# Mamo1031/Multimodal-MTRSSM

Measured on AMD Instinct MI355X. Metric: seq-steps/s (BxT) MoPoE-MRSSM train step, higher is better.
Workload: dtype bf16x2-split, fp32 accumulate; 1 GPU; BASELINE configs[1]: MoPoE-MRSSM train step, B=64/GPU T=50 deter=200 stoch=30, vision 1x64x64 + audio 1x128x32 + action 4; global_batch=64, seq_len=50, parallelism=dp1, hidden=200, embed=256, categoricals_x_classes=6x5, residual_blocks=3, activation=ELU, optimizer=AdamW lr 1e-3 + clip 10 (fused HIP), params=4151600, streams=1, launch=eager (host enqueues every launch), backend=none, rccl_ranks=0, collective_ranks=0, noise=uniforms keyed by global batch row (parallel.GlobalRowNoise)

## Files before the change

### include/mtrssm.h

```cpp
#ifndef MTRSSM_H
#define MTRSSM_H

#include <stddef.h>
#include <stdint.h>

#ifdef __cplusplus
extern "C" {
#endif

#define MTRSSM_VERSION 100

#define MTRSSM_OK 0
#define MTRSSM_EINVAL (-1)
#define MTRSSM_ELAUNCH (-2)
#define MTRSSM_ELDS (-3)

#define MTRSSM_ACT_IDENTITY 0
#define MTRSSM_ACT_RELU 1
#define MTRSSM_ACT_ELU 2
#define MTRSSM_ACT_TANH 3

int mtrssm_version(void);
const char* mtrssm_last_error(void);
const char* mtrssm_last_kernel(void);
// ... 52 lines not shown
  const int32_t* modality;
} MtrssmMrssmFwdIO;

int mtrssm_mrssm_rollout_fwd(const MtrssmMrssmDims* dims, const MtrssmMrssmFwdWeights* w,
                             const MtrssmMrssmFwdIO* io, void* stream);

typedef struct MtrssmMrssmClusterWeights {
  const float* w1s_t;
  const float* wf_t;
  const float* bf;
  const float* whh_t;
  const float* bhh;
  const float* wh1_t;
  const float* b3;
  const float* w4;
  const float* b4;
  const float* wa2;
  const float* ba2;
  const float* wv2;
  const float* bv2;
} MtrssmMrssmClusterWeights;
int mtrssm_mrssm_cluster_supported(const MtrssmMrssmDims* dims);
int64_t mtrssm_mrssm_cluster_workspace_bytes(const MtrssmMrssmDims* dims);
int mtrssm_mrssm_rollout_fwd_cluster(const MtrssmMrssmDims* dims, const MtrssmMrssmClusterWeights* weights, const MtrssmMrssmFwdIO* io,
                                     void* workspace, int64_t workspace_bytes, void* stream);

typedef struct MtrssmMrssmBwdWeights {
  const float* w1s_t;
  const float* w2;
  const float* wih;
  const float* whh;
  const float* wh1;
  const float* w4;
  const float* wa2;
  const float* wv2;
} MtrssmMrssmBwdWeights;

typedef struct MtrssmMrssmBwdIO {
  const float* deter0;
  const float* deter;
  const float* prior_logits;
  const float* post_logits;
  const float* sv_h1;
  const float* sv_h2;
  const float* sv_gates;
  const float* sv_heads;
  const float* sv_la;
  const float* sv_lv;
  const float* g_deter;
  const float* g_post_stoch;
  const float* g_prior_stoch;
  const float* g_post_logits;
  const float* g_prior_logits;
  const float* g_kl;
  float* g_deter0;
  float* g_stoch0;
  float* d_z1;
  float* d_h2;
  float* d_gi;
  float* d_gh;
  float* d_zh;
  float* d_lp;
  float* d_la;
  float* d_lv;
  const float* expert_logw;
  float* g_expert_logw;
  const int32_t* modality;
} MtrssmMrssmBwdIO;

int64_t mtrssm_mrssm_cluster_bwd_workspace_bytes(const MtrssmMrssmDims* dims);
int mtrssm_mrssm_rollout_bwd_cluster(const MtrssmMrssmDims* dims, const MtrssmMrssmClusterWeights* weights, const MtrssmMrssmBwdIO* io,
                                     void* workspace, int64_t workspace_bytes, void* stream);

int mtrssm_mrssm_wide_supported(const MtrssmMrssmDims* dims, int32_t pieces);
int64_t mtrssm_mrssm_wide_workspace_bytes(const MtrssmMrssmDims* dims, int32_t pieces);
int64_t mtrssm_mrssm_wide_bwd_workspace_bytes(const MtrssmMrssmDims* dims, int32_t pieces);
int mtrssm_mrssm_rollout_fwd_wide(const MtrssmMrssmDims* dims, const MtrssmMrssmClusterWeights* weights, const MtrssmMrssmFwdIO* io,
                                  int32_t pieces, void* workspace, int64_t workspace_bytes, void* stream);
int mtrssm_mrssm_rollout_bwd_wide(const MtrssmMrssmDims* dims, const MtrssmMrssmClusterWeights* weights, const MtrssmMrssmBwdIO* io,
                                  int32_t pieces, void* workspace, int64_t workspace_bytes, void* stream);

int mtrssm_mrssm_rollout_bwd(const MtrssmMrssmDims* dims, const MtrssmMrssmBwdWeights* w,
                             const MtrssmMrssmBwdIO* io, void* stream);

typedef struct MtrssmMmtrssmDims {
  int32_t B, T;
  int32_t LD, HD;
  int32_t H;
  int32_t KL, CL;
  int32_t KH, CH;
  int32_t act;
  int32_t post;
  float tau_l, tau_h;
  float keep_l, keep_h;
  float kl_w_post, kl_w_prior;
  int32_t rows_per_block;
  int32_t threads;
} MtrssmMmtrssmDims;

typedef struct MtrssmMmtrssmFwdWeights {
  const float* wxl_s_t;
  const float* wdl_t;
  const float* wxh_t;
  const float* wdh_t;
  const float* bh;
  const float* wl1_t;
  const float* bl1;
  const float* wh1_t;
  const float* bh1;
  const float* wlp2;
  const float* blp2;
  const float* wa2;
  const float* ba2;
  const float* wv2;
  const float* bv2;
  const float* whp2;
  const float* bhp2;
  const float* whq2;
  const float* bhq2;
} MtrssmMmtrssmFwdWeights;

typedef struct MtrssmMmtrssmFwdIO {
  const float* xl;
  const float* pa;
  const float* pv;
  const float* deter_l0;
  const float* deter_h0;
  const float* hidden_l0;
  const float* hidden_h0;
  const float* stoch_l0;
  const float* stoch_h0;
  const float* u_post_l;
  const float* u_post_h;
  const float* u_prior_l;
  const float* u_prior_h;
  float* deter_l;
  float* deter_h;
  float* hidden_l;
  float* hidden_h;
  float* prior_logits_l;
  float* prior_logits_h;
  float* prior_stoch_l;
  float* prior_stoch_h;
  float* post_logits_l;
  float* post_logits_h;
  float* post_stoch_l;
  float* post_stoch_h;
  float* kl_l;
  float* kl_h;
  float* sv_l1;
  float* sv_h1;
  float* sv_la;
  float* sv_lv;
  const float* expert_logw;
  const int32_t* modality;
} MtrssmMmtrssmFwdIO;

int mtrssm_mmtrssm_rollout_fwd(const MtrssmMmtrssmDims* dims, const MtrssmMmtrssmFwdWeights* w,
                               const MtrssmMmtrssmFwdIO* io, void* stream);

typedef struct MtrssmMmtrssmBwdWeights {
  const float* wxl_s_t;
  const float* wdl;
  const float* wxh_t;
  const float* wdh;
  const float* wl1;
// ... 246 lines not shown
```

### multimodal_mtrssm_amd/_lib.py

```python

from __future__ import annotations

import ctypes as C
import os
from pathlib import Path

import torch
from torch import Tensor

_HERE = Path(__file__).resolve().parent
LIB_PATH = _HERE / "libmtrssm_hip.so"

ACT_IDS = {"Identity": 0, "ReLU": 1, "ELU": 2, "Tanh": 3}

_f = C.c_float
_i = C.c_int32
_p = C.c_void_p


def _struct(name: str, fields: list[tuple[str, type]]) -> type:
    return type(name, (C.Structure,), {"_fields_": fields})


def _ptrs(*names: str) -> list[tuple[str, type]]:
    return [(n, _p) for n in names]


MrssmDims = _struct("MtrssmMrssmDims", [
    ("B", _i), ("T", _i), ("D", _i), ("H", _i), ("K", _i), ("C", _i), ("act", _i), ("post", _i),
    ("kl_w_post", _f), ("kl_w_prior", _f), ("rows_per_block", _i), ("threads", _i),
])
MrssmFwdWeights = _struct("MtrssmMrssmFwdWeights", _ptrs(
    "w1s_t", "w2_t", "b2", "wih_t", "bih", "whh_t", "bhh", "wh1_t", "b3", "w4", "b4", "wa2", "ba2", "wv2", "bv2"))
MrssmFwdIO = _struct("MtrssmMrssmFwdIO", _ptrs(
    "xa", "pa", "pv", "deter0", "stoch0", "u_post", "u_prior",
    "deter", "prior_logits", "prior_stoch", "post_logits", "post_stoch", "kl",
    "sv_h1", "sv_h2", "sv_gates", "sv_heads", "sv_la", "sv_lv", "expert_logw", "modality"))
MrssmClusterWeights = _struct("MtrssmMrssmClusterWeights", _ptrs(
    "w1s_t", "wf_t", "bf", "whh_t", "bhh", "wh1_t", "b3", "w4", "b4", "wa2", "ba2", "wv2", "bv2"))
MrssmBwdWeights = _struct("MtrssmMrssmBwdWeights", _ptrs("w1s_t", "w2", "wih", "whh", "wh1", "w4", "wa2", "wv2"))
MrssmBwdIO = _struct("MtrssmMrssmBwdIO", _ptrs(
    "deter0", "deter", "prior_logits", "post_logits", "sv_h1", "sv_h2", "sv_gates", "sv_heads", "sv_la", "sv_lv",
    "g_deter", "g_post_stoch", "g_prior_stoch", "g_post_logits", "g_prior_logits", "g_kl",
    "g_deter0", "g_stoch0", "d_z1", "d_h2", "d_gi", "d_gh", "d_zh", "d_lp", "d_la", "d_lv", "expert_logw", "g_expert_logw", "modality"))

MmtrssmDims = _struct("MtrssmMmtrssmDims", [
    ("B", _i), ("T", _i), ("LD", _i), ("HD", _i), ("H", _i), ("KL", _i), ("CL", _i), ("KH", _i), ("CH", _i),
    ("act", _i), ("post", _i), ("tau_l", _f), ("tau_h", _f), ("keep_l", _f), ("keep_h", _f),
    ("kl_w_post", _f), ("kl_w_prior", _f), ("rows_per_block", _i), ("threads", _i),
])
MmtrssmFwdWeights = _struct("MtrssmMmtrssmFwdWeights", _ptrs(
    "wxl_s_t", "wdl_t", "wxh_t", "wdh_t", "bh", "wl1_t", "bl1", "wh1_t", "bh1",
    "wlp2", "blp2", "wa2", "ba2", "wv2", "bv2", "whp2", "bhp2", "whq2", "bhq2"))
MmtrssmFwdIO = _struct("MtrssmMmtrssmFwdIO", _ptrs(
    "xl", "pa", "pv", "deter_l0", "deter_h0", "hidden_l0", "hidden_h0", "stoch_l0", "stoch_h0",
    "u_post_l", "u_post_h", "u_prior_l", "u_prior_h",
    "deter_l", "deter_h", "hidden_l", "hidden_h", "prior_logits_l", "prior_logits_h", "prior_stoch_l", "prior_stoch_h",
    "post_logits_l", "post_logits_h", "post_stoch_l", "post_stoch_h", "kl_l", "kl_h",
    "sv_l1", "sv_h1", "sv_la", "sv_lv", "expert_logw", "modality"))
MmtrssmBwdWeights = _struct("MtrssmMmtrssmBwdWeights", _ptrs(
    "wxl_s_t", "wdl", "wxh_t", "wdh", "wl1", "wh1", "wlp2", "wa2", "wv2", "whp2", "whq2"))
MmtrssmBwdIO = _struct("MtrssmMmtrssmBwdIO", _ptrs(
    "deter_l0", "deter_h0", "deter_l", "deter_h", "prior_logits_l", "prior_logits_h", "post_logits_l", "post_logits_h",
    "sv_l1", "sv_h1", "sv_la", "sv_lv",
    "g_deter_l", "g_deter_h", "g_hidden_l", "g_hidden_h", "g_post_stoch_l", "g_post_stoch_h", "g_prior_stoch_l",
    "g_prior_stoch_h", "g_post_logits_l", "g_post_logits_h", "g_prior_logits_l", "g_prior_logits_h", "g_kl_l", "g_kl_h",
    "g_deter_l0", "g_deter_h0", "g_hidden_l0", "g_hidden_h0", "g_stoch_l0", "g_stoch_h0",
    "d_ul", "d_uh", "d_zl1", "d_zh1", "d_lpl", "d_la", "d_lv", "d_lph", "d_lqh", "expert_logw", "g_expert_logw", "modality"))

ConvGeom = _struct("MtrssmConvGeom", [(n, _i) for n in (
    "N", "C", "Hs", "Ws", "C2", "Cpad", "KH", "KW", "SS", "TS", "OFFY", "OFFX", "Hq", "Wq", "OS", "QY", "QX", "Ho", "Wo",
    "Cout", "CoutPad", "pre_act", "act", "mfma_split")])

Gemm = _struct("MtrssmGemm", _ptrs("A", "B", "C", "bias", "zgrad", "colsum") + [(n, _i) for n in (
    "M", "N", "R", "lda", "ldb", "ldc", "ldz", "a_rmajor", "b_rmajor", "act_a", "act_b", "act_out", "act_z", "accumulate", "split_r")]
    + [("tickets", _p), ("n_tickets", _i), ("mfma_split", _i)])

ElboSchedule = _struct("MtrssmElboSchedule", [(n, _f) for n in ("c0", "c1", "free0", "free1", "w_a", "w_v", "beta_start", "warmup")])

STATE_MAX = 6
StateTable = _struct("MtrssmStateTable", [
    ("count", _i), ("width", _i * STATE_MAX), ("src_stride", C.c_int64 * STATE_MAX), ("src", _p * STATE_MAX), ("alt", _p * STATE_MAX),
    ("dst", _p * STATE_MAX)])

SYMBOLS: dict[str, tuple[type | None, list[type]]] = {
    "mtrssm_version": (C.c_int, []),
    "mtrssm_last_error": (C.c_char_p, []),
    "mtrssm_last_kernel": (C.c_char_p, []),
    "mtrssm_mrssm_rollout_fwd": (C.c_int, [C.POINTER(MrssmDims), C.POINTER(MrssmFwdWeights), C.POINTER(MrssmFwdIO), _p]),
    "mtrssm_mrssm_cluster_supported": (C.c_int, [C.POINTER(MrssmDims)]),
    "mtrssm_mrssm_cluster_workspace_bytes": (C.c_int64, [C.POINTER(MrssmDims)]),
    "mtrssm_mrssm_rollout_fwd_cluster": (C.c_int, [C.POINTER(MrssmDims), C.POINTER(MrssmClusterWeights), C.POINTER(MrssmFwdIO), _p, C.c_int64, _p]),
    "mtrssm_mrssm_cluster_bwd_workspace_bytes": (C.c_int64, [C.POINTER(MrssmDims)]),
    "mtrssm_mrssm_rollout_bwd_cluster": (C.c_int, [C.POINTER(MrssmDims), C.POINTER(MrssmClusterWeights), C.POINTER(MrssmBwdIO), _p, C.c_int64, _p]),
    "mtrssm_mrssm_wide_supported": (C.c_int, [C.POINTER(MrssmDims), _i]),
    "mtrssm_mrssm_wide_workspace_bytes": (C.c_int64, [C.POINTER(MrssmDims), _i]),
    "mtrssm_mrssm_wide_bwd_workspace_bytes": (C.c_int64, [C.POINTER(MrssmDims), _i]),
    "mtrssm_mrssm_rollout_fwd_wide": (C.c_int, [C.POINTER(MrssmDims), C.POINTER(MrssmClusterWeights), C.POINTER(MrssmFwdIO), _i, _p, C.c_int64, _p]),
    "mtrssm_mrssm_rollout_bwd_wide": (C.c_int, [C.POINTER(MrssmDims), C.POINTER(MrssmClusterWeights), C.POINTER(MrssmBwdIO), _i, _p, C.c_int64, _p]),
    "mtrssm_mrssm_rollout_bwd": (C.c_int, [C.POINTER(MrssmDims), C.POINTER(MrssmBwdWeights), C.POINTER(MrssmBwdIO), _p]),
    "mtrssm_mmtrssm_rollout_fwd": (C.c_int, [C.POINTER(MmtrssmDims), C.POINTER(MmtrssmFwdWeights), C.POINTER(MmtrssmFwdIO), _p]),
    "mtrssm_mmtrssm_rollout_bwd": (C.c_int, [C.POINTER(MmtrssmDims), C.POINTER(MmtrssmBwdWeights), C.POINTER(MmtrssmBwdIO), _p]),
    "mtrssm_mmtrssm_wide_supported": (C.c_int, [C.POINTER(MmtrssmDims), _i]),
    "mtrssm_mmtrssm_wide_workspace_bytes": (C.c_int64, [C.POINTER(MmtrssmDims), _i]),
    "mtrssm_mmtrssm_wide_bwd_workspace_bytes": (C.c_int64, [C.POINTER(MmtrssmDims), _i]),
    "mtrssm_mmtrssm_rollout_fwd_wide": (C.c_int, [C.POINTER(MmtrssmDims), C.POINTER(MmtrssmFwdWeights), C.POINTER(MmtrssmFwdIO), _i, _p, C.c_int64, _p]),
    "mtrssm_mmtrssm_rollout_bwd_wide": (C.c_int, [C.POINTER(MmtrssmDims), C.POINTER(MmtrssmBwdWeights), C.POINTER(MmtrssmBwdIO), _i, _p, C.c_int64, _p]),
    "mtrssm_conv_gather_gemm": (C.c_int, [C.POINTER(ConvGeom), _p, _p, _p, _p, _p, _p, _p, _p, _p]),
    "mtrssm_conv_gather_gemm_pair": (C.c_int, [C.POINTER(ConvGeom), _p, _p, _p, _p, _p, _p, _p, _p,
                                               C.POINTER(ConvGeom), _p, _p, _p, _p, _p, _p, _p, _p, _p]),
    "mtrssm_conv_gather_pair_merges": (C.c_int, [C.POINTER(ConvGeom), C.POINTER(ConvGeom), _i]),
    "mtrssm_residual_block_fwd_supported": (C.c_int, [C.POINTER(ConvGeom)]),
    "mtrssm_residual_block_fwd": (C.c_int, [C.POINTER(ConvGeom), _p, _p, _p, _p, _p, _p, _p, C.POINTER(ConvGeom), _p, _p, _p, _p, _p, _p, _p, _p]),
    "mtrssm_pack_conv_weight": (C.c_int, [_p, _i, _i, _i, _i, C.c_int64, C.c_int64, C.c_int64, C.c_int64, _i, _i, _i, _p, _p, _p]),
    "mtrssm_pack_conv_weights": (C.c_int, [_p, _i, _i, _p]),
    "mtrssm_unpack_conv_grads": (C.c_int, [_p, _i, _i, _p]),
    "mtrssm_conv_weight_grad": (C.c_int, [C.POINTER(ConvGeom), _p, _p, _p, _i, _p, _p, _p, C.c_int64, _p]),
    "mtrssm_conv_weight_grad_deferred": (C.c_int, [C.POINTER(ConvGeom), _p, _p, _p, _i, _p, _p, _p, C.c_int64, _p]),
    "mtrssm_residual_bwd1x1_supported": (C.c_int, [C.POINTER(ConvGeom)]),
    "mtrssm_residual_bwd1x1": (C.c_int, [C.POINTER(ConvGeom), _p, _p, _p, _p, _p, _p, _p, C.c_int64, _i, _p]),
    "mtrssm_conv_weight_grad_src_bias_supported": (C.c_int, [C.POINTER(ConvGeom), _i]),
    "mtrssm_conv_weight_grad_src_bias": (C.c_int, [C.POINTER(ConvGeom), _p, _p, _i, _p, _p, _p, C.c_int64, _i, _p]),
    "mtrssm_conv_weight_grad_reduce": (C.c_int, [_p]),
    "mtrssm_conv_weight_grad_workspace_bytes": (C.c_int64, [C.POINTER(ConvGeom), _i]),
    "mtrssm_residual_bwd1x1_pair_supported": (C.c_int, [C.POINTER(ConvGeom), C.POINTER(ConvGeom)]),
    "mtrssm_residual_bwd1x1_pair": (C.c_int, [C.POINTER(ConvGeom), _p, _p, _p, _p, _p, _p, _p, C.c_int64,
                                              C.POINTER(ConvGeom), _p, _p, _p, _p, _p, _p, _p, C.c_int64, _i, _p]),
    "mtrssm_conv_weight_grad_pair_supported": (C.c_int, [C.POINTER(ConvGeom), C.POINTER(ConvGeom)]),
    "mtrssm_conv_weight_grad_pair": (C.c_int, [C.POINTER(ConvGeom), _p, _p, _p, _p, _p, C.c_int64,
                                               C.POINTER(ConvGeom), _p, _p, _p, _p, _p, C.c_int64, _i, _p]),
    "mtrssm_channel_sum": (C.c_int, [_p, _i, _i, _i, _p, _p]),
    "mtrssm_convt_k4s2_thin": (C.c_int, [_i, _i, _i, _i, _i, _p, _p, _p, _i, _i, _p, _p]),
    "mtrssm_convt_k4s2_band_supported": (C.c_int, [_i, _i, _i, _i, _i]),
    "mtrssm_convt_k4s2_band": (C.c_int, [_i, _i, _i, _i, _i, _p, _p, _p, _i, _i, _p, _p]),
    "mtrssm_convt_quad_supported": (C.c_int, [C.POINTER(ConvGeom)]),
    "mtrssm_convt_quad": (C.c_int, [C.POINTER(ConvGeom), _p, C.POINTER(C.c_void_p), _p, _p, _p, C.POINTER(ConvGeom), _p, C.POINTER(C.c_void_p),
                                    _p, _p, _p, _p]),
    "mtrssm_conv_tgather_thin": (C.c_int, [_i] * 11 + [_p, _p, _p, _i, _i, _p, _p, _p, _p]),
    "mtrssm_episode_gather": (C.c_int, [_p, _p, _p, C.c_int64, C.c_int64, C.c_int64, C.c_int64, C.c_int64, _f, _p, _p, _p]),
    "mtrssm_episode_gather_window": (C.c_int, [_p, _p, _p, _p, C.c_int64, C.c_int64, C.c_int64, C.c_int64, C.c_int64, _f, _p, _p, _p]),
    "mtrssm_state_select": (C.c_int, [C.POINTER(StateTable), _p, C.c_int64, _p]),
    "mtrssm_state_save": (C.c_int, [C.POINTER(StateTable), C.c_int64, C.c_int64, _p]),
    "mtrssm_state_save_at": (C.c_int, [C.POINTER(StateTable), _p, C.c_int64, C.c_int64, _p]),
    "mtrssm_episode_gather_ragged": (C.c_int, [_p, _p, _p, _p, _p, C.c_int64, C.c_int64, C.c_int64, C.c_int64, C.c_int64, _f, _p, _p, _p, _p]),
    "mtrssm_episode_gather_seeded": (C.c_int, [_p, _p, _p, _p, _p, C.c_uint32, C.c_uint32, C.c_uint32, C.c_int64, C.c_int64, C.c_int64, C.c_int64,
                                               C.c_int64, _f, _p, _p, _p]),
    "mtrssm_step_mask_ragged": (C.c_int, [_p, _p, C.c_int64, C.c_int64, C.c_int64, _f, _f, C.c_int64, C.c_int64, _p, _p, _p, _p, _p, _p, _p, _p]),
    "mtrssm_step_mask_forecast": (C.c_int, [_p, _p, _p, C.c_int64, C.c_int64, C.c_int64, _f, _f, C.c_int64, C.c_int64, C.c_int64, C.c_int64, _p, _p, _p,
                                            _p, _p, _p, _p, _p, _p]),
    "mtrssm_ensemble_score": (C.c_int, [_p, _p, _p, C.c_int64, C.c_int64, C.c_int64, C.c_int64, _i, _p, _p, _p, _p, _p, _p]),
    "mtrssm_horizon_table": (C.c_int, [_p, C.c_int64, _p, _p, C.c_int64, C.c_int64, _p, _p, _p]),
    "mtrssm_digit_features": (C.c_int, [_p, C.c_int64, _p, C.c_int64, _i, _p, _p, _p, _p, _p, _p]),
    "mtrssm_digit_head": (C.c_int, [_p, _p, _p, C.c_int64, _p, C.c_int64, _p, _p, _p]),
    "mtrssm_word_counts": (C.c_int, [_p, _p, C.c_int64, _p, _p]),
    "mtrssm_elbo_combine_counted_fwd": (C.c_int, [_p, _p, _p, _p, _p, _p, C.c_int64, C.c_float, C.c_float, _p, _p, _p, _p, _p]),
    "mtrssm_elbo_combine_counted_bwd": (C.c_int, [_p, _p, _p, _p, _p, _p, C.c_int64, C.c_float, C.c_float, _p, _p, _p, _p, _p]),
    "mtrssm_elbo_schedule_fwd": (C.c_int, [_p, _p, _p, _p, _p, _p, _p, C.c_int64, ElboSchedule, _p, _p, _p, _p, _p, _p, _p]),
    "mtrssm_elbo_schedule_bwd": (C.c_int, [_p, _p, _p, _p, _p, _p, _p, _p, _p, C.c_int64, ElboSchedule, _p, _p, _p, _p, _p]),
    "mtrssm_elbo_combine_fwd": (C.c_int, [_p, _p, _p, _p, C.c_int64, C.c_float, C.c_float, _p, _p, _p, _p, _p]),
    "mtrssm_elbo_combine_bwd": (C.c_int, [_p, _p, _p, _p, C.c_int64, C.c_float, C.c_float, _p, _p, _p, _p, _p]),
    "mtrssm_categorical_sample_fwd": (C.c_int, [_p, _p, C.c_int64, _i, _i, _p, _p, _p, _p]),
    "mtrssm_categorical_sample_bwd": (C.c_int, [_p, _p, _p, C.c_int64, _i, _i, _p, _p]),
    "mtrssm_gaussian_nll_fwd": (C.c_int, [_p, _p, C.c_int64, C.c_int64, _i, _p, _p]),
    "mtrssm_gaussian_nll_bwd": (C.c_int, [_p, _p, _p, C.c_int64, C.c_int64, _i, _p, _p]),
    "mtrssm_gaussian_nll_masked_fwd": (C.c_int, [_p, _p, _p, _p, C.c_int64, C.c_int64, _i, _p, _p]),
    "mtrssm_gaussian_nll_masked_bwd": (C.c_int, [_p, _p, _p, _p, _p, C.c_int64, C.c_int64, _i, _p, _p]),
    "mtrssm_modality_dropout": (C.c_int, [_p, C.c_int64, C.c_int64, C.c_int64, _f, _f, C.c_int64, C.c_int64, _p, _p, _p, _p, _p, _p]),
    "mtrssm_sumsq": (C.c_int, [_p, C.c_int64, _p, _p]),
    "mtrssm_adamw_step": (C.c_int, [_p, _p, _p, _p, C.c_int64, _p, _f, _f, _f, _f, _f, _f, _f, _i, _p]),
    "mtrssm_gemm": (C.c_int, [C.POINTER(Gemm), _p]),
    "mtrssm_gemm_group": (C.c_int, [C.POINTER(Gemm), _i, _p]),
    "mtrssm_clear": (C.c_int, [_p, C.c_int64, _p]),
    "mtrssm_adamw_prepare": (C.c_int, [_p, C.c_int64, _p, _p, _p, _f, _f, _p]),
    "mtrssm_adamw_apply": (C.c_int, [_p, _p, _p, _p, _p, C.c_int64, _p, _p, _p, _f, _f, _f, _f, _f, _f, _p]),
}

_LIB: C.CDLL | None = None


class MtrssmLibraryError(RuntimeError):
    """The HIP library is missing or a kernel call failed.  There is no fallback path."""


# ... 113 lines not shown
```

### multimodal_mtrssm_amd/cnn.py

```python

from __future__ import annotations

from typing import Any

import torch
from torch import Tensor, nn

from multimodal_mtrssm_amd import _lib
from multimodal_mtrssm_amd.linear import linear
from multimodal_mtrssm_amd.conv import (
    gemm_pieces,
    conv2d,
    conv2d_pair,
    conv_transpose2d,
    conv_transpose2d_pair,
    residual_block,
    residual_block_pair,
)


def _act(name: str) -> nn.Module:
    return getattr(nn, name)()


def _cfg(config: Any) -> dict[str, Any]:
    return dict(config) if isinstance(config, dict) else dict(vars(config))


def _conv(x: Tensor, m: nn.Conv2d, *, pre_act: bool, act: int, coords: Tensor | None = None) -> Tensor:
    return conv2d(x, m.weight, m.bias, stride=m.stride[0], padding=m.padding[0], pre_act=pre_act, act=act, coords=coords)


def _deconv(x: Tensor, m: nn.ConvTranspose2d, *, pre_act: bool, act: int) -> Tensor:
    return conv_transpose2d(x, m.weight, m.bias, stride=m.stride[0], padding=m.padding[0],
                            output_padding=m.output_padding[0], pre_act=pre_act, act=act)


class ResidualBlock(nn.Module):

    def __init__(self, channels: int, intermediate: int, activation_name: str) -> None:
        super().__init__()
        self.conv3 = nn.Conv2d(channels, intermediate, 3, 1, 1)
        self.conv1 = nn.Conv2d(intermediate, channels, 1, 1, 0)
        self.act_id = _lib.ACT_IDS[activation_name]

    def forward(self, x: Tensor) -> Tensor:
        return residual_block(x, self.conv3.weight, self.conv3.bias, self.conv1.weight, self.conv1.bias, act=self.act_id)

    def params(self) -> tuple[Tensor, Tensor, Tensor, Tensor]:
        return self.conv3.weight, self.conv3.bias, self.conv1.weight, self.conv1.bias


def _res_pair(res_a: nn.ModuleList, res_b: nn.ModuleList, xa: Tensor, xb: Tensor) -> tuple[Tensor, Tensor]:
    n = min(len(res_a), len(res_b))
    for ba, bb in zip(res_a[:n], res_b[:n], strict=True):
        if ba.act_id == bb.act_id and ba.conv3.weight.shape == bb.conv3.weight.shape and ba.conv1.weight.shape == bb.conv1.weight.shape:
            xa, xb = residual_block_pair(xa, ba.params(), xb, bb.params(), act=ba.act_id)
        else:
            xa, xb = ba(xa), bb(xb)
    for ba in res_a[n:]:
        xa = ba(xa)
    for bb in res_b[n:]:
        xb = bb(xb)
    return xa, xb


def _same_layer(ma: nn.Module, mb: nn.Module) -> bool:
    return (ma.weight.shape[0] == mb.weight.shape[0] and ma.weight.shape[2:] == mb.weight.shape[2:] and ma.stride == mb.stride
            and ma.padding == mb.padding and getattr(ma, "output_padding", 0) == getattr(mb, "output_padding", 0))


def _conv_pair(xa: Tensor, ma: nn.Conv2d, ca: Tensor | None, xb: Tensor, mb: nn.Conv2d, cb: Tensor | None, *, pre_act: bool,
               act_a: int, act_b: int) -> tuple[Tensor, Tensor]:
    if _same_layer(ma, mb) and act_a == act_b:
        return conv2d_pair((xa, ma.weight, ma.bias, ma.stride[0], ma.padding[0], pre_act, act_a, ca),
                           (xb, mb.weight, mb.bias, mb.stride[0], mb.padding[0], pre_act, act_b, cb))
    return _conv(xa, ma, pre_act=pre_act, act=act_a, coords=ca), _conv(xb, mb, pre_act=pre_act, act=act_b, coords=cb)


def encode_pair(enc_a: "Encoder", enc_b: "Encoder", xa: Tensor, xb: Tensor) -> tuple[Tensor, Tensor]:
    lead_a, lead_b = xa.shape[:-3], xb.shape[:-3]
    xa, ca = enc_a.prepare(xa)
    xb, cb = enc_b.prepare(xb)
    if len(enc_a.convs) == len(enc_b.convs) and (enc_a.res_in is None) == (enc_b.res_in is None):
        for i, (ma, mb) in enumerate(zip(enc_a.convs, enc_b.convs, strict=True)):
            xa, xb = _conv_pair(xa, ma, ca if i == 0 else None, xb, mb, cb if i == 0 else None, pre_act=i > 0, act_a=enc_a.act_id,
                                act_b=enc_b.act_id)
        if enc_a.res_in is not None:
            xa, xb = _conv_pair(xa, enc_a.res_in, None, xb, enc_b.res_in, None, pre_act=True, act_a=enc_a.act_id, act_b=enc_b.act_id)
    else:
        xa, xb = enc_a.stem_convs(xa, ca), enc_b.stem_convs(xb, cb)
    xa, xb = _res_pair(enc_a.res, enc_b.res, xa, xb)
    return enc_a.head(xa, lead_a), enc_b.head(xb, lead_b)


def decode_pair(dec_a: "Decoder", dec_b: "Decoder", fa: Tensor, fb: Tensor, *, raw: bool = False) -> tuple[Tensor, Tensor]:
    lead_a, lead_b = fa.shape[:-1], fb.shape[:-1]
    xa, xb = dec_a.stem(fa), dec_b.stem(fb)
    xa, xb = _res_pair(dec_a.res, dec_b.res, xa, xb)
    if len(dec_a.deconvs) != len(dec_b.deconvs) or (len(dec_a.res) > 0) != (len(dec_b.res) > 0):
        return dec_a.tail(xa, lead_a, raw=raw), dec_b.tail(xb, lead_b, raw=raw)
    for i, (ma, mb) in enumerate(zip(dec_a.deconvs, dec_b.deconvs, strict=True)):
        pre = i > 0 or len(dec_a.res) > 0
        if _same_layer(ma, mb) and dec_a.act_id == dec_b.act_id:
            xa, xb = conv_transpose2d_pair(
                (xa, ma.weight, ma.bias, ma.stride[0], ma.padding[0], ma.output_padding[0], pre, dec_a.act_id),
                (xb, mb.weight, mb.bias, mb.stride[0], mb.padding[0], mb.output_padding[0], pre, dec_b.act_id))
        else:
            xa, xb = _deconv(xa, ma, pre_act=pre, act=dec_a.act_id), _deconv(xb, mb, pre_act=pre, act=dec_b.act_id)
    return dec_a.finish(xa, lead_a, raw=raw), dec_b.finish(xb, lead_b, raw=raw)


class Encoder(nn.Module):

    def __init__(self, config: Any) -> None:
        super().__init__()
        self.cfg = _cfg(config)
        self.coord_conv = bool(self.cfg.get("coord_conv", False))
        self.act = _act(self.cfg["activation_name"])
        self.act_id = _lib.ACT_IDS[self.cfg["activation_name"]]
        self.out_act = _act(self.cfg.get("out_activation_name", "Identity"))
        self.convs = nn.ModuleList()
        self.res_in: nn.Module | None = None
        self.res = nn.ModuleList()
        self.linears = nn.ModuleList()
        self.input_shape: tuple[int, int, int] | None = None
        self._coords: Tensor | None = None
        if self.cfg.get("input_shape") is not None:
            self.materialize(tuple(self.cfg["input_shape"]))

    def materialize(self, input_shape: tuple[int, ...]) -> None:
        cfg = self.cfg
        c, h, w = (int(v) for v in input_shape)
        self.input_shape = (c, h, w)
        cin = c + (2 if self.coord_conv else 0)
        for ch, k, s, p in zip(cfg["channels"], cfg["kernel_sizes"], cfg["strides"], cfg["paddings"], strict=True):
            self.convs.append(nn.Conv2d(cin, ch, k, s, p))
            h, w, cin = (h + 2 * p - k) // s + 1, (w + 2 * p - k) // s + 1, ch
        if cfg.get("num_residual_blocks", 0) > 0:
            rout = cfg["residual_output_size"]
            self.res_in = nn.Conv2d(cin, rout, 3, 1, 1)
            for _ in range(cfg["num_residual_blocks"]):
                self.res.append(ResidualBlock(rout, cfg["residual_intermediate_size"], cfg["activation_name"]))
            cin = rout
        width = cin * h * w
        for out in cfg["linear_sizes"]:
            self.linears.append(nn.Linear(width, out))
            width = out

    def _coord_channels(self, x: Tensor) -> Tensor:
        h, w = x.shape[-2:]
        if self._coords is None or self._coords.shape[-2:] != (h, w) or self._coords.device != x.device:
            yy = torch.linspace(-1.0, 1.0, h, dtype=x.dtype, device=x.device)
            xx = torch.linspace(-1.0, 1.0, w, dtype=x.dtype, device=x.device)
            self._coords = torch.stack([yy[:, None].expand(h, w), xx[None, :].expand(h, w)], dim=0)
        return self._coords

    def forward(self, x: Tensor) -> Tensor:
        lead = x.shape[:-3]
        x = self.stem(x)
        for blk in self.res:
            x = blk(x)
        return self.head(x, lead)

    def prepare(self, x: Tensor) -> tuple[Tensor, Tensor | None]:
        if len(self.linears) == 0:
            self.materialize(tuple(x.shape[-3:]))
            self.to(x.device)
        x = x.reshape(-1, *x.shape[-3:]).float()
        return x, (self._coord_channels(x) if self.coord_conv else None)

    def stem_convs(self, x: Tensor, coords: Tensor | None) -> Tensor:
        for i, conv in enumerate(self.convs):
            x = _conv(x, conv, pre_act=i > 0, act=self.act_id, coords=coords if i == 0 else None)
        if self.res_in is not None:
            x = _conv(x, self.res_in, pre_act=True, act=self.act_id)
        return x

    def stem(self, x: Tensor) -> Tensor:
        return self.stem_convs(*self.prepare(x))

    def head(self, x: Tensor, lead: torch.Size) -> Tensor:
        x = x.flatten(start_dim=1)
        for lin in self.linears:
            x = linear(x, lin.weight, lin.bias, pre_act=self.act_id, pieces=gemm_pieces())
        return self.out_act(x).reshape(*lead, -1)


class Decoder(nn.Module):

    def __init__(self, config: Any) -> None:
        super().__init__()
        cfg = self.cfg = _cfg(config)
        self.act = _act(cfg["activation_name"])
        self.act_id = _lib.ACT_IDS[cfg["activation_name"]]
        self.out_act = _act(cfg.get("out_activation_name", "Identity"))
        self.conv_in_shape = tuple(int(v) for v in cfg["conv_in_shape"])
        self.linears = nn.ModuleList()
        self.res = nn.ModuleList()
        self.deconvs = nn.ModuleList()
        cin = self.conv_in_shape[0]
        for _ in range(cfg.get("num_residual_blocks", 0)):
            self.res.append(ResidualBlock(cin, cfg["residual_intermediate_size"], cfg["activation_name"]))
        n = len(cfg["channels"])
        ops = cfg.get("output_paddings", [0] * n)
        for ch, k, s, p, op in zip(cfg["channels"], cfg["kernel_sizes"], cfg["strides"], cfg["paddings"], ops, strict=True):
            self.deconvs.append(nn.ConvTranspose2d(cin, ch, k, s, p, op))
            cin = ch
        if cfg.get("in_features") is not None:
            self.materialize(int(cfg["in_features"]))

    def materialize(self, in_features: int) -> None:
        width = in_features
        for out in self.cfg["linear_sizes"]:
            self.linears.append(nn.Linear(width, out))
            width = out
        self.in_features = in_features

    def forward(self, f: Tensor, *, raw: bool = False) -> Tensor:
        lead = f.shape[:-1]
        x = self.stem(f)
        for blk in self.res:
            x = blk(x)
        return self.tail(x, lead, raw=raw)

    @property
    def out_act_id(self) -> int | None:
        name = type(self.out_act).__name__
        return {"Identity": 0, "Tanh": 3}.get(name)

    def stem(self, f: Tensor) -> Tensor:
        if len(self.linears) == 0:
            self.materialize(f.shape[-1])
            self.to(f.device)
        x = f.reshape(-1, f.shape[-1])
        for i, lin in enumerate(self.linears):
            x = linear(x, lin.weight, lin.bias, pre_act=self.act_id if i > 0 else 0, pieces=gemm_pieces())
        return x.reshape(-1, *self.conv_in_shape)

    def tail(self, x: Tensor, lead: torch.Size, *, raw: bool = False) -> Tensor:
        for i, dc in enumerate(self.deconvs):
            x = _deconv(x, dc, pre_act=i > 0 or len(self.res) > 0, act=self.act_id)
        return self.finish(x, lead, raw=raw)

    def finish(self, x: Tensor, lead: torch.Size, *, raw: bool = False) -> Tensor:
        if not raw:
            x = self.out_act(x)
        return x.reshape(*lead, *x.shape[-3:])
```

### multimodal_mtrssm_amd/core.py

```python

from __future__ import annotations

import torch
from torch import Tensor, nn

from multimodal_mtrssm_amd import cnn, conv, scan
from multimodal_mtrssm_amd.carry import StateCarry
from multimodal_mtrssm_amd.distributions import MultiOneHot, MultiOneHotFactory, draw_uniforms, kl_divergence, onehot_from_uniforms
from multimodal_mtrssm_amd.digits import DigitClassifier, word_counts
from multimodal_mtrssm_amd.dropout import ModalityDropout, StepMask, ragged_step_mask
from multimodal_mtrssm_amd.experts import ExpertWeights
from multimodal_mtrssm_amd.forecast import Forecast
from multimodal_mtrssm_amd.networks import MTRNN, Representation, Transition
from multimodal_mtrssm_amd.objective import likelihood
from multimodal_mtrssm_amd.schedule import ElboSchedule, ElboTerms
from multimodal_mtrssm_amd.skill import ForecastSkill, SkillTable
from multimodal_mtrssm_amd.words import TransitionTable, WordTransitions
from multimodal_mtrssm_amd.state import MTState, State

try:
    from lightning import LightningModule as _Base
except ImportError:

    class _Base(nn.Module):
        @property
        def device(self) -> torch.device:
            for p in self.parameters():
                return p.device
            return torch.device("cpu")

        def log_dict(self, *args, **kwargs) -> None:
            return None


Noise = dict[str, Tensor | None]

def _pairable(a: nn.Module, b: nn.Module, kind: type) -> bool:
    return conv.PAIR_LAUNCH and isinstance(a, kind) and isinstance(b, kind)


def _st_onehot(dist: MultiOneHot, u: Tensor | None) -> Tensor:
    if u is None:
        return dist.rsample()
    onehot = onehot_from_uniforms(dist.probs.detach(), u.to(dist.probs))
    return (onehot + (dist.probs - dist.probs.detach())).flatten(start_dim=-2)


class _CategoricalHead(torch.autograd.Function):

    @staticmethod
    def forward(ctx, logits: Tensor, u: Tensor, cats: int, classes: int):
        from multimodal_mtrssm_amd import _lib

        ctx.set_materialize_grads(False)
        logits, u = logits.contiguous().float(), u.contiguous().float()
        rows = logits.numel() // (cats * classes)
        logp = torch.empty(*logits.shape[:-1], cats, classes, device=logits.device, dtype=torch.float32)
        probs, onehot = torch.empty_like(logp), torch.empty_like(logits)
        _lib.check(_lib.load().mtrssm_categorical_sample_fwd(_lib.ptr(logits), _lib.ptr(u), rows, cats, classes, _lib.ptr(logp), _lib.ptr(probs),
                                                             _lib.ptr(onehot), _lib.stream_ptr(logits.device)), "mtrssm_categorical_sample_fwd")
        ctx.save_for_backward(probs)
        ctx.dims = (rows, cats, classes)
        return onehot, logp, probs

    @staticmethod
    def backward(ctx, g_stoch, g_logp, g_probs):
        from multimodal_mtrssm_amd import _lib

        (probs,) = ctx.saved_tensors
        rows, cats, classes = ctx.dims
        gp = None
        if g_stoch is not None:
            gp = g_stoch.reshape(probs.shape)
        if g_probs is not None:
            gp = g_probs if gp is None else gp + g_probs
        if gp is None and g_logp is None:
            return None, None, None, None
        gp = None if gp is None else gp.contiguous().float()
        gl = None if g_logp is None else g_logp.contiguous().float()
        d = torch.empty(*probs.shape[:-2], cats * classes, device=probs.device, dtype=torch.float32)
        _lib.check(_lib.load().mtrssm_categorical_sample_bwd(_lib.ptr(probs), _lib.ptr(gp), _lib.ptr(gl), rows, cats, classes, _lib.ptr(d),
                                                             _lib.stream_ptr(probs.device)), "mtrssm_categorical_sample_bwd")
        return d, None, None, None


class _ElboCombine(torch.autograd.Function):

    @staticmethod
    def forward(ctx, nll_a: Tensor, nll_v: Tensor, kl0: Tensor, kl1: Tensor | None, c0: float, c1: float):
        from multimodal_mtrssm_amd import _lib

        ctx.set_materialize_grads(False)
        nll_a, nll_v, kl0 = nll_a.contiguous().float(), nll_v.contiguous().float(), kl0.contiguous().float()
        kl1 = None if kl1 is None else kl1.contiguous().float()
        outs = [torch.empty((), device=kl0.device, dtype=torch.float32) for _ in range(4)]
        _lib.check(_lib.load().mtrssm_elbo_combine_fwd(_lib.ptr(nll_a), _lib.ptr(nll_v), _lib.ptr(kl0), _lib.ptr(kl1), kl0.numel(), float(c0), float(c1),
                                                       _lib.ptr(outs[0]), _lib.ptr(outs[1]), _lib.ptr(outs[2]) if kl1 is not None else None,
                                                       _lib.ptr(outs[3]), _lib.stream_ptr(kl0.device)), "mtrssm_elbo_combine_fwd")
        ctx.meta = (kl0.shape, None if kl1 is None else kl1.shape, float(c0), float(c1))
        ctx.dev = kl0.device
        return outs[0], outs[1], outs[2], outs[3]

    @staticmethod
    def backward(ctx, g_recon, g_k0, g_k1, g_loss):
        from multimodal_mtrssm_amd import _lib

        shape0, shape1, c0, c1 = ctx.meta
        n = 1
        for d in shape0:
            n *= d
        g_a, g_v = (torch.empty((), device=ctx.dev, dtype=torch.float32) for _ in range(2))
        g_kl0 = torch.empty(shape0, device=ctx.dev, dtype=torch.float32)
        g_kl1 = None if shape1 is None else torch.empty(shape1, device=ctx.dev, dtype=torch.float32)
        opt = lambda t: None if t is None else _lib.ptr(t.contiguous().float())
        _lib.check(_lib.load().mtrssm_elbo_combine_bwd(opt(g_recon), opt(g_k0), opt(g_k1) if shape1 is not None else None, opt(g_loss), n, c0, c1,
                                                       _lib.ptr(g_a), _lib.ptr(g_v), _lib.ptr(g_kl0), _lib.ptr(g_kl1), _lib.stream_ptr(ctx.dev)),
                   "mtrssm_elbo_combine_bwd")
        return g_a, g_v, g_kl0, g_kl1, None, None


class _ElboCombineCounted(torch.autograd.Function):

    @staticmethod
    def forward(ctx, nll_a: Tensor, nll_v: Tensor, kl0: Tensor, kl1: Tensor | None, live: Tensor, count: Tensor, c0: float, c1: float):
        from multimodal_mtrssm_amd import _lib

        ctx.set_materialize_grads(False)
        nll_a, nll_v, kl0 = nll_a.contiguous().float(), nll_v.contiguous().float(), kl0.contiguous().float()
        kl1 = None if kl1 is None else kl1.contiguous().float()
        live, count = live.contiguous().float(), count.contiguous().float()
        if live.numel() != kl0.numel() or count.numel() != 1:
            msg = f"live must have one entry per KL step ({kl0.numel()}), count one; got {live.numel()} and {count.numel()}"
            raise ValueError(msg)
        outs = [torch.empty((), device=kl0.device, dtype=torch.float32) for _ in range(4)]
        _lib.check(_lib.load().mtrssm_elbo_combine_counted_fwd(
            _lib.ptr(nll_a), _lib.ptr(nll_v), _lib.ptr(kl0), _lib.ptr(kl1), _lib.ptr(live), _lib.ptr(count), kl0.numel(), float(c0), float(c1),
            _lib.ptr(outs[0]), _lib.ptr(outs[1]), _lib.ptr(outs[2]) if kl1 is not None else None, _lib.ptr(outs[3]),
            _lib.stream_ptr(kl0.device)), "mtrssm_elbo_combine_counted_fwd")
        ctx.meta = (kl0.shape, None if kl1 is None else kl1.shape, float(c0), float(c1))
        ctx.dev = kl0.device
        ctx.save_for_backward(live, count)
        return outs[0], outs[1], outs[2], outs[3]

    @staticmethod
    def backward(ctx, g_recon, g_k0, g_k1, g_loss):
        from multimodal_mtrssm_amd import _lib

        shape0, shape1, c0, c1 = ctx.meta
        live, count = ctx.saved_tensors
        g_a, g_v = (torch.empty((), device=ctx.dev, dtype=torch.float32) for _ in range(2))
        g_kl0 = torch.empty(shape0, device=ctx.dev, dtype=torch.float32)
        g_kl1 = None if shape1 is None else torch.empty(shape1, device=ctx.dev, dtype=torch.float32)
        opt = lambda t: None if t is None else _lib.ptr(t.contiguous().float())
        _lib.check(_lib.load().mtrssm_elbo_combine_counted_bwd(
            opt(g_recon), opt(g_k0), opt(g_k1) if shape1 is not None else None, opt(g_loss), _lib.ptr(live), _lib.ptr(count), live.numel(), c0, c1,
            _lib.ptr(g_a), _lib.ptr(g_v), _lib.ptr(g_kl0), _lib.ptr(g_kl1), _lib.stream_ptr(ctx.dev)), "mtrssm_elbo_combine_counted_bwd")
        return g_a, g_v, g_kl0, g_kl1, None, None, None, None


class _ElboScheduled(torch.autograd.Function):

    @staticmethod
    def forward(ctx, nll_a: Tensor, nll_v: Tensor, kl0: Tensor, kl1: Tensor | None, live: Tensor | None, count: Tensor | None,
                step: Tensor | None, sched: ElboSchedule, c0: float, c1: float):
        from multimodal_mtrssm_amd import _lib

# ... 197 lines not shown
        self.vision_decoder = vision_decoder
        self.scan_rows_per_block = 0
        self.scan_threads = 0
        self.modality_dropout: ModalityDropout | None = None
        self.state_carry: StateCarry | None = None
        self.forecast: Forecast | None = None
        self.val_forecast: Forecast | None = None
        self.elbo_schedule: ElboSchedule | None = None
        self.val_skill: ForecastSkill | None = None
        self.skill_table: SkillTable | None = None
        self.expert_weights: ExpertWeights | None = None
        self.weights_timeseries: Tensor | None = None
        self._weights_both: Tensor | None = None

    @staticmethod
    def get_observations_from_batch(batch: tuple[Tensor, ...]) -> tuple[Tensor, Tensor]:
        return batch[1], batch[2]

    @staticmethod
    def get_initial_observation(observations: tuple[Tensor, Tensor]) -> tuple[Tensor, Tensor]:
        audio_obs, vision_obs = observations
        return audio_obs[:, 0], vision_obs[:, 0]

    @staticmethod
    def get_targets_from_batch(batch: tuple[Tensor, ...]) -> dict[str, Tensor]:
        return {"recon/audio": batch[4], "recon/vision": batch[5]}

    @staticmethod
    def get_modality_mask_from_batch(batch: tuple[Tensor, ...]) -> Tensor | None:
        return batch[6] if len(batch) > 6 else None

    def encode_observation(self, observation: tuple[Tensor, Tensor] | Tensor, modality_mask: Tensor | None = None) -> Tensor:
        if isinstance(observation, tuple):
            audio_obs, vision_obs = observation
            ea = None if audio_obs is None else self.audio_encoder(audio_obs)
            ev = None if vision_obs is None else self.vision_encoder(vision_obs)
            if ea is None and ev is None:
                msg = "observation: at least one of (audio_obs, vision_obs) must be given"
                raise ValueError(msg)
            return _masked_mean_embed(ea, ev, modality_mask)
        return observation

    def decode_state(self, state: State | MTState) -> dict[str, Tensor]:
        return {"recon/audio": self.audio_decoder(state.feature), "recon/vision": self.vision_decoder(state.feature)}

    @staticmethod
    def compute_reconstruction_loss(reconstructions: dict[str, Tensor], targets: dict[str, Tensor],
                                    modality_mask: Tensor | None = None) -> dict[str, Tensor]:
        fa = fv = None
        if modality_mask is not None:
            fa, fv = modality_mask[..., 0], modality_mask[..., 1]
        audio = likelihood(prediction=reconstructions["recon/audio"], target=targets["recon/audio"], event_ndims=3, frame_mask=fa)
        vision = likelihood(prediction=reconstructions["recon/vision"], target=targets["recon/vision"], event_ndims=3, frame_mask=fv)
        return {"recon": audio + vision, "recon/audio": audio, "recon/vision": vision}

    def _encode_both(self, audio_obs: Tensor, vision_obs: Tensor) -> tuple[Tensor, Tensor]:
        if _pairable(self.audio_encoder, self.vision_encoder, cnn.Encoder):
            return cnn.encode_pair(self.audio_encoder, self.vision_encoder, audio_obs, vision_obs)
        return self.audio_encoder(audio_obs), self.vision_encoder(vision_obs)

    def _reconstruction_losses(self, feature: Tensor, targets: dict[str, Tensor], *, sum_recon: bool = True,
                               modality_mask: Tensor | None = None, step_mask: StepMask | None = None) -> dict[str, Tensor]:
        da, dv = self.audio_decoder, self.vision_decoder
        fused = isinstance(da, cnn.Decoder) and isinstance(dv, cnn.Decoder) and da.out_act_id is not None and dv.out_act_id is not None
        if fused and _pairable(da, dv, cnn.Decoder):
            pa, pv = cnn.decode_pair(da, dv, feature, feature, raw=True)
        elif fused:
            pa, pv = da(feature, raw=True), dv(feature, raw=True)
        else:
            pa, pv = da(feature), dv(feature)
        fa = fv = ca = cv = None
        if modality_mask is not None:
            fa, fv = modality_mask[..., 0], modality_mask[..., 1]
        if step_mask is not None:
            ca, cv = (step_mask.present_audio, step_mask.count_audio), (step_mask.present_vision, step_mask.count_vision)
        audio = likelihood(prediction=pa, target=targets["recon/audio"], event_ndims=3, out_act=da.out_act_id if fused else 0,
                           frame_mask=fa, frame_present=ca)
        vision = likelihood(prediction=pv, target=targets["recon/vision"], event_ndims=3, out_act=dv.out_act_id if fused else 0,
                            frame_mask=fv, frame_present=cv)
        if not sum_recon:
            return {"recon/audio": audio, "recon/vision": vision}
        return {"recon": audio + vision, "recon/audio": audio, "recon/vision": vision}

    def _initial_from_embed(self, obs_embed: Tensor, u_init: Tensor | None) -> State:
        deter = self.init_proj(obs_embed)
        logits = self.transition.rnn_to_prior_projector(deter)
        dist, stoch = _sampled_head(self.representation.distribution_factory, logits, u_init)
        return State(deter=deter, distribution=dist, stoch=stoch)

    def _initial_embed(self, observation: tuple[Tensor, Tensor] | Tensor, modality_mask: Tensor | None) -> Tensor:
        if modality_mask is not None:
            if not isinstance(observation, tuple):
                msg = "modality_mask needs the (audio_obs, vision_obs) tuple"
                raise ValueError(msg)
            ref = observation[0] if observation[0] is not None else observation[1]
            _check_modality_mask(modality_mask, ref.shape[0], None, ref.device, first_step=True)
            for j, name in enumerate(("audio", "vision")):
                if observation[j] is None and bool(modality_mask[:, j].any()):
                    msg = f"modality_mask marks {name} present, but the observation carries None for it"
                    raise ValueError(msg)
        return self.encode_observation(observation, modality_mask)

    def initial_state(self, observation: tuple[Tensor, Tensor] | Tensor, noise: Noise | None = None,
                      modality_mask: Tensor | None = None) -> State:
        u = None if noise is None else noise.get("u_init")
        return self._initial_from_embed(self._initial_embed(observation, modality_mask), u).to(self.device)

    def noise_shapes(self, batch: int, steps: int) -> dict[str, tuple[int, ...]]:
        k = self.transition.distribution_factory.category_size
        return self._with_mask_noise({"u_init": (batch, k), "u_post": (batch, steps, k)}, batch, steps)

    def _with_mask_noise(self, shapes: dict[str, tuple[int, ...]], batch: int, steps: int) -> dict[str, tuple[int, ...]]:
        if self.modality_dropout is not None:
            shapes["u_mask"] = self.modality_dropout.noise_shape(batch, steps)
        if self.forecast is not None:
            shapes["u_context"] = self.forecast.noise_shape(batch)
        return shapes

    def _rollout_embedded(self, actions: Tensor, audio_embed: Tensor | None, vision_embed: Tensor | None, prev_state: State,
                          noise: Noise | None, *, sample_prior: bool, modality: Tensor | None = None,
                          expert_log_weights: Tensor | None = None) -> dict[str, Tensor]:
        noise = noise or {}
        B, T = actions.shape[:2]
        K = self.transition.distribution_factory.category_size
        logw = self._expert_logw(audio_embed, vision_embed, expert_log_weights, B, T)
        self._report_weights(logw, modality, B, T, actions.device)
        u_post = noise.get("u_post")
        u_prior = noise.get("u_prior")
        if u_post is None:
            u_post = _rand(actions, B, T, K)
        if u_prior is None and sample_prior:
            u_prior = _rand(actions, B, T, K)
        return scan.mrssm_posterior_rollout(
            self.transition, self.audio_representation, self.vision_representation, actions, audio_embed, vision_embed,
            prev_state.deter, prev_state.stoch, u_post, u_prior, balancing=bool(self.use_kl_balancing),
            rows_per_block=self.scan_rows_per_block, threads=self.scan_threads, modality=modality, expert_logw=logw,
        )

    def _expert_logw(self, audio_embed: Tensor | None, vision_embed: Tensor | None, explicit: Tensor | None, B: int, T: int) -> Tensor | None:
        if audio_embed is None or vision_embed is None:
            return None
        if explicit is not None:
            return scan.check_expert_logw(explicit, B, T)
        if self.expert_weights is None:
            return None
        return self.expert_weights(audio_embed, vision_embed)

    def _report_weights(self, logw: Tensor | None, codes: Tensor | None, B: int, T: int, device: torch.device) -> None:
        if logw is None and self.expert_weights is None:
            return
        with torch.no_grad():
            if codes is None:
                codes = torch.full((B, T), 3, device=device, dtype=torch.int32)
            self._weights_both = (codes & 3) == 3
            self.weights_timeseries = ExpertWeights.table(logw, codes & 3)

    def _posterior_from_rollout(self, out: dict[str, Tensor]) -> State:
        post = State(deter=out["deter"], distribution=self.audio_representation.distribution_factory(out["post_logits"]), stoch=out["post_stoch"])
        post.kl_per_step = out["kl"]
        return post

    def _states_from_rollout(self, out: dict[str, Tensor]) -> tuple[State, State]:
        factory = self.audio_representation.distribution_factory
        prior = State(deter=out["deter"], distribution=factory(out["prior_logits"]), stoch=out["prior_stoch"])
        return self._posterior_from_rollout(out), prior

    def rollout_representation(
# ... 343 lines not shown
                return None
            _check_modality_mask(mask, B, T, batch[0].device, first_step=True)
            return StepMask.from_mask(mask)
        if mask is not None:
            msg = "give a modality_mask (or a 7-tuple batch) or a modality_dropout, not both"
            raise ValueError(msg)
        if not isinstance(modality_dropout, ModalityDropout):
            msg = f"modality_dropout must be a ModalityDropout, got {type(modality_dropout).__name__}"
            raise ValueError(msg)
        return modality_dropout.sample(self._dropout_uniforms(batch, noise, modality_dropout, modality_dropout.world), T).step_mask()

    def shared_step(self, batch: tuple[Tensor, ...], noise: Noise | None = None, modality_mask: Tensor | None = None,
                    modality_dropout: ModalityDropout | None = None, state_carry: StateCarry | None = None,
                    reset: Tensor | None = None, *, carry_prefix: str = "train", lengths: Tensor | None = None,
                    forecast: Forecast | None = None, elbo_schedule: ElboSchedule | None = None,
                    expert_log_weights: Tensor | None = None) -> dict[str, Tensor]:
        if forecast is not None:
            if modality_mask is not None or self.get_modality_mask_from_batch(batch) is not None:
                msg = "forecast= decides what the model observes: a modality_mask (or a 7-tuple batch) already says what is seen, give one of them"
                raise ValueError(msg)
            if state_carry is not None:
                msg = "forecast= does not combine with state_carry: the state a forecast step ends with is an open-loop state, not one to continue from"
                raise ValueError(msg)
            return self._elbo_step(batch, noise, self._forecast_step_mask(batch, noise, forecast, modality_dropout, lengths), schedule=elbo_schedule,
                                   expert_log_weights=expert_log_weights)
        reset_host = None
        if state_carry is not None:
            reset_host = getattr(batch, "reset_host", None) if reset is None else (None if reset.is_cuda else reset)
        on_device = state_carry is not None and isinstance(reset, Tensor) and reset.is_cuda
        sm = self._step_mask(batch, noise, modality_mask, modality_dropout, lengths, reset_host, trust_reset=on_device)
        if state_carry is None:
            return self._elbo_step(batch, noise, sm, schedule=elbo_schedule, expert_log_weights=expert_log_weights)
        return self._elbo_step(batch, noise, sm, self._carry_of(batch, state_carry, reset, carry_prefix), schedule=elbo_schedule,
                               expert_log_weights=expert_log_weights)

    @staticmethod
    def _carry_of(batch: tuple[Tensor, ...], state_carry: StateCarry, reset: Tensor | None, prefix: str) -> tuple[StateCarry, str, Tensor]:
        if not isinstance(state_carry, StateCarry):
            msg = f"state_carry must be a StateCarry, got {type(state_carry).__name__}"
            raise ValueError(msg)
        dev = batch[0].device
        if reset is None:
            reset, reset_host = getattr(batch, "reset", None), getattr(batch, "reset_host", None)
            if reset is None:
                msg = "state_carry needs reset= (bool [B]) or a batch that carries one (an EpisodeBatch of a windowed loader)"
                raise ValueError(msg)
        elif not isinstance(reset, Tensor) or reset.dtype != torch.bool:
            msg = f"reset must be a bool tensor, got {getattr(reset, 'dtype', type(reset))}"
            raise ValueError(msg)
        else:
            reset_host = None if reset.is_cuda else reset
        if tuple(reset.shape) != (batch[0].shape[0],):
            msg = f"reset must have shape ({batch[0].shape[0]},), got {tuple(reset.shape)}"
            raise ValueError(msg)
        state_carry.check(prefix, batch[0].shape[0], reset_host)
        return state_carry, prefix, reset.to(dev).contiguous()

    _FRESH_KEYS = ("deter", "stoch")
    _LAST_KEYS = {"deter": "deter", "stoch": "post_stoch"}

    def _state0(self, fresh: State | MTState, carry: tuple[StateCarry, str, Tensor] | None) -> State | MTState:
        if carry is None:
            return fresh
        sc, prefix, reset = carry
        got = sc.select(prefix, reset, {k: getattr(fresh, k) for k in self._FRESH_KEYS})
        return self._state_like(fresh, got)

    @staticmethod
    def _state_like(fresh: State, got: dict[str, Tensor]) -> State:
        return State(deter=got["deter"], distribution=fresh.distribution, stoch=got["stoch"])

    def _save_carry(self, out: dict[str, Tensor], carry: tuple[StateCarry, str, Tensor] | None, last: Tensor | None = None) -> None:
        if carry is not None:
            carry[0].save(carry[1], {k: out[v] for k, v in self._LAST_KEYS.items()}, last)

    def _elbo_step(self, batch: tuple[Tensor, ...], noise: Noise | None, sm: StepMask | None,
                   carry: tuple[StateCarry, str, Tensor] | None = None, schedule: ElboSchedule | None = None,
                   expert_log_weights: Tensor | None = None) -> dict[str, Tensor]:
        action_input = batch[0]
        audio_obs, vision_obs = self.get_observations_from_batch(batch)
        conv.begin_step(audio_obs.device)
        audio_embed, vision_embed = self._encode_both(audio_obs, vision_obs)
        u_init = None if noise is None else noise.get("u_init")
        state0 = self._initial_from_embed(_masked_mean_embed(audio_embed[:, 0], vision_embed[:, 0], None if sm is None else sm.mask0),
                                          u_init)
        state0 = self._state0(state0, carry)
        out = self._rollout_embedded(action_input, audio_embed, vision_embed, state0, noise, sample_prior=False,
                                     modality=None if sm is None else sm.codes, expert_log_weights=expert_log_weights)
        self._save_carry(out, carry, None if sm is None else sm.last)
        feature = torch.cat([out["deter"], out["post_stoch"]], dim=-1)
        parts = self._reconstruction_losses(feature, self.get_targets_from_batch(batch), sum_recon=False, step_mask=sm)
        recon, kl_div, _, loss = _elbo(parts["recon/audio"], parts["recon/vision"], out["kl"], float(self.kl_coeff), step_mask=sm, schedule=schedule)
        if schedule is not None:
            return {"recon": recon, **parts, "kl": kl_div, "loss": loss, "kl_raw": schedule.stats["kl_raw"]}
        return {"recon": recon, **parts, "kl": kl_div, "loss": loss}

    def _step(self, batch: tuple[Tensor, ...], prefix: str, *, with_loss_key: bool, modality_dropout: ModalityDropout | None = None,
              forecast: Forecast | None = None, elbo_schedule: ElboSchedule | None = None) -> dict[str, Tensor]:
        if forecast is not None:
            loss_dict = self.shared_step(batch, modality_dropout=modality_dropout, state_carry=self.state_carry, forecast=forecast,
                                         elbo_schedule=elbo_schedule)
        elif self.state_carry is None:
            loss_dict = self.shared_step(batch, modality_dropout=modality_dropout, elbo_schedule=elbo_schedule)
        else:
            loss_dict = self.shared_step(batch, modality_dropout=modality_dropout, state_carry=self.state_carry, carry_prefix=prefix,
                                         elbo_schedule=elbo_schedule)
        renamed = {"loss": loss_dict["loss"]} if with_loss_key else {}
        renamed[f"{prefix}/loss"] = loss_dict["loss"]
        for key, value in loss_dict.items():
            if key != "loss":
                renamed[f"{prefix}/{key}"] = value
        self.log_dict(renamed, prog_bar=True, sync_dist=True, on_step=False, on_epoch=True)
        return renamed

    def training_step(self, batch: tuple[Tensor, ...], _: int = 0) -> dict[str, Tensor]:
        return self._step(batch, "train", with_loss_key=True, modality_dropout=self.modality_dropout, forecast=self.forecast,
                          elbo_schedule=self.elbo_schedule)

    def validation_step(self, batch: tuple[Tensor, ...], _batch_index: int = 0) -> dict[str, Tensor]:
        logged = self._step(batch, "val", with_loss_key=False)
        if self.expert_weights is not None and self.weights_timeseries is not None:
            both = self._weights_both.unsqueeze(-1).to(torch.float32)
            mean = (self.weights_timeseries * both).sum(dim=(0, 1)) / both.sum().clamp(min=1.0)
            weights = {f"val/weights/{name}": mean[i] for i, name in enumerate(("audio", "vision", "fused"))}
            self.log_dict(weights, prog_bar=False, sync_dist=True, on_step=False, on_epoch=True)
            logged.update(weights)
        if self.val_forecast is not None:
            fore = {f"val/forecast/{k}": v for k, v in self.shared_step(batch, forecast=self.val_forecast).items()}
            self.log_dict(fore, prog_bar=False, sync_dist=True, on_step=False, on_epoch=True)
            logged.update(fore)
        if self.val_skill is not None:
            self.skill_table = self.forecast_skill(batch, self.val_skill, table=self.skill_table)
        return logged

    def on_validation_epoch_end(self) -> dict[str, Tensor]:
        table, self.skill_table = self.skill_table, None
        if table is None:
            return {}
        table.all_reduce(getattr(self.val_skill, "group", None))
        logged = table.scalars("val/skill")
        self.log_dict(logged, prog_bar=False, sync_dist=False, on_step=False, on_epoch=True)
        return logged


class MoPoE_MMTRSSM(MoPoE_MRSSM):

    def __init__(
        self,
        *,
        audio_representation: Representation,
        vision_representation: Representation,
        audio_encoder: nn.Module,
        vision_encoder: nn.Module,
        audio_decoder: nn.Module,
        vision_decoder: nn.Module,
        init_proj: nn.Module,
        kl_coeff: float,
        use_kl_balancing: bool,
        action_size: int,
        hd_dim: int,
        hs_dim: int,
        ld_dim: int,
        ls_dim: int,
        l_tau: float,
        h_tau: float,
        l_prior: nn.Module,
        l_posterior: nn.Module,
        h_prior: nn.Module,
# ... 182 lines not shown
```

### multimodal_mtrssm_amd/csrc/capi.hip

```cpp
#include <stdarg.h>
#include <stdio.h>

#include "scan_common.h"

namespace mtrssm {

static thread_local char g_err[512] = "";
static thread_local const char* g_kernel = "";

void set_last_kernel(const char* name) { g_kernel = name; }

void set_error(const char* fmt, ...) {
  va_list ap;
  va_start(ap, fmt);
  vsnprintf(g_err, sizeof(g_err), fmt, ap);
  va_end(ap);
}

int mrssm_fwd_launch(const MtrssmMrssmDims*, const MtrssmMrssmFwdWeights*, const MtrssmMrssmFwdIO*, hipStream_t);
int mrssm_bwd_launch(const MtrssmMrssmDims*, const MtrssmMrssmBwdWeights*, const MtrssmMrssmBwdIO*, hipStream_t);
int mmtrssm_fwd_launch(const MtrssmMmtrssmDims*, const MtrssmMmtrssmFwdWeights*, const MtrssmMmtrssmFwdIO*, hipStream_t);
int mmtrssm_bwd_launch(const MtrssmMmtrssmDims*, const MtrssmMmtrssmBwdWeights*, const MtrssmMmtrssmBwdIO*, hipStream_t);
int conv_gather_gemm_launch(const MtrssmConvGeom*, const float*, const float*, const float*, const unsigned short*, const float*, const float*, const float*, float*, hipStream_t);
int episode_gather_launch(const float*, const int64_t*, const float*, int64_t, int64_t, int64_t, int64_t, int64_t, float, float*, float*, hipStream_t);
// ... 6 lines not shown
                                 int64_t, float, float*, float*, int32_t*, hipStream_t);
int episode_gather_seeded_launch(const float*, const int64_t*, const int32_t*, const int32_t*, int32_t*, uint32_t, uint32_t, uint32_t, int64_t, int64_t,
                                 int64_t, int64_t, int64_t, float, float*, float*, hipStream_t);
int step_mask_ragged_launch(const int32_t*, const float*, int64_t, int64_t, int64_t, float, float, int64_t, int64_t, int32_t*, float*, float*, float*,
                            unsigned char*, int32_t*, float*, hipStream_t);
int step_mask_forecast_launch(const int32_t*, const float*, const float*, int64_t, int64_t, int64_t, float, float, int64_t, int64_t, int64_t, int64_t,
                              int32_t*, float*, float*, float*, float*, unsigned char*, int32_t*, float*, hipStream_t);
int elbo_combine_counted_fwd_launch(const float*, const float*, const float*, const float*, const float*, const float*, int64_t, float, float, float*,
                                    float*, float*, float*, hipStream_t);
int elbo_combine_counted_bwd_launch(const float*, const float*, const float*, const float*, const float*, const float*, int64_t, float, float, float*,
                                    float*, float*, float*, hipStream_t);
int elbo_schedule_fwd_launch(const float*, const float*, const float*, const float*, const float*, const float*, const float*, int64_t,
                             MtrssmElboSchedule, float*, float*, float*, float*, float*, float*, hipStream_t);
int elbo_schedule_bwd_launch(const float*, const float*, const float*, const float*, const float*, const float*, const float*, const float*,
                             const float*, int64_t, MtrssmElboSchedule, float*, float*, float*, float*, hipStream_t);
int conv_gather_gemm_pair_launch(const MtrssmConvGeom*, const float*, const float*, const float*, const unsigned short*, const float*, const float*, const float*, float*,
                                 const MtrssmConvGeom*, const float*, const float*, const float*, const unsigned short*, const float*, const float*, const float*, float*, hipStream_t);
int conv_residual_fwd_supported(const MtrssmConvGeom*);
int conv_residual_fwd_launch(const MtrssmConvGeom*, const float*, const unsigned short*, const float*, const float*, const float*, float*, float*,
                             const MtrssmConvGeom*, const float*, const unsigned short*, const float*, const float*, const float*, float*, float*, hipStream_t);
int pack_conv_weight_launch(const float*, int, int, int, int, long, long, long, long, int, int, int, float*, unsigned short*, hipStream_t);
int pack_conv_weights_launch(const int64_t*, int, int, hipStream_t);
int conv_gather_pair_merges(const MtrssmConvGeom*, const MtrssmConvGeom*, bool);
int conv_weight_grad_launch(const MtrssmConvGeom*, const float*, const float*, const float*, int, float*, float*, void*, size_t, size_t*, hipStream_t);
int conv_weight_grad_deferred_launch(const MtrssmConvGeom*, const float*, const float*, const float*, int, float*, float*, void*, size_t, hipStream_t);
int conv_weight_grad_reduce_flush(hipStream_t);
int conv_residual_bwd1x1_supported(const MtrssmConvGeom*);
int conv_residual_bwd1x1_launch(const MtrssmConvGeom*, const float*, const float*, const unsigned short*, float*, float*, float*, void*, size_t, int,
                                hipStream_t);
int conv_residual_bwd1x1_pair_supported(const MtrssmConvGeom*, const MtrssmConvGeom*);
int conv_residual_bwd1x1_pair_launch(const MtrssmConvGeom*, const float*, const float*, const unsigned short*, float*, float*, float*, void*, size_t,
                                     const MtrssmConvGeom*, const float*, const float*, const unsigned short*, float*, float*, float*, void*, size_t, int,
                                     hipStream_t);
int conv_weight_grad_pair_supported(const MtrssmConvGeom*, const MtrssmConvGeom*);
int conv_weight_grad_pair_launch(const MtrssmConvGeom*, const float*, const float*, float*, float*, void*, size_t, const MtrssmConvGeom*, const float*,
                                 const float*, float*, float*, void*, size_t, int, hipStream_t);
int conv_weight_grad_src_bias_supported(const MtrssmConvGeom*, int);
int conv_weight_grad_src_bias_launch(const MtrssmConvGeom*, const float*, const float*, int, float*, float*, void*, size_t, int, hipStream_t);
int channel_sum_launch(const float*, int, int, int, float*, hipStream_t);
int convt_k4s2_band_supported(int, int, int, int, int);
int convt_k4s2_band_launch(int, int, int, int, int, const float*, const float*, const float*, int, int, float*, hipStream_t);
int convt_k4s2_thin_launch(int, int, int, int, int, const float*, const float*, const float*, int, int, float*, hipStream_t);
int conv_convt_quad_supported(const MtrssmConvGeom*);
int conv_convt_quad_launch(const MtrssmConvGeom*, const float*, const unsigned short* const*, const float*, const float*, float*,
                           const MtrssmConvGeom*, const float*, const unsigned short* const*, const float*, const float*, float*, hipStream_t);
int conv_tgather_thin_launch(int, int, int, int, int, int, int, int, int, int, int, const float*, const float*, const float*, int, int, const float*,
                             const float*, float*, hipStream_t);
int categorical_sample_fwd_launch(const float*, const float*, int64_t, int, int, float*, float*, float*, hipStream_t);
int categorical_sample_bwd_launch(const float*, const float*, const float*, int64_t, int, int, float*, hipStream_t);
int elbo_combine_fwd_launch(const float*, const float*, const float*, const float*, int64_t, float, float, float*, float*, float*, float*, hipStream_t);
int elbo_combine_bwd_launch(const float*, const float*, const float*, const float*, int64_t, float, float, float*, float*, float*, float*, hipStream_t);
int nll_fwd_launch(const float*, const float*, int64_t, int64_t, int, float*, hipStream_t);
int nll_bwd_launch(const float*, const float*, const float*, int64_t, int64_t, int, float*, hipStream_t);
int nll_masked_fwd_launch(const float*, const float*, const float*, const float*, int64_t, int64_t, int, float*, hipStream_t);
int nll_masked_bwd_launch(const float*, const float*, const float*, const float*, const float*, int64_t, int64_t, int, float*, hipStream_t);
int ensemble_score_launch(const float*, const float*, const int32_t*, int64_t, int64_t, int64_t, int64_t, int, float*, float*, float*, float*, float*,
                          hipStream_t);
int horizon_table_launch(const float*, int64_t, const int32_t*, const int32_t*, int64_t, int64_t, float*, float*, hipStream_t);
int digit_features_launch(const float*, int64_t, const int32_t*, int64_t, int, const float*, const float*, const float*, const float*, float*,
                          hipStream_t);
int digit_head_launch(const float*, const float*, const float*, int64_t, const int32_t*, int64_t, int32_t*, float*, hipStream_t);
int word_counts_launch(const int32_t*, const int32_t*, int64_t, float*, hipStream_t);
int modality_dropout_launch(const float*, int64_t, int64_t, int64_t, float, float, int64_t, int64_t, int32_t*, float*, float*, unsigned char*, float*,
                            hipStream_t);
int sumsq_launch(const float*, int64_t, float*, hipStream_t);
int adamw_launch(float*, const float*, float*, float*, int64_t, const float*, float, float, float, float, float, float, float, int, hipStream_t);
int gemm_launch(const MtrssmGemm*, hipStream_t);
int gemm_group_launch(const MtrssmGemm*, int, hipStream_t);
int debug_set_cluster_profile(void*);
int debug_set_resident_profile(void*);
int debug_set_wide_profile(void*);
int debug_set_mmt_profile(void*);
int mrssm_cluster_supported(const MtrssmMrssmDims*);
size_t mrssm_cluster_workspace_bytes(const MtrssmMrssmDims*);
size_t mrssm_cluster_bwd_workspace_bytes(const MtrssmMrssmDims*);
int mrssm_bwd_cluster_launch(const MtrssmMrssmDims*, const MtrssmMrssmClusterWeights*, const MtrssmMrssmBwdIO*, void*, size_t, hipStream_t);
int mrssm_fwd_cluster_launch(const MtrssmMrssmDims*, const MtrssmMrssmClusterWeights*, const MtrssmMrssmFwdIO*, void*, size_t, hipStream_t);
int unpack_conv_grads_launch(const int64_t*, int, int, hipStream_t);
int mrssm_wide_supported(const MtrssmMrssmDims*, int);
size_t mrssm_wide_workspace_bytes(const MtrssmMrssmDims*, int);
size_t mrssm_wide_bwd_workspace_bytes(const MtrssmMrssmDims*, int);
int mrssm_wide_fwd_launch(const MtrssmMrssmDims*, const MtrssmMrssmClusterWeights*, const MtrssmMrssmFwdIO*, int, void*, size_t, hipStream_t);
int mrssm_wide_bwd_launch(const MtrssmMrssmDims*, const MtrssmMrssmClusterWeights*, const MtrssmMrssmBwdIO*, int, void*, size_t, hipStream_t);
int adamw_prepare_launch(const float*, int64_t, float*, float*, const int*, float, float, hipStream_t);
int adamw_apply_launch(float*, const float*, float*, float*, const unsigned char*, int64_t, const float*, const float*, const int*, float, float, float,
                       float, float, float, hipStream_t);

int mmtrssm_wide_supported(const MtrssmMmtrssmDims*, int);
size_t mmtrssm_wide_workspace_bytes(const MtrssmMmtrssmDims*, int);
size_t mmtrssm_wide_bwd_workspace_bytes(const MtrssmMmtrssmDims*, int);
int mmtrssm_wide_fwd_launch(const MtrssmMmtrssmDims*, const MtrssmMmtrssmFwdWeights*, const MtrssmMmtrssmFwdIO*, int, void*, size_t, hipStream_t);
int mmtrssm_wide_bwd_launch(const MtrssmMmtrssmDims*, const MtrssmMmtrssmBwdWeights*, const MtrssmMmtrssmBwdIO*, int, void*, size_t, hipStream_t);

int device_cu_count() {
  static int cached[64] = {0};
  int dev = 0;
  if (hipGetDevice(&dev) != hipSuccess) { (void)hipGetLastError(); return 0; }
  if (dev < 0 || dev >= 64) return 0;
  if (cached[dev] > 0) return cached[dev];
  int v = 0;
  if (hipDeviceGetAttribute(&v, hipDeviceAttributeMultiprocessorCount, dev) != hipSuccess || v <= 0) { (void)hipGetLastError(); return 0; }
  cached[dev] = v;
  return v;
}

}

using namespace mtrssm;
#define MTRSSM_API extern "C" __attribute__((visibility("default")))

template <typename IO>
static bool expert_logw_ok(const IO* io, bool post, const char* entry) {
  if (io && post && io->expert_logw && !io->modality) {
    set_error("%s: expert_logw needs modality (pass code 3 everywhere when no modality is missing)", entry);
    return false;
  }
  return true;
}
template <typename IO>
static bool g_expert_logw_ok(const IO* io, const char* entry) {
  if (!expert_logw_ok(io, true, entry)) return false;
  if (io && io->g_expert_logw && !io->expert_logw) {
    set_error("%s: g_expert_logw needs expert_logw", entry);
    return false;
  }
  return true;
}

MTRSSM_API int mtrssm_version(void) { return MTRSSM_VERSION; }
MTRSSM_API const char* mtrssm_last_error(void) { return g_err; }
MTRSSM_API const char* mtrssm_last_kernel(void) { return g_kernel; }

MTRSSM_API int mtrssm_mrssm_rollout_fwd(const MtrssmMrssmDims* d, const MtrssmMrssmFwdWeights* w, const MtrssmMrssmFwdIO* io, void* stream) {
  if (!expert_logw_ok(io, d && d->post, "mrssm_rollout_fwd")) return MTRSSM_EINVAL;
  return mrssm_fwd_launch(d, w, io, static_cast<hipStream_t>(stream));
}
MTRSSM_API int mtrssm_mrssm_rollout_bwd(const MtrssmMrssmDims* d, const MtrssmMrssmBwdWeights* w, const MtrssmMrssmBwdIO* io, void* stream) {
  if (!g_expert_logw_ok(io, "mrssm_rollout_bwd")) return MTRSSM_EINVAL;
  return mrssm_bwd_launch(d, w, io, static_cast<hipStream_t>(stream));
}
MTRSSM_API int mtrssm_mmtrssm_rollout_fwd(const MtrssmMmtrssmDims* d, const MtrssmMmtrssmFwdWeights* w, const MtrssmMmtrssmFwdIO* io, void* stream) {
  if (!expert_logw_ok(io, d && d->post, "mmtrssm_rollout_fwd")) return MTRSSM_EINVAL;
  return mmtrssm_fwd_launch(d, w, io, static_cast<hipStream_t>(stream));
}
MTRSSM_API int mtrssm_mmtrssm_rollout_bwd(const MtrssmMmtrssmDims* d, const MtrssmMmtrssmBwdWeights* w, const MtrssmMmtrssmBwdIO* io, void* stream) {
  if (!g_expert_logw_ok(io, "mmtrssm_rollout_bwd")) return MTRSSM_EINVAL;
  return mmtrssm_bwd_launch(d, w, io, static_cast<hipStream_t>(stream));
}
MTRSSM_API int mtrssm_categorical_sample_fwd(const float* logits, const float* u, int64_t rows, int32_t K, int32_t C, float* logp, float* probs,
                                            float* onehot, void* stream) {
  return categorical_sample_fwd_launch(logits, u, rows, K, C, logp, probs, onehot, static_cast<hipStream_t>(stream));
}
MTRSSM_API int mtrssm_categorical_sample_bwd(const float* probs, const float* g_probs, const float* g_logp, int64_t rows, int32_t K, int32_t C,
                                            float* d_logits, void* stream) {
  return categorical_sample_bwd_launch(probs, g_probs, g_logp, rows, K, C, d_logits, static_cast<hipStream_t>(stream));
}
MTRSSM_API int mtrssm_elbo_combine_fwd(const float* nll_a, const float* nll_v, const float* kl0, const float* kl1, int64_t n, float c0, float c1,
                                      float* o_recon, float* o_k0, float* o_k1, float* o_loss, void* stream) {
  return elbo_combine_fwd_launch(nll_a, nll_v, kl0, kl1, n, c0, c1, o_recon, o_k0, o_k1, o_loss, static_cast<hipStream_t>(stream));
}
MTRSSM_API int mtrssm_elbo_combine_bwd(const float* g_recon, const float* g_k0, const float* g_k1, const float* g_loss, int64_t n, float c0,
                                      float c1, float* g_nll_a, float* g_nll_v, float* g_kl0, float* g_kl1, void* stream) {
  return elbo_combine_bwd_launch(g_recon, g_k0, g_k1, g_loss, n, c0, c1, g_nll_a, g_nll_v, g_kl0, g_kl1, static_cast<hipStream_t>(stream));
}
MTRSSM_API int mtrssm_gaussian_nll_fwd(const float* pred, const float* target, int64_t frames, int64_t event, int32_t act, float* out, void* stream) {
  return nll_fwd_launch(pred, target, frames, event, act, out, static_cast<hipStream_t>(stream));
}
MTRSSM_API int mtrssm_gaussian_nll_bwd(const float* pred, const float* target, const float* g_out, int64_t frames, int64_t event, int32_t act,
                                       float* g_pred, void* stream) {
  return nll_bwd_launch(pred, target, g_out, frames, event, act, g_pred, static_cast<hipStream_t>(stream));
}
MTRSSM_API int mtrssm_gaussian_nll_masked_fwd(const float* pred, const float* target, const float* present, const float* count, int64_t frames,
                                              int64_t event, int32_t act, float* out, void* stream) {
  return nll_masked_fwd_launch(pred, target, present, count, frames, event, act, out, static_cast<hipStream_t>(stream));
}
MTRSSM_API int mtrssm_gaussian_nll_masked_bwd(const float* pred, const float* target, const float* present, const float* count,
                                              const float* g_out, int64_t frames, int64_t event, int32_t act, float* g_pred, void* stream) {
  return nll_masked_bwd_launch(pred, target, present, count, g_out, frames, event, act, g_pred, static_cast<hipStream_t>(stream));
}
MTRSSM_API int mtrssm_modality_dropout(const float* u, int64_t b_global, int64_t steps, int64_t span, float p_audio, float p_vision, int64_t row0,
                                       int64_t b_local, int32_t* codes, float* present_audio, float* present_vision, uint8_t* mask0,
                                       float* counts, void* stream) {
  return modality_dropout_launch(u, b_global, steps, span, p_audio, p_vision, row0, b_local, codes, present_audio, present_vision, mask0, counts,
                                 static_cast<hipStream_t>(stream));
}
MTRSSM_API int mtrssm_sumsq(const float* x, int64_t n, float* out, void* stream) {
  return sumsq_launch(x, n, out, static_cast<hipStream_t>(stream));
}
MTRSSM_API int mtrssm_adamw_step(float* param, const float* grad, float* exp_avg, float* exp_avg_sq, int64_t n, const float* sumsq,
                                 float clip_norm, float grad_scale, float lr, float beta1, float beta2, float eps, float weight_decay,
                                 int32_t step, void* stream) {
  return adamw_launch(param, grad, exp_avg, exp_avg_sq, n, sumsq, clip_norm, grad_scale, lr, beta1, beta2, eps, weight_decay, step,
                      static_cast<hipStream_t>(stream));
}
MTRSSM_API int mtrssm_unpack_conv_grads(const int64_t* table, int32_t count, int32_t blocks_per_entry, void* stream) {
  return unpack_conv_grads_launch(table, count, blocks_per_entry, static_cast<hipStream_t>(stream));
}
MTRSSM_API int mtrssm_mrssm_cluster_supported(const MtrssmMrssmDims* d) { return mrssm_cluster_supported(d); }
MTRSSM_API int64_t mtrssm_mrssm_cluster_workspace_bytes(const MtrssmMrssmDims* d) { return (int64_t)mrssm_cluster_workspace_bytes(d); }
MTRSSM_API int mtrssm_mrssm_rollout_fwd_cluster(const MtrssmMrssmDims* d, const MtrssmMrssmClusterWeights* w, const MtrssmMrssmFwdIO* io,
                                                void* workspace, int64_t workspace_bytes, void* stream) {
  if (!expert_logw_ok(io, true, "mrssm_rollout_fwd_cluster")) return MTRSSM_EINVAL;
  return mrssm_fwd_cluster_launch(d, w, io, workspace, workspace_bytes < 0 ? 0 : (size_t)workspace_bytes, static_cast<hipStream_t>(stream));
}
extern "C" __attribute__((visibility("default"))) int mtrssm_debug_set_cluster_profile(void* buf) { return debug_set_cluster_profile(buf); }
extern "C" __attribute__((visibility("default"))) int mtrssm_debug_set_resident_profile(void* buf) { return debug_set_resident_profile(buf); }
extern "C" __attribute__((visibility("default"))) int mtrssm_debug_set_wide_profile(void* buf) { return debug_set_wide_profile(buf); }
extern "C" __attribute__((visibility("default"))) int mtrssm_debug_set_mmt_profile(void* buf) { return debug_set_mmt_profile(buf); }
MTRSSM_API int64_t mtrssm_mrssm_cluster_bwd_workspace_bytes(const MtrssmMrssmDims* d) { return (int64_t)mrssm_cluster_bwd_workspace_bytes(d); }
MTRSSM_API int mtrssm_mrssm_rollout_bwd_cluster(const MtrssmMrssmDims* d, const MtrssmMrssmClusterWeights* w, const MtrssmMrssmBwdIO* io,
                                                void* workspace, int64_t workspace_bytes, void* stream) {
  if (!g_expert_logw_ok(io, "mrssm_rollout_bwd_cluster")) return MTRSSM_EINVAL;
  return mrssm_bwd_cluster_launch(d, w, io, workspace, workspace_bytes < 0 ? 0 : (size_t)workspace_bytes, static_cast<hipStream_t>(stream));
}
MTRSSM_API int mtrssm_mrssm_wide_supported(const MtrssmMrssmDims* d, int32_t pieces) { return mrssm_wide_supported(d, pieces); }
MTRSSM_API int64_t mtrssm_mrssm_wide_workspace_bytes(const MtrssmMrssmDims* d, int32_t pieces) { return (int64_t)mrssm_wide_workspace_bytes(d, pieces); }
MTRSSM_API int64_t mtrssm_mrssm_wide_bwd_workspace_bytes(const MtrssmMrssmDims* d, int32_t pieces) {
  return (int64_t)mrssm_wide_bwd_workspace_bytes(d, pieces);
}
MTRSSM_API int mtrssm_mrssm_rollout_fwd_wide(const MtrssmMrssmDims* d, const MtrssmMrssmClusterWeights* w, const MtrssmMrssmFwdIO* io, int32_t pieces,
                                             void* workspace, int64_t workspace_bytes, void* stream) {
  if (!expert_logw_ok(io, true, "mrssm_rollout_fwd_wide")) return MTRSSM_EINVAL;
  return mrssm_wide_fwd_launch(d, w, io, pieces, workspace, workspace_bytes < 0 ? 0 : (size_t)workspace_bytes, static_cast<hipStream_t>(stream));
}
MTRSSM_API int mtrssm_mrssm_rollout_bwd_wide(const MtrssmMrssmDims* d, const MtrssmMrssmClusterWeights* w, const MtrssmMrssmBwdIO* io, int32_t pieces,
                                             void* workspace, int64_t workspace_bytes, void* stream) {
  if (!g_expert_logw_ok(io, "mrssm_rollout_bwd_wide")) return MTRSSM_EINVAL;
  return mrssm_wide_bwd_launch(d, w, io, pieces, workspace, workspace_bytes < 0 ? 0 : (size_t)workspace_bytes, static_cast<hipStream_t>(stream));
}
MTRSSM_API int mtrssm_mmtrssm_wide_supported(const MtrssmMmtrssmDims* d, int32_t pieces) { return mmtrssm_wide_supported(d, pieces); }
MTRSSM_API int64_t mtrssm_mmtrssm_wide_workspace_bytes(const MtrssmMmtrssmDims* d, int32_t pieces) { return (int64_t)mmtrssm_wide_workspace_bytes(d, pieces); }
MTRSSM_API int64_t mtrssm_mmtrssm_wide_bwd_workspace_bytes(const MtrssmMmtrssmDims* d, int32_t pieces) {
  return (int64_t)mmtrssm_wide_bwd_workspace_bytes(d, pieces);
}
MTRSSM_API int mtrssm_mmtrssm_rollout_fwd_wide(const MtrssmMmtrssmDims* d, const MtrssmMmtrssmFwdWeights* w, const MtrssmMmtrssmFwdIO* io, int32_t pieces,
                                               void* workspace, int64_t workspace_bytes, void* stream) {
  if (!expert_logw_ok(io, true, "mmtrssm_rollout_fwd_wide")) return MTRSSM_EINVAL;
  return mmtrssm_wide_fwd_launch(d, w, io, pieces, workspace, workspace_bytes < 0 ? 0 : (size_t)workspace_bytes, static_cast<hipStream_t>(stream));
}
MTRSSM_API int mtrssm_mmtrssm_rollout_bwd_wide(const MtrssmMmtrssmDims* d, const MtrssmMmtrssmBwdWeights* w, const MtrssmMmtrssmBwdIO* io, int32_t pieces,
                                               void* workspace, int64_t workspace_bytes, void* stream) {
  if (!g_expert_logw_ok(io, "mmtrssm_rollout_bwd_wide")) return MTRSSM_EINVAL;
  return mmtrssm_wide_bwd_launch(d, w, io, pieces, workspace, workspace_bytes < 0 ? 0 : (size_t)workspace_bytes, static_cast<hipStream_t>(stream));
}
MTRSSM_API int mtrssm_gemm(const MtrssmGemm* g, void* stream) { return gemm_launch(g, static_cast<hipStream_t>(stream)); }
MTRSSM_API int mtrssm_gemm_group(const MtrssmGemm* problems, int32_t count, void* stream) {
  return gemm_group_launch(problems, count, static_cast<hipStream_t>(stream));
}
MTRSSM_API int mtrssm_clear(void* p, int64_t bytes, void* stream) {
  return clear_async(p, bytes < 0 ? 0 : (size_t)bytes, static_cast<hipStream_t>(stream));
}
MTRSSM_API int mtrssm_adamw_prepare(const float* grad, int64_t n, float* sumsq, float* state, const int32_t* status, float beta1, float beta2,
                                    void* stream) {
  return adamw_prepare_launch(grad, n, sumsq, state, status, beta1, beta2, static_cast<hipStream_t>(stream));
}
MTRSSM_API int mtrssm_adamw_apply(float* param, const float* grad, float* exp_avg, float* exp_avg_sq, const uint8_t* active, int64_t n,
                                  const float* sumsq, const float* state, const int32_t* status, float clip_norm, float grad_scale, float beta1,
                                  float beta2, float eps, float weight_decay, void* stream) {
  return adamw_apply_launch(param, grad, exp_avg, exp_avg_sq, active, n, sumsq, state, status, clip_norm, grad_scale, beta1, beta2, eps,
                            weight_decay, static_cast<hipStream_t>(stream));
}
MTRSSM_API int mtrssm_conv_gather_gemm(const MtrssmConvGeom* g, const float* src, const float* src2, const float* wp, const uint16_t* wq,
                                       const float* bias, const float* actgrad_in, const float* add_in, float* out, void* stream) {
  return conv_gather_gemm_launch(g, src, src2, wp, wq, bias, actgrad_in, add_in, out, static_cast<hipStream_t>(stream));
}
MTRSSM_API int mtrssm_episode_gather(const float* store, const int64_t* idx, const float* noise, int64_t n_episodes, int64_t B, int64_t T,
                                     int64_t Tfull, int64_t E, float std_, float* input, float* target, void* stream) {
  return episode_gather_launch(store, idx, noise, n_episodes, B, T, Tfull, E, std_, input, target, static_cast<hipStream_t>(stream));
}
MTRSSM_API int mtrssm_episode_gather_window(const float* store, const int64_t* idx, const int32_t* start, const float* noise, int64_t n_episodes,
                                            int64_t B, int64_t T, int64_t Tfull, int64_t E, float std_, float* input, float* target, void* stream) {
  return episode_gather_window_launch(store, idx, start, noise, n_episodes, B, T, Tfull, E, std_, input, target, static_cast<hipStream_t>(stream));
}
MTRSSM_API int mtrssm_state_select(const MtrssmStateTable* table, const uint8_t* reset, int64_t B, void* stream) {
  return state_select_launch(table, reset, B, static_cast<hipStream_t>(stream));
}
MTRSSM_API int mtrssm_state_save(const MtrssmStateTable* table, int64_t B, int64_t steps, void* stream) {
  return state_save_launch(table, B, steps, static_cast<hipStream_t>(stream));
}
MTRSSM_API int mtrssm_state_save_at(const MtrssmStateTable* table, const int32_t* last, int64_t B, int64_t steps, void* stream) {
  return state_save_at_launch(table, last, B, steps, static_cast<hipStream_t>(stream));
}
MTRSSM_API int mtrssm_episode_gather_ragged(const float* store, const int64_t* idx, const int32_t* start, const int32_t* lengths,
                                            const float* noise, int64_t n_episodes, int64_t B, int64_t T, int64_t Tfull, int64_t E, float std_,
                                            float* input, float* target, int32_t* valid_out, void* stream) {
  return episode_gather_ragged_launch(store, idx, start, lengths, noise, n_episodes, B, T, Tfull, E, std_, input, target, valid_out,
                                      static_cast<hipStream_t>(stream));
}
MTRSSM_API int mtrssm_episode_gather_seeded(const float* store, const int64_t* idx, const int32_t* start, const int32_t* lengths,
                                            int32_t* valid_out, uint32_t key0, uint32_t key1, uint32_t epoch, int64_t n_episodes, int64_t B,
                                            int64_t T, int64_t Tfull, int64_t E, float std_, float* input, float* target, void* stream) {
  return episode_gather_seeded_launch(store, idx, start, lengths, valid_out, key0, key1, epoch, n_episodes, B, T, Tfull, E, std_, input, target,
                                      static_cast<hipStream_t>(stream));
}
MTRSSM_API int mtrssm_step_mask_ragged(const int32_t* valid, const float* u, int64_t b_global, int64_t steps, int64_t span, float p_audio,
                                       float p_vision, int64_t row0, int64_t b_local, int32_t* codes, float* present_audio,
                                       float* present_vision, float* live, uint8_t* mask0, int32_t* last, float* counts, void* stream) {
  return step_mask_ragged_launch(valid, u, b_global, steps, span, p_audio, p_vision, row0, b_local, codes, present_audio, present_vision, live,
                                 mask0, last, counts, static_cast<hipStream_t>(stream));
}
MTRSSM_API int mtrssm_step_mask_forecast(const int32_t* valid, const float* u_mask, const float* u_context, int64_t b_global, int64_t steps,
                                         int64_t span, float p_audio, float p_vision, int64_t lo, int64_t hi, int64_t row0, int64_t b_local,
                                         int32_t* codes, float* seen_audio, float* seen_vision, float* target, float* observed, uint8_t* mask0,
                                         int32_t* last, float* counts, void* stream) {
  return step_mask_forecast_launch(valid, u_mask, u_context, b_global, steps, span, p_audio, p_vision, lo, hi, row0, b_local, codes, seen_audio,
                                   seen_vision, target, observed, mask0, last, counts, static_cast<hipStream_t>(stream));
}
MTRSSM_API int mtrssm_elbo_schedule_fwd(const float* nll_a, const float* nll_v, const float* kl0, const float* kl1, const float* live,
                                       const float* count, const float* step, int64_t n, MtrssmElboSchedule p, float* o_recon, float* o_k0,
                                       float* o_k1, float* o_loss, float* o_beta, float* o_stats, void* stream) {
  return elbo_schedule_fwd_launch(nll_a, nll_v, kl0, kl1, live, count, step, n, p, o_recon, o_k0, o_k1, o_loss, o_beta, o_stats,
                                  static_cast<hipStream_t>(stream));
}
MTRSSM_API int mtrssm_elbo_schedule_bwd(const float* g_recon, const float* g_k0, const float* g_k1, const float* g_loss, const float* kl0,
                                       const float* kl1, const float* live, const float* count, const float* beta, int64_t n,
                                       MtrssmElboSchedule p, float* g_nll_a, float* g_nll_v, float* g_kl0, float* g_kl1, void* stream) {
  return elbo_schedule_bwd_launch(g_recon, g_k0, g_k1, g_loss, kl0, kl1, live, count, beta, n, p, g_nll_a, g_nll_v, g_kl0, g_kl1,
                                  static_cast<hipStream_t>(stream));
}
MTRSSM_API int mtrssm_elbo_combine_counted_fwd(const float* nll_a, const float* nll_v, const float* kl0, const float* kl1, const float* live,
                                               const float* count, int64_t n, float c0, float c1, float* o_recon, float* o_k0, float* o_k1,
                                               float* o_loss, void* stream) {
  return elbo_combine_counted_fwd_launch(nll_a, nll_v, kl0, kl1, live, count, n, c0, c1, o_recon, o_k0, o_k1, o_loss,
                                         static_cast<hipStream_t>(stream));
}
MTRSSM_API int mtrssm_elbo_combine_counted_bwd(const float* g_recon, const float* g_k0, const float* g_k1, const float* g_loss, const float* live,
                                               const float* count, int64_t n, float c0, float c1, float* g_nll_a, float* g_nll_v, float* g_kl0,
                                               float* g_kl1, void* stream) {
  return elbo_combine_counted_bwd_launch(g_recon, g_k0, g_k1, g_loss, live, count, n, c0, c1, g_nll_a, g_nll_v, g_kl0, g_kl1,
                                         static_cast<hipStream_t>(stream));
}
// ... 123 lines not shown
```

### multimodal_mtrssm_amd/csrc/train_ops.hip

```cpp
#include "scan_common.h"

namespace mtrssm {

void set_error(const char* fmt, ...);
void set_last_kernel(const char* name);

constexpr int kThreads = 256;

__device__ __forceinline__ float block_sum(float v, float* red) {
  v = wave_sum(v);
  const int lane = threadIdx.x & (kWave - 1), wave = threadIdx.x / kWave;
  if (lane == 0) red[wave] = v;
  __syncthreads();
  float t = 0.f;
  if (threadIdx.x < kWave) {
    t = threadIdx.x < blockDim.x / kWave ? red[threadIdx.x] : 0.f;
    t = wave_sum(t);
  }
  return t;
}

template <bool TANH>
__global__ void nll_fwd_kernel(const float* __restrict__ pred, const float* __restrict__ target, int64_t n,
                               float scale, float constant, float* __restrict__ out) {
  __shared__ float red[kThreads / kWave];
  const int64_t n4 = n / 4;
  const float4* p4 = reinterpret_cast<const float4*>(pred);
  const float4* t4 = reinterpret_cast<const float4*>(target);
  float acc = 0.f;
  auto term = [](float4 p, const float4 t) {
    if (TANH) { p.x = tanh_fast(p.x); p.y = tanh_fast(p.y); p.z = tanh_fast(p.z); p.w = tanh_fast(p.w); }
    const float a = t.x - p.x, b = t.y - p.y, c = t.z - p.z, d = t.w - p.w;
    return 0.5f * (a * a) + 0.5f * (b * b) + 0.5f * (c * c) + 0.5f * (d * d);
  };
  const int64_t stride = (int64_t)gridDim.x * blockDim.x;
  int64_t i = (int64_t)blockIdx.x * blockDim.x + threadIdx.x;
  for (; i + 3 * stride < n4; i += 4 * stride) {
    const float4 pa = p4[i], pb = p4[i + stride], pc = p4[i + 2 * stride], pd = p4[i + 3 * stride];
    const float4 ta = t4[i], tb = t4[i + stride], tc = t4[i + 2 * stride], td = t4[i + 3 * stride];
    acc += (term(pa, ta) + term(pb, tb)) + (term(pc, tc) + term(pd, td));
  }
  for (; i < n4; i += stride) acc += term(p4[i], t4[i]);
  if (blockIdx.x == 0) {
    for (int64_t i = n4 * 4 + threadIdx.x; i < n; i += blockDim.x) {
      const float a = target[i] - (TANH ? tanh_fast(pred[i]) : pred[i]);
      acc += 0.5f * a * a;
    }
  }
  const float tot = block_sum(acc, red);
  if (threadIdx.x == 0) atomicAdd(out, tot * scale + (blockIdx.x == 0 ? constant : 0.f));
}

template <bool TANH>
__global__ void nll_bwd_kernel(const float* __restrict__ pred, const float* __restrict__ target,
                               const float* __restrict__ g_out, int64_t n, float inv_frames, float* __restrict__ g_pred) {
  const float g = g_out[0] * inv_frames;
  const int64_t n4 = n / 4;
  const float4* p4 = reinterpret_cast<const float4*>(pred);
  const float4* t4 = reinterpret_cast<const float4*>(target);
  float4* o4 = reinterpret_cast<float4*>(g_pred);
  for (int64_t i = (int64_t)blockIdx.x * blockDim.x + threadIdx.x; i < n4; i += (int64_t)gridDim.x * blockDim.x) {
    float4 p = p4[i];
    const float4 t = t4[i];
    float4 d = make_float4(1.f, 1.f, 1.f, 1.f);
    if (TANH) {
      p.x = tanh_fast(p.x); p.y = tanh_fast(p.y); p.z = tanh_fast(p.z); p.w = tanh_fast(p.w);
      d = make_float4(1.f - p.x * p.x, 1.f - p.y * p.y, 1.f - p.z * p.z, 1.f - p.w * p.w);
    }
    o4[i] = make_float4(g * (p.x - t.x) * d.x, g * (p.y - t.y) * d.y, g * (p.z - t.z) * d.z, g * (p.w - t.w) * d.w);
  }
  if (blockIdx.x == 0)
    for (int64_t i = n4 * 4 + threadIdx.x; i < n; i += blockDim.x) {
      const float p = TANH ? tanh_fast(pred[i]) : pred[i];
      g_pred[i] = g * (p - target[i]) * (TANH ? 1.f - p * p : 1.f);
    }
}

__device__ __forceinline__ bool frame_present(const float* __restrict__ present, uint32_t e, uint32_t event) {
  return present[e / event] != 0.f;
}

template <bool EV4>
__device__ __forceinline__ float4 masked_diff(const float* __restrict__ present, uint32_t e0, uint32_t event, float4 t, float4 p) {
// ... 104 lines not shown
    pi -= step * mi / (sqrtf(vi) / bc2_sqrt + eps);
    p[i] = pi;
  }
}

__global__ void sumsq_tick_kernel(const float* __restrict__ x, int64_t n, float* __restrict__ out, float* __restrict__ state,
                                  const int* __restrict__ status, float b1, float b2) {
  __shared__ float red[kThreads / kWave];
  if (blockIdx.x == 0 && threadIdx.x == 0 && state && !(status && *status)) {
    const float step = state[1] + 1.f;
    state[1] = step;
    state[2] = 1.f - powf(b1, step);
    state[3] = sqrtf(1.f - powf(b2, step));
  }
  const int64_t n4 = n / 4;
  const float4* x4 = reinterpret_cast<const float4*>(x);
  float acc = 0.f;
  for (int64_t i = (int64_t)blockIdx.x * blockDim.x + threadIdx.x; i < n4; i += (int64_t)gridDim.x * blockDim.x) {
    const float4 v = x4[i];
    acc += v.x * v.x + v.y * v.y + v.z * v.z + v.w * v.w;
  }
  if (blockIdx.x == 0)
    for (int64_t i = n4 * 4 + threadIdx.x; i < n; i += blockDim.x) acc += x[i] * x[i];
  const float tot = block_sum(acc, red);
  if (threadIdx.x == 0) atomicAdd(out, tot);
}

__global__ void adamw_masked_kernel(float* __restrict__ p, const float* __restrict__ g, float* __restrict__ m, float* __restrict__ v,
                                    const unsigned char* __restrict__ active, int64_t n, const float* __restrict__ sumsq,
                                    const float* __restrict__ state, const int* __restrict__ status, float clip, float gscale, float b1,
                                    float b2, float eps, float wd) {
  if (status && *status) return;
  const float lr = state[0], bc1 = state[2], bc2_sqrt = state[3];
  float coef = gscale;
  if (clip > 0.f && sumsq) {
    const float norm = sqrtf(sumsq[0]) * gscale;
    coef *= fminf(1.f, clip / (norm + 1e-6f));
  }
  const float step = lr / bc1;
  for (int64_t i = (int64_t)blockIdx.x * blockDim.x + threadIdx.x; i < n; i += (int64_t)gridDim.x * blockDim.x) {
    if (active && !active[i]) continue;
    const float gi = g[i] * coef;
    float pi = p[i] * (1.f - lr * wd);
    const float mi = b1 * m[i] + (1.f - b1) * gi;
    const float vi = b2 * v[i] + (1.f - b2) * gi * gi;
    m[i] = mi;
    v[i] = vi;
    pi -= step * mi / (sqrtf(vi) / bc2_sqrt + eps);
    p[i] = pi;
  }
}

__global__ void clear_words_kernel(unsigned* __restrict__ p, size_t n) {
  for (size_t i = (size_t)blockIdx.x * blockDim.x + threadIdx.x; i < n; i += (size_t)gridDim.x * blockDim.x) p[i] = 0u;
}

int clear_async(void* p, size_t bytes, hipStream_t stream) {
  if (!p || (bytes & 3) || ((uintptr_t)p & 3)) { set_error("clear_async: needs a 4-byte aligned buffer of a multiple of 4 bytes"); return MTRSSM_EINVAL; }
  const size_t n = bytes / 4;
  if (n == 0) return MTRSSM_OK;
  const size_t blocks = (n + kThreads - 1) / kThreads;
  hipLaunchKernelGGL(clear_words_kernel, dim3((unsigned)(blocks < 2048 ? blocks : 2048)), dim3(kThreads), 0, stream, static_cast<unsigned*>(p), n);
  return hipGetLastError() == hipSuccess ? MTRSSM_OK : MTRSSM_ELAUNCH;
}

static int grid_for(int64_t n) {
  int64_t g = (n + kThreads - 1) / kThreads;
  return (int)(g < 1 ? 1 : (g > 2048 ? 2048 : g));
}

static int check_launch(const char* what) {
  hipError_t e = hipGetLastError();
  if (e != hipSuccess) {
    set_error("%s launch failed: %s", what, hipGetErrorString(e));
    return MTRSSM_ELAUNCH;
  }
  return MTRSSM_OK;
}

__global__ void categorical_sample_fwd_kernel(const float* __restrict__ logits, const float* __restrict__ u, int64_t n, int C,
                                              float* __restrict__ logp, float* __restrict__ probs, float* __restrict__ onehot) {
  const int64_t i = (int64_t)blockIdx.x * blockDim.x + threadIdx.x;
  if (i >= n) return;
  const float* x = logits + i * C;
  float m = x[0];
  for (int c = 1; c < C; ++c) m = fmaxf(m, x[c]);
  float sum = 0.f;
  for (int c = 0; c < C; ++c) sum += expf(x[c] - m);
  double dsum = 0.0;
  for (int c = 0; c < C; ++c) dsum += exp((double)x[c] - (double)m);
  const double ls = log(dsum);
  const float uu = u[i];
  float acc = 0.f;
  int idx = 0;
  for (int c = 0; c < C; ++c) {
    const float p = expf(x[c] - m) / sum;
    probs[i * C + c] = p;
    logp[i * C + c] = (float)(((double)x[c] - (double)m) - ls);
    acc += p;
    if (c + 1 < C && acc <= uu) ++idx;
  }
  for (int c = 0; c < C; ++c) onehot[i * C + c] = c == idx ? 1.f : 0.f;
}

__global__ void categorical_sample_bwd_kernel(const float* __restrict__ probs, const float* __restrict__ g_p, const float* __restrict__ g_l,
                                              int64_t n, int C, float* __restrict__ d_logits) {
  const int64_t i = (int64_t)blockIdx.x * blockDim.x + threadIdx.x;
  if (i >= n) return;
  float dot = 0.f, sl = 0.f;
  for (int c = 0; c < C; ++c) {
    const float p = probs[i * C + c];
    if (g_p) dot += p * g_p[i * C + c];
    if (g_l) sl += g_l[i * C + c];
  }
  for (int c = 0; c < C; ++c) {
    const float p = probs[i * C + c];
    float d = 0.f;
    if (g_p) d += p * (g_p[i * C + c] - dot);
    if (g_l) d += g_l[i * C + c] - p * sl;
    d_logits[i * C + c] = d;
  }
}

int categorical_sample_fwd_launch(const float* logits, const float* u, int64_t rows, int K, int C, float* logp, float* probs, float* onehot,
                                  hipStream_t s) {
  if (!logits || !u || !logp || !probs || !onehot || rows <= 0 || K <= 0 || C <= 0) { set_error("categorical_sample_fwd: bad argument"); return MTRSSM_EINVAL; }
  const int64_t n = rows * K;
  set_last_kernel("mtrssm::categorical_sample_fwd_kernel");
  hipLaunchKernelGGL(categorical_sample_fwd_kernel, dim3((unsigned)((n + kThreads - 1) / kThreads)), dim3(kThreads), 0, s, logits, u, n, C, logp, probs, onehot);
  return check_launch("categorical_sample_fwd");
}

int categorical_sample_bwd_launch(const float* probs, const float* g_p, const float* g_l, int64_t rows, int K, int C, float* d_logits,
                                  hipStream_t s) {
  if (!probs || !d_logits || rows <= 0 || K <= 0 || C <= 0) { set_error("categorical_sample_bwd: bad argument"); return MTRSSM_EINVAL; }
  const int64_t n = rows * K;
  set_last_kernel("mtrssm::categorical_sample_bwd_kernel");
  hipLaunchKernelGGL(categorical_sample_bwd_kernel, dim3((unsigned)((n + kThreads - 1) / kThreads)), dim3(kThreads), 0, s, probs, g_p, g_l, n, C, d_logits);
  return check_launch("categorical_sample_bwd");
}

__global__ void elbo_combine_fwd_kernel(const float* __restrict__ nll_a, const float* __restrict__ nll_v, const float* __restrict__ kl0,
                                        const float* __restrict__ kl1, int64_t n, float c0, float c1, float* __restrict__ o_recon, float* __restrict__ o_k0,
                                        float* __restrict__ o_k1, float* __restrict__ o_loss) {
  __shared__ float red[kThreads / kWave];
  float a0 = 0.f, a1 = 0.f;
  for (int64_t i = threadIdx.x; i < n; i += blockDim.x) {
    a0 += kl0[i];
    if (kl1) a1 += kl1[i];
  }
  const float s0 = block_sum(a0, red);
  __syncthreads();
  const float s1 = block_sum(a1, red);
  if (threadIdx.x == 0) {
    const float recon = nll_a[0] + nll_v[0];
    const float k0 = s0 / (float)n * c0, k1 = kl1 ? s1 / (float)n * c1 : 0.f;
    o_recon[0] = recon; o_k0[0] = k0; if (o_k1) o_k1[0] = k1; o_loss[0] = recon + k0 + k1;
  }
}
__global__ void elbo_combine_bwd_kernel(const float* __restrict__ g_recon, const float* __restrict__ g_k0, const float* __restrict__ g_k1,
                                        const float* __restrict__ g_loss, int64_t n, float c0, float c1, float* __restrict__ g_nll_a,
                                        float* __restrict__ g_nll_v, float* __restrict__ g_kl0, float* __restrict__ g_kl1) {
  const float gl = g_loss ? g_loss[0] : 0.f;
  const float gn = (g_recon ? g_recon[0] : 0.f) + gl;
  const float v0 = ((g_k0 ? g_k0[0] : 0.f) + gl) * c0 / (float)n, v1 = ((g_k1 ? g_k1[0] : 0.f) + gl) * c1 / (float)n;
  const int64_t i = (int64_t)blockIdx.x * blockDim.x + threadIdx.x;
  if (i == 0) { g_nll_a[0] = gn; g_nll_v[0] = gn; }
  if (i < n) {
    g_kl0[i] = v0;
    if (g_kl1) g_kl1[i] = v1;
  }
}
int elbo_combine_fwd_launch(const float* nll_a, const float* nll_v, const float* kl0, const float* kl1, int64_t n, float c0, float c1,
                            float* o_recon, float* o_k0, float* o_k1, float* o_loss, hipStream_t s) {
  if (!nll_a || !nll_v || !kl0 || !o_recon || !o_k0 || !o_loss || n <= 0) { set_error("elbo_combine_fwd: bad argument"); return MTRSSM_EINVAL; }
  set_last_kernel("mtrssm::elbo_combine_fwd_kernel");
  hipLaunchKernelGGL(elbo_combine_fwd_kernel, dim3(1), dim3(kThreads), 0, s, nll_a, nll_v, kl0, kl1, n, c0, c1, o_recon, o_k0, o_k1, o_loss);
  return check_launch("elbo_combine_fwd");
}
int elbo_combine_bwd_launch(const float* g_recon, const float* g_k0, const float* g_k1, const float* g_loss, int64_t n, float c0, float c1,
                            float* g_nll_a, float* g_nll_v, float* g_kl0, float* g_kl1, hipStream_t s) {
  if (!g_nll_a || !g_nll_v || !g_kl0 || n <= 0) { set_error("elbo_combine_bwd: bad argument"); return MTRSSM_EINVAL; }
  set_last_kernel("mtrssm::elbo_combine_bwd_kernel");
  hipLaunchKernelGGL(elbo_combine_bwd_kernel, dim3((unsigned)((n + kThreads - 1) / kThreads)), dim3(kThreads), 0, s, g_recon, g_k0, g_k1, g_loss, n,
                     c0, c1, g_nll_a, g_nll_v, g_kl0, g_kl1);
  return check_launch("elbo_combine_bwd");
}

__global__ void elbo_combine_counted_fwd_kernel(const float* __restrict__ nll_a, const float* __restrict__ nll_v, const float* __restrict__ kl0,
                                                const float* __restrict__ kl1, const float* __restrict__ live, const float* __restrict__ count,
                                                int64_t n, float c0, float c1, float* __restrict__ o_recon, float* __restrict__ o_k0,
                                                float* __restrict__ o_k1, float* __restrict__ o_loss) {
  __shared__ float red[kThreads / kWave];
  float a0 = 0.f, a1 = 0.f;
  for (int64_t i = threadIdx.x; i < n; i += blockDim.x) {
    const bool on = live[i] != 0.f;
    a0 += on ? kl0[i] : 0.f;
    if (kl1) a1 += on ? kl1[i] : 0.f;
  }
  const float s0 = block_sum(a0, red);
  __syncthreads();
  const float s1 = block_sum(a1, red);
  if (threadIdx.x == 0) {
    const float cnt = count[0];
// ... 903 lines not shown
```

### multimodal_mtrssm_amd/linear.py

```python

from __future__ import annotations

import bisect
import ctypes as C
import weakref

import torch
from torch import Tensor

from multimodal_mtrssm_amd import _lib

_SINKS: list = []
SINK_ENABLED = True


def register_sink(flat) -> None:
    _SINKS.append(weakref.ref(flat))


def grad_target(t: Tensor) -> Tensor | None:
    found = grad_target_owner(t)
    return None if found is None else found[0]


# ... 7 lines not shown
        flat = ref()
        if flat is None or flat.param.device != t.device:
            continue
        base = flat.param.data_ptr()
        off = (addr - base) // 4
        if addr < base or off >= flat.numel:
            continue
        i = bisect.bisect_right(flat.offsets, off) - 1
        p = flat.params[i]
        extent = sum((n - 1) * s for n, s in zip(t.shape, t.stride(), strict=True)) + 1 if t.numel() else 0
        if off + extent > flat.offsets[i] + p.numel():
            return None
        flat.mark_touched(i)
        return flat.grad_full.as_strided(t.shape, t.stride(), off), flat
    return None


_TICKETS: dict = {}
_N_TICKETS = 8192


def _ld(t: Tensor) -> int:
    if t.dim() != 2 or t.stride(1) != 1 or t.dtype != torch.float32 or not t.is_cuda:
        msg = f"mtrssm_gemm operands are fp32 GPU matrices with unit column stride, got shape {tuple(t.shape)} stride {t.stride()} {t.dtype} {t.device}"
        raise _lib.MtrssmLibraryError(msg)
    return int(t.stride(0)) if t.shape[0] > 1 else max(int(t.stride(0)), int(t.shape[1]))


import os as _os

SPLIT_PIECES = int(_os.environ.get("MTRSSM_GEMM_PIECES", "2"))
SPLIT_MIN_FLOPS = 5.0e8


def _problem(a: Tensor, b: Tensor, c: Tensor, *, a_rmajor: bool, b_rmajor: bool, bias: Tensor | None = None, zgrad: Tensor | None = None,
             colsum: Tensor | None = None, act_a: int = 0, act_b: int = 0, act_z: int = 0, accumulate: bool = False, split_r: int = 0,
             mfma_split: int | None = None) -> tuple[C.Structure, float, float]:
    m, r = (a.shape[1], a.shape[0]) if a_rmajor else (a.shape[0], a.shape[1])
    n, r2 = (b.shape[1], b.shape[0]) if b_rmajor else (b.shape[0], b.shape[1])
    if r != r2 or tuple(c.shape) != (m, n):
        msg = f"gemm shapes do not agree: a' [{m}, {r}], b' [{n}, {r2}], c {tuple(c.shape)}"
        raise ValueError(msg)
    if bias is not None and bias.numel() != n or colsum is not None and colsum.numel() != m or zgrad is not None and tuple(zgrad.shape) != (m, n):
        msg = "gemm: bias must have N entries, colsum M entries, zgrad the shape of c"
        raise ValueError(msg)
    g = _lib.Gemm()
    g.A, g.B, g.C = _lib.raw_ptr(a), _lib.raw_ptr(b), _lib.raw_ptr(c)
    g.bias, g.zgrad, g.colsum = _lib.raw_ptr(bias), _lib.raw_ptr(zgrad), _lib.raw_ptr(colsum)
    g.M, g.N, g.R = m, n, r
    g.lda, g.ldb, g.ldc = _ld(a), _ld(b), _ld(c)
    g.ldz = _ld(zgrad) if zgrad is not None else 0
    g.a_rmajor, g.b_rmajor = int(a_rmajor), int(b_rmajor)
    g.act_a, g.act_b, g.act_out, g.act_z = int(act_a), int(act_b), 0, int(act_z)
    g.accumulate, g.split_r = int(accumulate), int(split_r)
    if mfma_split is None:
        mfma_split = SPLIT_PIECES if 2.0 * m * n * r >= SPLIT_MIN_FLOPS else 0
    g.mfma_split = int(mfma_split)
    if zgrad is not None and not accumulate:
        tk = _TICKETS.get(a.device)
        if tk is None:
            tk = _TICKETS[a.device] = torch.zeros(_N_TICKETS, device=a.device, dtype=torch.int32)
        g.tickets, g.n_tickets = tk.data_ptr(), _N_TICKETS
    for t in (bias, colsum):
        if t is not None and (t.dtype != torch.float32 or not t.is_contiguous()):
            msg = "gemm: bias / colsum must be contiguous fp32 vectors"
            raise _lib.MtrssmLibraryError(msg)
    return g, 2.0 * m * n * r, 4.0 * (m * r + n * r + m * n)


def gemm(a: Tensor, b: Tensor, c: Tensor, **kw) -> None:
    g, flops, nbytes = _problem(a, b, c, **kw)
    lib = _lib.load()
    _lib.check(_lib.TIMERS.call("mtrssm_gemm", lib.mtrssm_gemm, C.byref(g), _lib.stream_ptr(a.device), flops=flops, nbytes=nbytes), "mtrssm_gemm")


GROUP_GEMMS = True


def _span(t: Tensor) -> tuple[int, int]:
    lo = t.data_ptr()
    return lo, lo + 4 * (sum((n - 1) * st for n, st in zip(t.shape, t.stride(), strict=True)) + 1 if t.numel() else 0)


def _rounds(problems: list) -> list[list]:
    rounds: list[tuple[list, list]] = []
    for problem in problems:
        (_a, _b, c), kw = problem
        spans = [_span(c)] + ([_span(kw["colsum"])] if kw.get("colsum") is not None else [])
        for members, taken in rounds:
            if all(hi <= lo2 or hi2 <= lo for lo, hi in spans for lo2, hi2 in taken):
                members.append(problem)
                taken.extend(spans)
                break
        else:
            rounds.append(([problem], list(spans)))
    return [members for members, _ in rounds]


def gemm_group(problems: list[tuple[tuple[Tensor, Tensor, Tensor], dict]]) -> None:
    if not problems:
        return
    if not GROUP_GEMMS or len(problems) == 1:
        for (a, b, c), kw in problems:
            gemm(a, b, c, **kw)
        return
    rounds = _rounds(problems)
    if len(rounds) > 1:
        for members in rounds:
            gemm_group(members)
        return
    built = [_problem(a, b, c, **{**kw, "mfma_split": 0}) for (a, b, c), kw in problems]
    arr = (_lib.Gemm * len(built))(*[g for g, _, _ in built])
    dev = problems[0][0][0].device
    lib = _lib.load()
    _lib.check(_lib.TIMERS.call("mtrssm_gemm_group", lib.mtrssm_gemm_group, arr, len(built), _lib.stream_ptr(dev),
                                flops=sum(f for _, f, _ in built), nbytes=sum(n for _, _, n in built)), "mtrssm_gemm_group")


class _DeferredWeightGrads:

    def __init__(self) -> None:
        self.pending: list = []
        self.armed = False

    def add(self, problem: tuple) -> bool:
        if not self.armed:
            try:
                torch.autograd.Variable._execution_engine.queue_callback(self.flush)
            except RuntimeError:
                return False
            self.armed = True
        self.pending.append(problem)
        return True

    def flush(self) -> None:
        self.armed = False
        problems, self.pending = self.pending, []
        small = [p for p in problems if 2.0 * p[0][0].numel() * p[0][1].shape[1] < GROUP_MAX_FLOPS]
        big = [p for p in problems if 2.0 * p[0][0].numel() * p[0][1].shape[1] >= GROUP_MAX_FLOPS]
        gemm_group(small)
        for (a, b, c), kw in big:
            gemm(a, b, c, **kw)

    def discard(self) -> None:
        self.armed = False
        self.pending = []


DEFER_WEIGHT_GRADS = True
GROUP_MAX_FLOPS = 1.0e9
_DEFERRED = _DeferredWeightGrads()


def flush_deferred() -> None:
    if _DEFERRED.pending:
        _DEFERRED.flush()


def discard_deferred() -> None:
    _DEFERRED.discard()


def _pick(pieces: int | None, m: int, n: int, r: int) -> int | None:
    return None if pieces is None else (int(pieces) if 2.0 * m * n * r >= SPLIT_MIN_FLOPS else 0)


def weight_grad(gy: Tensor, x: Tensor, weight: Tensor, bias: Tensor | None, *, act_x: int = 0, want_weight: bool = True,
                want_bias: bool = True, pieces: int | None = None) -> tuple[Tensor | None, Tensor | None]:
    gw_ret = gb_ret = None
    if want_weight:
        gw = grad_target(weight)
        if gw is None:
            gw = gw_ret = torch.zeros(weight.shape, device=gy.device, dtype=torch.float32)
    gb = None
    if bias is not None and want_bias:
        gb = grad_target(bias)
        if gb is None:
            gb = gb_ret = torch.zeros(bias.shape, device=gy.device, dtype=torch.float32)
    if want_weight:
        problem = ((gy, x, gw), dict(a_rmajor=True, b_rmajor=True, act_b=act_x, colsum=gb, accumulate=True,
                                     mfma_split=_pick(pieces, gy.shape[1], x.shape[1], gy.shape[0])))
        sunk = gw_ret is None and gb_ret is None
        if not (DEFER_WEIGHT_GRADS and sunk and _DEFERRED.add(problem)):
            gemm(gy, x, gw, **problem[1])
    elif gb is not None:
        gb.add_(gy.sum(0))
    return gw_ret, gb_ret


class _Linear(torch.autograd.Function):
    @staticmethod
    def forward(ctx, x: Tensor, weight: Tensor, bias: Tensor | None, pre_act: int, pieces: int | None) -> Tensor:
        lead = x.shape[:-1]
        x2 = x.reshape(-1, x.shape[-1])
        if x2.stride(1) != 1:
            x2 = x2.contiguous()
        w = weight if weight.stride(1) == 1 else weight.contiguous()
        y = torch.empty(x2.shape[0], w.shape[0], device=x.device, dtype=torch.float32)
        gemm(x2, w, y, a_rmajor=False, b_rmajor=False, bias=None if bias is None else bias.contiguous(), act_a=pre_act,
             mfma_split=_pick(pieces, x2.shape[0], w.shape[0], x2.shape[1]))
        ctx.save_for_backward(x2, weight, bias if bias is not None else x2.new_zeros(0))
        ctx.pre_act, ctx.has_bias, ctx.lead, ctx.pieces = pre_act, bias is not None, lead, pieces
        return y.reshape(*lead, w.shape[0])

    @staticmethod
    def backward(ctx, gy: Tensor):
        x2, weight, bias = ctx.saved_tensors
        bias = bias if ctx.has_bias else None
        gy2 = gy.reshape(-1, gy.shape[-1])
        if gy2.stride(1) != 1:
            gy2 = gy2.contiguous()
        gx = None
        if ctx.needs_input_grad[0]:
            w = weight if weight.stride(1) == 1 else weight.contiguous()
            gx = torch.empty_like(x2)
            gemm(gy2, w, gx, a_rmajor=False, b_rmajor=True, zgrad=x2 if ctx.pre_act else None, act_z=ctx.pre_act,
                 mfma_split=_pick(ctx.pieces, gy2.shape[0], x2.shape[1], gy2.shape[1]))
            gx = gx.reshape(*ctx.lead, x2.shape[1])
        gw, gb = weight_grad(gy2, x2, weight, bias, act_x=ctx.pre_act, want_weight=ctx.needs_input_grad[1],
                             want_bias=ctx.has_bias and ctx.needs_input_grad[2], pieces=ctx.pieces)
        return gx, gw, gb, None, None


def linear(x: Tensor, weight: Tensor, bias: Tensor | None = None, *, pre_act: int = 0, pieces: int | None = None) -> Tensor:
    return _Linear.apply(x, weight, bias, int(pre_act), pieces)
```

### multimodal_mtrssm_amd/scan.py

```python

from __future__ import annotations

import ctypes as C
from dataclasses import dataclass

import torch
from torch import Tensor

from multimodal_mtrssm_amd import _lib
from multimodal_mtrssm_amd.distributions import KL_BALANCE_ALPHA
from multimodal_mtrssm_amd import linear as _linear
from multimodal_mtrssm_amd.linear import gemm, gemm_group, grad_target, linear


@dataclass(frozen=True)
class ScanConfig:
    cats: int
    classes: int
    act: int
    balancing: bool = True
    rows_per_block: int = 0
    threads: int = 0

    @property
    def kl_weights(self) -> tuple[float, float]:
        return (1.0 - KL_BALANCE_ALPHA, KL_BALANCE_ALPHA) if self.balancing else (1.0, 1.0)


KERNEL_TIMERS = _lib.TIMERS
DEFER_SCAN_GRADS = True

import os as _os

CLUSTER_SCAN = _os.environ.get("MTRSSM_SCAN_CLUSTER", "1") != "0"
WIDE_SCAN = _os.environ.get("MTRSSM_SCAN_WIDE", "1") != "0"
WIDE_BWD = _os.environ.get("MTRSSM_SCAN_WIDE_BWD", "1") != "0"
WIDE_PIECES = int(_os.environ.get("MTRSSM_WIDE_PIECES", "2"))
_WS: dict[tuple, Tensor] = {}
_WS_RETIRED: list[Tensor] = []


def _workspace(device: torch.device, nbytes: int) -> Tensor:
    key = (torch.device(device).index or 0, _lib.stream_ptr(device))
    ws = _WS.get(key)
    if ws is None or ws.numel() * 8 < nbytes:
        new = torch.zeros((nbytes + 7) // 8 + 32, device=device, dtype=torch.int64)
        if ws is not None:
            new[:2].copy_(ws[:2])
            _WS_RETIRED.append(ws)
        ws = _WS[key] = new
        STATUS.watch(key, ws)
    return ws


def status_word(device: torch.device) -> Tensor | None:
    ws = _WS.get((torch.device(device).index or 0, _lib.stream_ptr(device)))
    return None if ws is None else ws[:1].view(torch.int32)[:1]


class StatusMonitor:

    def __init__(self) -> None:
        self._words: dict[tuple, Tensor] = {}
        self._pending: list[tuple[tuple, Tensor, object]] = []

    def watch(self, key: tuple, ws: Tensor) -> None:
        self._words[key] = ws

    @staticmethod
    def _raise(key: tuple, code: int) -> None:
        msg = (f"cooperative scan kernel (workspace {key}): an exchange between workgroups timed out (status {code}); the results of "
               "that step are invalid and the optimizer skipped its update.  The GPU was probably shared, partitioned or CU-masked: "
               "set MTRSSM_SCAN_CLUSTER=0 MTRSSM_SCAN_WIDE=0")
        raise _lib.MtrssmLibraryError(msg)

    def post(self) -> None:
        for key, ws in self._words.items():
            word = ws[:1].view(torch.int32)[:1]
            if word.is_cuda:
                host = torch.empty(1, dtype=torch.int32, pin_memory=True)
                host.copy_(word, non_blocking=True)
                ev = torch.cuda.Event()
                ev.record(torch.cuda.current_stream(word.device))
            else:
                host, ev = word.clone(), None
            self._pending.append((key, host, ev))

    def poll(self) -> None:
        keep = []
        for key, host, ev in self._pending:
            if ev is not None and not ev.query():
                keep.append((key, host, ev))
                continue
            code = int(host[0])
            if code:
# ... 39 lines not shown
class _WeightGrads:

    def __init__(self) -> None:
        self.own: dict[int, Tensor] = {}
        self.pending: list = []

    def _target(self, w: Tensor, rows: slice | None, cols: slice | None) -> tuple[Tensor, bool]:
        view = w
        if rows is not None:
            view = view[rows]
        if cols is not None:
            view = view[:, cols]
        tgt = grad_target(view)
        if tgt is not None:
            return tgt, True
        full = self.own.get(id(w))
        if full is None:
            full = self.own[id(w)] = torch.zeros_like(w)
        out = full
        if rows is not None:
            out = out[rows]
        if cols is not None:
            out = out[:, cols]
        return out, False

    def add(self, gy: Tensor, x: Tensor, w: Tensor, *, cols: slice | None = None, bias: Tensor | None = None) -> None:
        target, sunk = self._target(w, None, cols)
        colsum = None
        if bias is not None:
            colsum, bias_sunk = self._target(bias, None, None)
            sunk = sunk and bias_sunk
        self.pending.append((((gy, x, target), dict(a_rmajor=True, b_rmajor=True, colsum=colsum, accumulate=True)), sunk))

    def flush(self) -> None:
        now = [problem for problem, sunk in self.pending if not (DEFER_SCAN_GRADS and sunk and _linear._DEFERRED.add(problem))]
        gemm_group(now)
        self.pending = []

    def result(self, w: Tensor) -> Tensor | None:
        if self.pending:
            self.flush()
        return self.own.get(id(w))


def _modality(modality: Tensor | None, B: int, T: int) -> Tensor | None:
    if modality is None:
        return None
    if modality.dtype != torch.int32 or tuple(modality.shape) != (B, T):
        msg = f"modality codes must be int32 [{B}, {T}], got {modality.dtype} {tuple(modality.shape)}"
        raise ValueError(msg)
    return _c(modality)


def check_expert_logw(expert_logw: Tensor | None, B: int, T: int) -> Tensor | None:
    if expert_logw is None:
        return None
    if expert_logw.dtype != torch.float32 or tuple(expert_logw.shape) != (B, T, 3):
        msg = f"expert log-weights must be float32 [{B}, {T}, 3], got {expert_logw.dtype} {tuple(expert_logw.shape)}"
        raise ValueError(msg)
    return _c(expert_logw)


def _weighted_modality(modality: Tensor | None, expert_logw: Tensor | None) -> Tensor | None:
    if modality is None and expert_logw is not None:
        return torch.full(expert_logw.shape[:2], 3, device=expert_logw.device, dtype=torch.int32)
    return modality


def modality_codes(mask: Tensor) -> Tensor:
    return (mask[..., 0].to(torch.int32) + 2 * mask[..., 1].to(torch.int32)).contiguous()


def _projection(embed: Tensor | None, layer, deter: int, like: Tensor) -> Tensor:
    if embed is None:
        return like.new_zeros(*like.shape[:-1], layer.weight.shape[0])
    return linear(embed, layer.weight[:, deter:], layer.bias)


def _expect(**named: tuple[Tensor | None, tuple[int, ...]]) -> None:
    for name, (t, shape) in named.items():
        if t is not None and tuple(t.shape) != tuple(shape):
            msg = f"{name}: expected shape {tuple(shape)}, got {tuple(t.shape)}"
            raise ValueError(msg)


class _MrssmScan(torch.autograd.Function):

    @staticmethod
    def forward(
        ctx, cfg: ScanConfig, xa, pa, pv, deter0, stoch0, u_post, u_prior,
        w1, w2, b2, wih, bih, whh, bhh, w3, b3, w4, b4, wa1, wa2, ba2, wv1, wv2, bv2, modality=None,
        expert_logw=None,
    ):
        ctx.set_materialize_grads(False)
        lib = _lib.load()
        B, T, H = xa.shape
        D = deter0.shape[1]
        S = cfg.cats * cfg.classes
        A = w1.shape[1] - S
        K = cfg.cats
        _expect(pa=(pa, (B, T, H)), pv=(pv, (B, T, H)), deter0=(deter0, (B, D)), stoch0=(stoch0, (B, S)),
                u_post=(u_post, (B, T, K)), u_prior=(u_prior, (B, T, K)), w1=(w1, (H, A + S)), w2=(w2, (H, H)), b2=(b2, (H,)),
                wih=(wih, (3 * D, H)), bih=(bih, (3 * D,)), whh=(whh, (3 * D, D)), bhh=(bhh, (3 * D,)), w3=(w3, (H, D)),
                b3=(b3, (H,)), w4=(w4, (S, H)), b4=(b4, (S,)), wa2=(wa2, (S, H)), ba2=(ba2, (S,)), wv2=(wv2, (S, H)),
                bv2=(bv2, (S,)), wa1_rows=(wa1[:, :1], (H, 1)), wv1_rows=(wv1[:, :1], (H, 1)))
        if A < 0 or wa1.shape[1] <= D or wv1.shape[1] <= D:
            msg = "weight shapes are inconsistent with (deter, stoch, action, embed)"
            raise ValueError(msg)
        xa, pa, pv, deter0, stoch0, u_post = map(_c, (xa, pa, pv, deter0, stoch0, u_post))
        expert_logw = check_expert_logw(expert_logw, B, T)
        modality = _weighted_modality(_modality(modality, B, T), expert_logw)
        u_prior = _opt(u_prior)
        w1s_t = _c(w1[:, A:].t())
        wh1 = torch.cat([w3, wa1[:, :D], wv1[:, :D]], dim=0)
        whh_t, wh1_t = _c(whh.t()), _c(wh1.t())
        deter = _new(xa, B, T, D)
        prior_logits, post_logits, post_stoch = (_new(xa, B, T, S) for _ in range(3))
        prior_stoch = _new(xa, B, T, S) if u_prior is not None else None
        kl = _new(xa, B, T)
        need_grad = any(ctx.needs_input_grad)
        sv = dict(sv_h1=None, sv_h2=None, sv_gates=None, sv_heads=None, sv_la=None, sv_lv=None)
        if need_grad:
            sv = dict(sv_h1=_new(xa, B, T, H), sv_h2=_new(xa, B, T, H), sv_gates=_new(xa, B, T, 4 * D),
                      sv_heads=_new(xa, B, T, 3 * H), sv_la=_new(xa, B, T, S), sv_lv=_new(xa, B, T, S))
        io = _lib.fill(
            _lib.MrssmFwdIO(), xa=xa, pa=pa, pv=pv, deter0=deter0, stoch0=stoch0, u_post=u_post, u_prior=u_prior,
            deter=deter, prior_logits=prior_logits, prior_stoch=prior_stoch, post_logits=post_logits, post_stoch=post_stoch,
            kl=kl, **sv, modality=modality, expert_logw=expert_logw,
        )
        wp, wq = cfg.kl_weights
        dims = _lib.MrssmDims(B, T, D, H, cfg.cats, cfg.classes, cfg.act, 1, wp, wq, cfg.rows_per_block, cfg.threads)
        per_bt = 3 * H + 2 * K + D + 3 * S + 1 + (2 * H + 4 * D + 3 * H + 2 * S if need_grad else 0)
        macs = S * H + H * H + 3 * D * H + 3 * D * D + 3 * H * D + 3 * S * H
        plain = cfg.rows_per_block == 0 and cfg.threads == 0
        cluster = CLUSTER_SCAN and plain and bool(lib.mtrssm_mrssm_cluster_supported(C.byref(dims)))
        wide = WIDE_SCAN and plain and not cluster and bool(lib.mtrssm_mrssm_wide_supported(C.byref(dims), WIDE_PIECES))
        ctx.scan_kind = "cluster" if cluster else ("wide" if wide else None)
        if cluster or wide:
            wf_t = _new(xa, H, 3 * D)
            gemm(w2, wih, wf_t, a_rmajor=True, b_rmajor=False)
            bf = _new(xa, 1, 3 * D)
            gemm(b2.reshape(1, H), wih, bf, a_rmajor=False, b_rmajor=False, bias=_c(bih))
            cw = _lib.fill(_lib.MrssmClusterWeights(), w1s_t=w1s_t, wf_t=wf_t, bf=bf.reshape(-1), whh_t=whh_t, bhh=_c(bhh),
                           wh1_t=wh1_t, b3=_c(b3), w4=_c(w4), b4=_c(b4), wa2=_c(wa2), ba2=_c(ba2), wv2=_c(wv2), bv2=_c(bv2))
            io.sv_h2 = None
            stream = _lib.stream_ptr(xa.device)
            if cluster:
                ws = _workspace(xa.device, int(lib.mtrssm_mrssm_cluster_workspace_bytes(C.byref(dims))))
                _lib.check(_lib.TIMERS.call("mtrssm_mrssm_rollout_fwd_cluster", lib.mtrssm_mrssm_rollout_fwd_cluster, C.byref(dims), C.byref(cw),
                                            C.byref(io), _lib.raw_ptr(ws), ws.numel() * 8, stream,
                                            flops=2.0 * B * T * macs, nbytes=4.0 * B * T * per_bt), "mtrssm_mrssm_rollout_fwd_cluster")
            else:
                ws = _workspace(xa.device, int(lib.mtrssm_mrssm_wide_workspace_bytes(C.byref(dims), WIDE_PIECES)))
                _lib.check(_lib.TIMERS.call("mtrssm_mrssm_rollout_fwd_wide", lib.mtrssm_mrssm_rollout_fwd_wide, C.byref(dims), C.byref(cw),
                                            C.byref(io), WIDE_PIECES, _lib.raw_ptr(ws), ws.numel() * 8, stream,
                                            flops=2.0 * B * T * macs, nbytes=4.0 * B * T * per_bt), "mtrssm_mrssm_rollout_fwd_wide")
            sv["sv_h2"] = None
            ctx.cluster_w = (wf_t, whh_t, wh1_t)
        else:
            ctx.cluster_w = None
            fw = _lib.fill(
                _lib.MrssmFwdWeights(), w1s_t=w1s_t, w2_t=_c(w2.t()), b2=_c(b2), wih_t=_c(wih.t()), bih=_c(bih), whh_t=whh_t,
                bhh=_c(bhh), wh1_t=wh1_t, b3=_c(b3), w4=_c(w4), b4=_c(b4), wa2=_c(wa2), ba2=_c(ba2), wv2=_c(wv2), bv2=_c(bv2),
            )
            _lib.check(_lib.TIMERS.call("mtrssm_mrssm_rollout_fwd", lib.mtrssm_mrssm_rollout_fwd, C.byref(dims), C.byref(fw), C.byref(io),
                                        _lib.stream_ptr(xa.device), flops=2.0 * B * T * macs, nbytes=4.0 * B * T * per_bt),
                       "mtrssm_mrssm_rollout_fwd")
        if need_grad:
            ctx.cfg, ctx.A, ctx.modality, ctx.expert_logw = cfg, A, modality, expert_logw
            ctx.biases, ctx.w3 = (b2, bih, bhh, b3, b4, ba2, bv2), w3
            ctx.save_for_backward(deter0, stoch0, deter, prior_logits, post_logits, post_stoch, sv["sv_h1"], sv["sv_h2"],
                                  sv["sv_gates"], sv["sv_heads"], sv["sv_la"], sv["sv_lv"], w1s_t, wh1,
                                  w1, w2, wih, whh, w4, wa1, wa2, wv1, wv2)
        ctx.has_prior_stoch = prior_stoch is not None
        outs = (deter, prior_logits, post_logits, post_stoch, prior_stoch if prior_stoch is not None else deter.new_empty(()), kl)
        return outs

    @staticmethod
    def backward(ctx, g_deter, g_prior_logits, g_post_logits, g_post_stoch, g_prior_stoch, g_kl):
        lib = _lib.load()
        (deter0, stoch0, deter, prior_logits, post_logits, post_stoch, sv_h1, sv_h2, sv_gates, sv_heads, sv_la, sv_lv,
         w1s_t, wh1, w1, w2, wih, whh, w4, wa1, wa2, wv1, wv2) = ctx.saved_tensors
        cfg, A = ctx.cfg, ctx.A
        B, T, D = deter.shape
        H = sv_h1.shape[-1]
        S = cfg.cats * cfg.classes
        if not ctx.has_prior_stoch:
            g_prior_stoch = None
        _expect(g_deter=(g_deter, (B, T, D)), g_prior_logits=(g_prior_logits, (B, T, S)), g_post_logits=(g_post_logits, (B, T, S)),
                g_post_stoch=(g_post_stoch, (B, T, S)), g_prior_stoch=(g_prior_stoch, (B, T, S)), g_kl=(g_kl, (B, T)))
        bw = _lib.fill(_lib.MrssmBwdWeights(), w1s_t=w1s_t, w2=_c(w2), wih=_c(wih), whh=_c(whh), wh1=wh1, w4=_c(w4), wa2=_c(wa2),
                       wv2=_c(wv2))
        g_deter0, g_stoch0 = _new(deter, B, D), _new(deter, B, S)
        d_z1, d_h2 = _new(deter, B, T, H), _new(deter, B, T, H)
        d_gi, d_gh = _new(deter, B, T, 3 * D), _new(deter, B, T, 3 * D)
        d_zh = _new(deter, B, T, 3 * H)
        d_lp, d_la, d_lv = (_new(deter, B, T, S) for _ in range(3))
        g_logw = _new(deter, B, T, 3) if ctx.expert_logw is not None and ctx.needs_input_grad[-1] else None
        io = _lib.fill(
            _lib.MrssmBwdIO(), deter0=deter0, deter=deter, prior_logits=prior_logits, post_logits=post_logits, sv_h1=sv_h1,
            sv_h2=sv_h2, sv_gates=sv_gates, sv_heads=sv_heads, sv_la=sv_la, sv_lv=sv_lv,
            g_deter=_opt(g_deter), g_post_stoch=_opt(g_post_stoch), g_prior_stoch=_opt(g_prior_stoch),
            g_post_logits=_opt(g_post_logits), g_prior_logits=_opt(g_prior_logits), g_kl=_opt(g_kl),
            g_deter0=g_deter0, g_stoch0=g_stoch0, d_z1=d_z1, d_h2=d_h2, d_gi=d_gi, d_gh=d_gh, d_zh=d_zh, d_lp=d_lp, d_la=d_la,
            d_lv=d_lv, modality=ctx.modality, expert_logw=ctx.expert_logw, g_expert_logw=g_logw,
        )
        wp, wq = cfg.kl_weights
        dims = _lib.MrssmDims(B, T, D, H, cfg.cats, cfg.classes, cfg.act, 1, wp, wq, cfg.rows_per_block, cfg.threads)
        per_bt = (2 * H + 4 * D + 3 * H + 2 * S) + D + 2 * S + (D + S + 1) + 2 * H + 6 * D + 3 * H + 3 * S
        macs = S * H + H * H + 3 * D * H + 3 * D * D + 3 * H * D + 3 * S * H
        cw3 = getattr(ctx, "cluster_w", None)
        kind = getattr(ctx, "scan_kind", None)
        use_cluster = kind == "cluster" and CLUSTER_SCAN and cfg.classes * cfg.cats <= 32
        use_wide = kind == "wide" and WIDE_SCAN and WIDE_BWD
        if cw3 is not None and (use_cluster or use_wide):
            wf_t, whh_t, wh1_t = cw3
            cw = _lib.fill(_lib.MrssmClusterWeights(), w1s_t=w1s_t, wf_t=wf_t, whh_t=whh_t, wh1_t=wh1_t, w4=_c(w4), wa2=_c(wa2), wv2=_c(wv2))
            stream = _lib.stream_ptr(deter.device)
            if use_cluster:
                ws = _workspace(deter.device, int(lib.mtrssm_mrssm_cluster_bwd_workspace_bytes(C.byref(dims))))
                _lib.check(_lib.TIMERS.call("mtrssm_mrssm_rollout_bwd_cluster", lib.mtrssm_mrssm_rollout_bwd_cluster, C.byref(dims), C.byref(cw),
                                            C.byref(io), _lib.raw_ptr(ws), ws.numel() * 8, stream,
                                            flops=2.0 * B * T * macs, nbytes=4.0 * B * T * per_bt), "mtrssm_mrssm_rollout_bwd_cluster")
            else:
                ws = _workspace(deter.device, int(lib.mtrssm_mrssm_wide_bwd_workspace_bytes(C.byref(dims), WIDE_PIECES)))
                _lib.check(_lib.TIMERS.call("mtrssm_mrssm_rollout_bwd_wide", lib.mtrssm_mrssm_rollout_bwd_wide, C.byref(dims), C.byref(cw),
                                            C.byref(io), WIDE_PIECES, _lib.raw_ptr(ws), ws.numel() * 8, stream,
                                            flops=2.0 * B * T * macs, nbytes=4.0 * B * T * per_bt), "mtrssm_mrssm_rollout_bwd_wide")
            gemm(_flat2(d_gi), wih, _flat2(d_h2), a_rmajor=False, b_rmajor=True)
        else:
            _lib.check(_lib.TIMERS.call("mtrssm_mrssm_rollout_bwd", lib.mtrssm_mrssm_rollout_bwd, C.byref(dims), C.byref(bw), C.byref(io),
                                        _lib.stream_ptr(deter.device), flops=2.0 * B * T * macs, nbytes=4.0 * B * T * per_bt),
                       "mtrssm_mrssm_rollout_bwd")

        prev_stoch = _flat2(torch.cat([stoch0.unsqueeze(1), post_stoch[:, :-1]], dim=1))
        prev_deter = _flat2(torch.cat([deter0.unsqueeze(1), deter[:, :-1]], dim=1))
        fz1, fh2, fgi, fgh, fzh = map(_flat2, (d_z1, d_h2, d_gi, d_gh, d_zh))
        flp, fla, flv = map(_flat2, (d_lp, d_la, d_lv))
        (b2, bih, bhh, b3, b4, ba2, bv2) = ctx.biases
        if sv_h2 is None:
            sv_h2 = _new(deter, B, T, H)
            gemm(_flat2(sv_h1), w2, _flat2(sv_h2), a_rmajor=False, b_rmajor=False, bias=_c(b2))
        fdet, fh1, fsh2, fheads = map(_flat2, (deter, sv_h1, sv_h2, sv_heads))
        wg = _WeightGrads()
        wg.add(fz1, prev_stoch, w1, cols=slice(A, None))
        wg.add(fh2, fh1, w2, bias=b2)
        wg.add(fgi, fsh2, wih, bias=bih)
        wg.add(fgh, prev_deter, whh, bias=bhh)
        w3 = ctx.w3
        wg.add(fzh[:, :H], fdet, w3, bias=b3)
        wg.add(fzh[:, H : 2 * H], fdet, wa1, cols=slice(0, D))
        wg.add(fzh[:, 2 * H :], fdet, wv1, cols=slice(0, D))
        wg.add(flp, fheads[:, :H], w4, bias=b4)
        wg.add(fla, fheads[:, H : 2 * H], wa2, bias=ba2)
        wg.add(flv, fheads[:, 2 * H :], wv2, bias=bv2)
        g_pa, g_pv = d_zh[..., H : 2 * H], d_zh[..., 2 * H :]
        r = wg.result
        return (None, d_z1, g_pa, g_pv, g_deter0, g_stoch0, None, None,
                r(w1), r(w2), r(b2), r(wih), r(bih), r(whh), r(bhh), r(w3), r(b3), r(w4), r(b4), r(wa1), r(wa2), r(ba2), r(wv1), r(wv2),
                r(bv2), None, g_logw)


def mrssm_posterior_rollout(
    transition, audio_rep, vision_rep, actions: Tensor, audio_embed: Tensor, vision_embed: Tensor,
    deter0: Tensor, stoch0: Tensor, u_post: Tensor, u_prior: Tensor | None, *, balancing: bool, rows_per_block: int = 0,
    threads: int = 0, modality: Tensor | None = None, expert_logw: Tensor | None = None,
) -> dict[str, Tensor]:
    factory = transition.distribution_factory
    K, Cc = factory.category_size, factory.class_size
    D = transition.deterministic_size
    A = actions.shape[-1]
    l1, l2 = transition.action_state_projector.two_layer()
    p1, p2 = transition.rnn_to_prior_projector.two_layer()
    a1, a2 = audio_rep.rnn_to_post_projector.two_layer()
    v1, v2 = vision_rep.rnn_to_post_projector.two_layer()
    act_names = {transition.action_state_projector.activation_name, transition.rnn_to_prior_projector.activation_name,
                 audio_rep.rnn_to_post_projector.activation_name, vision_rep.rnn_to_post_projector.activation_name}
    if len(act_names) != 1:
        msg = f"the HIP scan uses one activation for all heads, got {sorted(act_names)}"
        raise NotImplementedError(msg)
    cfg = ScanConfig(K, Cc, _lib.ACT_IDS[act_names.pop()], balancing, rows_per_block, threads)
    xa = linear(actions, l1.weight[:, :A], l1.bias)
    pa = _projection(audio_embed, a1, D, xa)
    pv = _projection(vision_embed, v1, D, xa)
    cell = transition.rnn_cell
    deter, prior_logits, post_logits, post_stoch, prior_stoch, kl = _MrssmScan.apply(
        cfg, xa, pa, pv, deter0, stoch0, u_post, u_prior,
        l1.weight, l2.weight, l2.bias, cell.weight_ih, cell.bias_ih, cell.weight_hh, cell.bias_hh,
        p1.weight, p1.bias, p2.weight, p2.bias, a1.weight, a2.weight, a2.bias, v1.weight, v2.weight, v2.bias, modality, expert_logw,
    )
    return {"deter": deter, "prior_logits": prior_logits, "post_logits": post_logits, "post_stoch": post_stoch,
            "prior_stoch": prior_stoch if u_prior is not None else None, "kl": kl}


def _st_sample(logits: Tensor, cats: int, classes: int, u: Tensor) -> tuple[Tensor, Tensor]:
    from multimodal_mtrssm_amd.distributions import onehot_from_uniforms

    probs = torch.softmax(logits.reshape(*logits.shape[:-1], cats, classes), dim=-1)
    onehot = onehot_from_uniforms(probs.detach(), u)
    return (onehot + (probs - probs.detach())).flatten(start_dim=-2), probs


def _mrssm_prior_rollout_differentiable(transition, actions: Tensor, deter0: Tensor, stoch0: Tensor,
                                        u_prior: Tensor | None) -> dict[str, Tensor]:
    factory = transition.distribution_factory
    cats, classes = factory.category_size, factory.class_size
    B, T, _ = actions.shape
    cell = transition.rnn_cell
    if u_prior is None:
        u_prior = torch.rand(B, T, cats, device=actions.device)
    actions, deter, stoch, u_prior = actions.float(), deter0.float(), stoch0.float(), u_prior.float()
    deters, logits_all, stochs = [], [], []
    for t in range(T):
        x = transition.action_state_projector(_c(torch.cat([actions[:, t], stoch], dim=-1)))
        gi = linear(x, cell.weight_ih, cell.bias_ih)
        gh = linear(_c(deter), cell.weight_hh, cell.bias_hh)
        i_r, i_z, i_n = gi.chunk(3, dim=-1)
        h_r, h_z, h_n = gh.chunk(3, dim=-1)
        r, z = torch.sigmoid(i_r + h_r), torch.sigmoid(i_z + h_z)
        deter = (1.0 - z) * torch.tanh(i_n + r * h_n) + z * deter
        logits = transition.rnn_to_prior_projector(_c(deter))
        stoch, _ = _st_sample(logits, cats, classes, u_prior[:, t])
        deters.append(deter)
        logits_all.append(logits)
        stochs.append(stoch)
    return {"deter": torch.stack(deters, 1), "prior_logits": torch.stack(logits_all, 1), "prior_stoch": torch.stack(stochs, 1)}


def mrssm_prior_rollout(transition, actions: Tensor, deter0: Tensor, stoch0: Tensor, u_prior: Tensor | None,
                        *, rows_per_block: int = 0, threads: int = 0) -> dict[str, Tensor]:
    lib = _lib.load()
    if torch.is_grad_enabled() and (actions.requires_grad or deter0.requires_grad or stoch0.requires_grad
                                    or any(p.requires_grad for p in transition.parameters())):
        return _mrssm_prior_rollout_differentiable(transition, actions, deter0, stoch0, u_prior)
    with torch.no_grad():
        factory = transition.distribution_factory
        K, Cc = factory.category_size, factory.class_size
        S = K * Cc
        B, T, A = actions.shape
        D, H = transition.deterministic_size, transition.hidden_size
        l1, l2 = transition.action_state_projector.two_layer()
        p1, p2 = transition.rnn_to_prior_projector.two_layer()
        cell = transition.rnn_cell
        if u_prior is None:
            u_prior = torch.rand(B, T, K, device=actions.device)
        xa = _c(linear(actions, l1.weight[:, :A], l1.bias))
        tensors = dict(w1s_t=_c(l1.weight[:, A:].t()), w2_t=_c(l2.weight.t()), b2=_c(l2.bias), wih_t=_c(cell.weight_ih.t()),
                       bih=_c(cell.bias_ih), whh_t=_c(cell.weight_hh.t()), bhh=_c(cell.bias_hh), wh1_t=_c(p1.weight.t()),
                       b3=_c(p1.bias), w4=_c(p2.weight), b4=_c(p2.bias))
        fw = _lib.fill(_lib.MrssmFwdWeights(), **tensors)
        deter, prior_logits, prior_stoch = _new(xa, B, T, D), _new(xa, B, T, S), _new(xa, B, T, S)
        deter0, stoch0, u_prior = _c(deter0.float()), _c(stoch0.float()), _c(u_prior.float())
        _expect(deter0=(deter0, (B, D)), stoch0=(stoch0, (B, S)), u_prior=(u_prior, (B, T, K)), xa=(xa, (B, T, H)),
                w1=(l1.weight, (H, A + S)), wih=(cell.weight_ih, (3 * D, H)), whh=(cell.weight_hh, (3 * D, D)),
                w3=(p1.weight, (H, D)), w4=(p2.weight, (S, H)))
        io = _lib.fill(_lib.MrssmFwdIO(), xa=xa, deter0=deter0, stoch0=stoch0, u_prior=u_prior, deter=deter,
                       prior_logits=prior_logits, prior_stoch=prior_stoch)
        act = _lib.ACT_IDS[transition.action_state_projector.activation_name]
        dims = _lib.MrssmDims(B, T, D, H, K, Cc, act, 0, 1.0, 1.0, rows_per_block, threads)
        _lib.check(lib.mtrssm_mrssm_rollout_fwd(C.byref(dims), C.byref(fw), C.byref(io), _lib.stream_ptr(xa.device)),
                   "mtrssm_mrssm_rollout_fwd(prior-only)")
        del tensors
    return {"deter": deter, "prior_logits": prior_logits, "prior_stoch": prior_stoch}


@dataclass(frozen=True)
class MTScanConfig:
# ... 313 lines not shown
```

Baseline: 377,700 seq-steps/s.

## Fuse initial-state MLPs, scan weight prep, and group small linears

```diff
diff --git a/include/mtrssm.h b/include/mtrssm.h
--- a/include/mtrssm.h
+++ b/include/mtrssm.h
@@ -158,6 +158,63 @@
 
 int mtrssm_mrssm_rollout_bwd(const MtrssmMrssmDims* dims, const MtrssmMrssmBwdWeights* w,
                              const MtrssmMrssmBwdIO* io, void* stream);
+
+typedef struct MtrssmInitialState {
+  const float* ea;
+  const float* ev;
+  int64_t ea_stride, ev_stride;
+  const uint8_t* mask0;
+  const float* u;
+  const float* wi1;
+  const float* bi1;
+  const float* wi2;
+  const float* bi2;
+  const float* wp1;
+  const float* bp1;
+  const float* wp2;
+  const float* bp2;
+  int32_t ld_wi1, ld_wi2, ld_wp1, ld_wp2;
+  int32_t B, E, cells, D, H, K, C, act_i, act_p, depth_i, depth_p;
+  float* e;
+  float* z1;
+  float* deter0;
+  float* zp;
+  float* logp;
+  float* probs;
+  float* stoch;
+  const float* g_deter0;
+  const float* g_stoch0;
+  const float* g_logp;
+  const float* g_probs;
+  float* d_logits;
+  float* d_zp;
+  float* g_deter;
+  float* d_z1;
+  float* g_ea;
+  float* g_ev;
+} MtrssmInitialState;
+int mtrssm_initial_state_supported(const MtrssmInitialState* p);
+int mtrssm_initial_state_fwd(const MtrssmInitialState* p, void* stream);
+int mtrssm_initial_state_bwd(const MtrssmInitialState* p, void* stream);
+
+typedef struct MtrssmScanPrepare {
+  const float* w1;
+  const float* w2;
+  const float* b2;
+  const float* wih;
+  const float* bih;
+  const float* whh;
+  const float* w3;
+  const float* wa1;
+  const float* wv1;
+  int32_t ld_w1, ld_w2, ld_wih, ld_whh, ld_w3, ld_wa1, ld_wv1;
+  int32_t D, H, S, A;
+  int32_t product;
+  float* out;
+  int64_t out_floats;
+} MtrssmScanPrepare;
+int64_t mtrssm_mrssm_scan_prepare_layout(int32_t D, int32_t H, int32_t S, int64_t* offsets);
+int mtrssm_mrssm_scan_prepare(const MtrssmScanPrepare* p, void* stream);
 
 typedef struct MtrssmMmtrssmDims {
   int32_t B, T;
diff --git a/multimodal_mtrssm_amd/_lib.py b/multimodal_mtrssm_amd/_lib.py
--- a/multimodal_mtrssm_amd/_lib.py
+++ b/multimodal_mtrssm_amd/_lib.py
@@ -43,6 +43,16 @@
     "deter0", "deter", "prior_logits", "post_logits", "sv_h1", "sv_h2", "sv_gates", "sv_heads", "sv_la", "sv_lv",
     "g_deter", "g_post_stoch", "g_prior_stoch", "g_post_logits", "g_prior_logits", "g_kl",
     "g_deter0", "g_stoch0", "d_z1", "d_h2", "d_gi", "d_gh", "d_zh", "d_lp", "d_la", "d_lv", "expert_logw", "g_expert_logw", "modality"))
+
+ScanPrepare = _struct("MtrssmScanPrepare", _ptrs("w1", "w2", "b2", "wih", "bih", "whh", "w3", "wa1", "wv1") + [(n, _i) for n in (
+    "ld_w1", "ld_w2", "ld_wih", "ld_whh", "ld_w3", "ld_wa1", "ld_wv1", "D", "H", "S", "A", "product")]
+    + [("out", _p), ("out_floats", C.c_int64)])
+
+InitialState = _struct("MtrssmInitialState", _ptrs("ea", "ev") + [("ea_stride", C.c_int64), ("ev_stride", C.c_int64)] + _ptrs(
+    "mask0", "u", "wi1", "bi1", "wi2", "bi2", "wp1", "bp1", "wp2", "bp2") + [(n, _i) for n in (
+    "ld_wi1", "ld_wi2", "ld_wp1", "ld_wp2", "B", "E", "cells", "D", "H", "K", "C", "act_i", "act_p", "depth_i", "depth_p")] + _ptrs(
+    "e", "z1", "deter0", "zp", "logp", "probs", "stoch", "g_deter0", "g_stoch0", "g_logp", "g_probs",
+    "d_logits", "d_zp", "g_deter", "d_z1", "g_ea", "g_ev"))
 
 MmtrssmDims = _struct("MtrssmMmtrssmDims", [
     ("B", _i), ("T", _i), ("LD", _i), ("HD", _i), ("H", _i), ("KL", _i), ("CL", _i), ("KH", _i), ("CH", _i),
@@ -99,6 +109,11 @@
     "mtrssm_mrssm_rollout_fwd_wide": (C.c_int, [C.POINTER(MrssmDims), C.POINTER(MrssmClusterWeights), C.POINTER(MrssmFwdIO), _i, _p, C.c_int64, _p]),
     "mtrssm_mrssm_rollout_bwd_wide": (C.c_int, [C.POINTER(MrssmDims), C.POINTER(MrssmClusterWeights), C.POINTER(MrssmBwdIO), _i, _p, C.c_int64, _p]),
     "mtrssm_mrssm_rollout_bwd": (C.c_int, [C.POINTER(MrssmDims), C.POINTER(MrssmBwdWeights), C.POINTER(MrssmBwdIO), _p]),
+    "mtrssm_initial_state_supported": (C.c_int, [C.POINTER(InitialState)]),
+    "mtrssm_initial_state_fwd": (C.c_int, [C.POINTER(InitialState), _p]),
+    "mtrssm_initial_state_bwd": (C.c_int, [C.POINTER(InitialState), _p]),
+    "mtrssm_mrssm_scan_prepare_layout": (C.c_int64, [_i, _i, _i, C.POINTER(C.c_int64)]),
+    "mtrssm_mrssm_scan_prepare": (C.c_int, [C.POINTER(ScanPrepare), _p]),
     "mtrssm_mmtrssm_rollout_fwd": (C.c_int, [C.POINTER(MmtrssmDims), C.POINTER(MmtrssmFwdWeights), C.POINTER(MmtrssmFwdIO), _p]),
     "mtrssm_mmtrssm_rollout_bwd": (C.c_int, [C.POINTER(MmtrssmDims), C.POINTER(MmtrssmBwdWeights), C.POINTER(MmtrssmBwdIO), _p]),
     "mtrssm_mmtrssm_wide_supported": (C.c_int, [C.POINTER(MmtrssmDims), _i]),
diff --git a/multimodal_mtrssm_amd/cnn.py b/multimodal_mtrssm_amd/cnn.py
--- a/multimodal_mtrssm_amd/cnn.py
+++ b/multimodal_mtrssm_amd/cnn.py
@@ -7,7 +7,7 @@
 from torch import Tensor, nn
 
 from multimodal_mtrssm_amd import _lib
-from multimodal_mtrssm_amd.linear import linear
+from multimodal_mtrssm_amd.linear import SPLIT_MIN_FLOPS, linear, linear_group
 from multimodal_mtrssm_amd.conv import (
     gemm_pieces,
     conv2d,
@@ -96,7 +96,12 @@
 
 def decode_pair(dec_a: "Decoder", dec_b: "Decoder", fa: Tensor, fb: Tensor, *, raw: bool = False) -> tuple[Tensor, Tensor]:
     lead_a, lead_b = fa.shape[:-1], fb.shape[:-1]
-    xa, xb = dec_a.stem(fa), dec_b.stem(fb)
+    first_a = first_b = None
+    if len(dec_a.linears) > 0 and len(dec_b.linears) > 0 and all(
+            2.0 * f.numel() * d.linears[0].weight.shape[0] < SPLIT_MIN_FLOPS for f, d in ((fa, dec_a), (fb, dec_b))):
+        first_a, first_b = linear_group([(f.reshape(-1, f.shape[-1]), d.linears[0].weight, d.linears[0].bias, 0)
+                                         for f, d in ((fa, dec_a), (fb, dec_b))])
+    xa, xb = dec_a.stem(fa, first_a), dec_b.stem(fb, first_b)
     xa, xb = _res_pair(dec_a.res, dec_b.res, xa, xb)
     if len(dec_a.deconvs) != len(dec_b.deconvs) or (len(dec_a.res) > 0) != (len(dec_b.res) > 0):
         return dec_a.tail(xa, lead_a, raw=raw), dec_b.tail(xb, lead_b, raw=raw)
@@ -229,12 +234,15 @@
         name = type(self.out_act).__name__
         return {"Identity": 0, "Tanh": 3}.get(name)
 
-    def stem(self, f: Tensor) -> Tensor:
+    def stem(self, f: Tensor, first: Tensor | None = None) -> Tensor:
         if len(self.linears) == 0:
             self.materialize(f.shape[-1])
             self.to(f.device)
         x = f.reshape(-1, f.shape[-1])
         for i, lin in enumerate(self.linears):
+            if i == 0 and first is not None:
+                x = first
+                continue
             x = linear(x, lin.weight, lin.bias, pre_act=self.act_id if i > 0 else 0, pieces=gemm_pieces())
         return x.reshape(-1, *self.conv_in_shape)
 
diff --git a/multimodal_mtrssm_amd/core.py b/multimodal_mtrssm_amd/core.py
--- a/multimodal_mtrssm_amd/core.py
+++ b/multimodal_mtrssm_amd/core.py
@@ -82,6 +82,99 @@
         _lib.check(_lib.load().mtrssm_categorical_sample_bwd(_lib.ptr(probs), _lib.ptr(gp), _lib.ptr(gl), rows, cats, classes, _lib.ptr(d),
                                                              _lib.stream_ptr(probs.device)), "mtrssm_categorical_sample_bwd")
         return d, None, None, None
+
+
+FUSED_INITIAL_STATE = True
+
+
+def _initial_state_problem(ea, ev, mask0, u, params, acts, depths, cats: int, classes: int):
+    from multimodal_mtrssm_amd import _lib
+
+    ref = ea if ea is not None else ev
+    if ref is None or any(p is None for p in params) or any(a is None for a in acts):
+        return None
+    tensors = [t for t in (ea, ev, u, *params) if t is not None]
+    if not all(t.is_cuda and t.dtype == torch.float32 for t in tensors) or ref.dim() != 2 or any(t.stride(-1) != 1 for t in tensors):
+        return None
+    if any(e is not None and (e.shape != ref.shape or (e.shape[0] > 1 and e.stride(0) < e.shape[1])) for e in (ea, ev)):
+        return None
+    if mask0 is not None and (mask0.dtype != torch.bool or tuple(mask0.shape) != (ref.shape[0], 2) or not mask0.is_contiguous()):
+        return None
+    wi1, bi1, wi2, bi2, wp1, bp1, wp2, bp2 = params
+    B, E = ref.shape
+    cells, D, H, S = wi1.shape[0], wi2.shape[0], wp1.shape[0], wp2.shape[0]
+    if (wi1.shape[1], wi2.shape[1], wp1.shape[1], wp2.shape[1], S) != (E, cells, D, H, cats * classes):
+        return None
+    if u is not None and (tuple(u.shape) != (B, cats) or not u.is_contiguous()):
+        return None
+    if any(b.shape != (w.shape[0],) or not b.is_contiguous() for w, b in ((wi1, bi1), (wi2, bi2), (wp1, bp1), (wp2, bp2))):
+        return None
+    p = _lib.InitialState()
+    p.ea_stride = 0 if ea is None else max(int(ea.stride(0)), E)
+    p.ev_stride = 0 if ev is None else max(int(ev.stride(0)), E)
+    p.ld_wi1, p.ld_wi2, p.ld_wp1, p.ld_wp2 = (max(int(w.stride(0)), w.shape[1]) for w in (wi1, wi2, wp1, wp2))
+    p.B, p.E, p.cells, p.D, p.H, p.K, p.C = B, E, cells, D, H, cats, classes
+    p.act_i, p.act_p = acts
+    p.depth_i, p.depth_p = depths
+    if not _lib.load().mtrssm_initial_state_supported(p):
+        return None
+    return p
+
+
+class _InitialState(torch.autograd.Function):
+
+    @staticmethod
+    def forward(ctx, problem, mask0, ea, ev, u, wi1, bi1, wi2, bi2, wp1, bp1, wp2, bp2):
+        from multimodal_mtrssm_amd import _lib
+
+        ctx.set_materialize_grads(False)
+        params = (wi1, bi1, wi2, bi2, wp1, bp1, wp2, bp2)
+        p = type(problem).from_buffer_copy(problem)
+        new = lambda *shape: torch.empty(shape, device=u.device, dtype=torch.float32)
+        e, z1, deter0, zp = new(p.B, p.E), new(p.B, p.cells), new(p.B, p.D), new(p.B, p.H)
+        logp, probs, stoch = new(p.B, p.K, p.C), new(p.B, p.K, p.C), new(p.B, p.K * p.C)
+        p.ea, p.ev, p.mask0, p.u = _lib.raw_ptr(ea), _lib.raw_ptr(ev), _lib.raw_ptr(mask0), _lib.ptr(u)
+        p.wi1, p.bi1, p.wi2, p.bi2, p.wp1, p.bp1, p.wp2, p.bp2 = map(_lib.raw_ptr, params)
+        p.e, p.z1, p.deter0, p.zp, p.logp, p.probs, p.stoch = map(_lib.ptr, (e, z1, deter0, zp, logp, probs, stoch))
+        _lib.check(_lib.TIMERS.call("mtrssm_initial_state_fwd", _lib.load().mtrssm_initial_state_fwd, p, _lib.stream_ptr(u.device)),
+                   "mtrssm_initial_state_fwd")
+        ctx.plan, ctx.given, ctx.has_mask = bytes(problem), (ea is not None, ev is not None), mask0 is not None
+        saved = (e, z1, deter0, zp, probs, *params) + ((mask0,) if mask0 is not None else ())
+        ctx.save_for_backward(*saved)
+        ctx.mark_non_differentiable(e)
+        return deter0, stoch, logp, probs, e
+
+    @staticmethod
+    def backward(ctx, g_deter0, g_stoch, g_logp, g_probs, _g_e):
+        from multimodal_mtrssm_amd import _lib
+        from multimodal_mtrssm_amd.linear import weight_grad
+
+        if g_deter0 is None and g_stoch is None and g_logp is None and g_probs is None:
+            return (None,) * 13
+        e, z1, deter0, zp, probs, *rest = ctx.saved_tensors
+        params, mask0 = rest[:8], (rest[8] if ctx.has_mask else None)
+        p = _lib.InitialState.from_buffer_copy(ctx.plan)
+        new = lambda *shape: torch.empty(shape, device=e.device, dtype=torch.float32)
+        gs = [None if g is None else g.contiguous().float() for g in (g_deter0, g_stoch, g_logp, g_probs)]
+        d_logits, d_zp, g_deter, d_z1 = new(p.B, p.K * p.C), new(p.B, p.H), new(p.B, p.D), new(p.B, p.cells)
+        g_ea = new(p.B, p.E) if ctx.needs_input_grad[2] else None
+        g_ev = new(p.B, p.E) if ctx.needs_input_grad[3] else None
+        p.ea, p.ev = (_lib.ptr(e) if given else None for given in ctx.given)
+        p.ea_stride, p.ev_stride = (p.E if given else 0 for given in ctx.given)
+        p.mask0 = _lib.raw_ptr(mask0)
+        p.wi1, p.bi1, p.wi2, p.bi2, p.wp1, p.bp1, p.wp2, p.bp2 = map(_lib.raw_ptr, params)
+        p.z1, p.zp, p.probs = _lib.ptr(z1), _lib.ptr(zp), _lib.ptr(probs)
+        p.g_deter0, p.g_stoch0, p.g_logp, p.g_probs = map(_lib.ptr, gs)
+        p.d_logits, p.d_zp, p.g_deter, p.d_z1, p.g_ea, p.g_ev = map(_lib.ptr, (d_logits, d_zp, g_deter, d_z1, g_ea, g_ev))
+        _lib.check(_lib.TIMERS.call("mtrssm_initial_state_bwd", _lib.load().mtrssm_initial_state_bwd, p, _lib.stream_ptr(e.device)),
+                   "mtrssm_initial_state_bwd")
+        wi1, bi1, wi2, bi2, wp1, bp1, wp2, bp2 = params
+        need = ctx.needs_input_grad
+        grads = []
+        for j, (gy, x, w, b, act) in enumerate(((d_z1, e, wi1, bi1, 0), (g_deter, z1, wi2, bi2, p.act_i), (d_zp, deter0, wp1, bp1, 0),
+                                                (d_logits, zp, wp2, bp2, p.act_p))):
+            grads += weight_grad(gy, x, w, b, act_x=act, want_weight=need[5 + 2 * j], want_bias=need[6 + 2 * j])
+        return (None, None, g_ea, g_ev, None, *grads)
 
 
 class _ElboCombine(torch.autograd.Function):
@@ -445,7 +538,32 @@
             return {"recon/audio": audio, "recon/vision": vision}
         return {"recon": audio + vision, "recon/audio": audio, "recon/vision": vision}
 
+    def _initial_fused(self, ea: Tensor | None, ev: Tensor | None, mask0: Tensor | None, u_init: Tensor | None) -> State | None:
+        from multimodal_mtrssm_amd import _lib
+        from multimodal_mtrssm_amd.networks import MLP
+
+        proj, head = self.init_proj, self.transition.rnn_to_prior_projector
+        ref = ea if ea is not None else ev
+        if not FUSED_INITIAL_STATE or ref is None or not ref.is_cuda or not isinstance(proj, MLP) or not isinstance(head, MLP):
+            return None
+        if len(proj) != 3 or len(head) != 3 or proj.activate_last_layer or head.activate_last_layer:
+            return None
+        factory = self.representation.distribution_factory
+        params = (proj[0].weight, proj[0].bias, proj[2].weight, proj[2].bias, head[0].weight, head[0].bias, head[2].weight, head[2].bias)
+        acts = (_lib.ACT_IDS.get(proj.activation_name), _lib.ACT_IDS.get(head.activation_name))
+        u = None if u_init is None else u_init.to(ref).contiguous()
+        problem = _initial_state_problem(ea, ev, mask0, u, params, acts, (proj.depth, head.depth), factory.category_size, factory.class_size)
+        if problem is None:
+            return None
+        if u is None:
+            u = draw_uniforms((ref.shape[0], factory.category_size), ref).contiguous()
+        deter, stoch, logp, probs, _ = _InitialState.apply(problem, mask0, ea, ev, u, *params)
+        return State(deter=deter, distribution=MultiOneHot(logp, probs), stoch=stoch)
+
     def _initial_from_embed(self, obs_embed: Tensor, u_init: Tensor | None) -> State:
+        fused = self._initial_fused(obs_embed, None, None, u_init) if obs_embed.dim() == 2 else None
+        if fused is not None:
+            return fused
         deter = self.init_proj(obs_embed)
         logits = self.transition.rnn_to_prior_projector(deter)
         dist, stoch = _sampled_head(self.representation.distribution_factory, logits, u_init)
@@ -955,8 +1073,10 @@
         conv.begin_step(audio_obs.device)
         audio_embed, vision_embed = self._encode_both(audio_obs, vision_obs)
         u_init = None if noise is None else noise.get("u_init")
-        state0 = self._initial_from_embed(_masked_mean_embed(audio_embed[:, 0], vision_embed[:, 0], None if sm is None else sm.mask0),
-                                          u_init)
+        mask0 = None if sm is None else sm.mask0
+        state0 = self._initial_fused(audio_embed[:, 0], vision_embed[:, 0], mask0, u_init)
+        if state0 is None:
+            state0 = self._initial_from_embed(_masked_mean_embed(audio_embed[:, 0], vision_embed[:, 0], mask0), u_init)
         state0 = self._state0(state0, carry)
         out = self._rollout_embedded(action_input, audio_embed, vision_embed, state0, noise, sample_prior=False,
                                      modality=None if sm is None else sm.codes, expert_log_weights=expert_log_weights)
diff --git a/multimodal_mtrssm_amd/csrc/capi.hip b/multimodal_mtrssm_amd/csrc/capi.hip
--- a/multimodal_mtrssm_amd/csrc/capi.hip
+++ b/multimodal_mtrssm_amd/csrc/capi.hip
@@ -112,6 +112,11 @@
 size_t mrssm_wide_bwd_workspace_bytes(const MtrssmMrssmDims*, int);
 int mrssm_wide_fwd_launch(const MtrssmMrssmDims*, const MtrssmMrssmClusterWeights*, const MtrssmMrssmFwdIO*, int, void*, size_t, hipStream_t);
 int mrssm_wide_bwd_launch(const MtrssmMrssmDims*, const MtrssmMrssmClusterWeights*, const MtrssmMrssmBwdIO*, int, void*, size_t, hipStream_t);
+int64_t mrssm_scan_prepare_layout(int, int, int, int64_t*);
+int initial_state_supported(const MtrssmInitialState*);
+int initial_state_fwd_launch(const MtrssmInitialState*, hipStream_t);
+int initial_state_bwd_launch(const MtrssmInitialState*, hipStream_t);
+int mrssm_scan_prepare_launch(const MtrssmScanPrepare*, hipStream_t);
 int adamw_prepare_launch(const float*, int64_t, float*, float*, const int*, float, float, hipStream_t);
 int adamw_apply_launch(float*, const float*, float*, float*, const unsigned char*, int64_t, const float*, const float*, const int*, float, float, float,
                        float, float, float, hipStream_t);
@@ -277,6 +282,19 @@
 MTRSSM_API int mtrssm_gemm_group(const MtrssmGemm* problems, int32_t count, void* stream) {
   return gemm_group_launch(problems, count, static_cast<hipStream_t>(stream));
 }
+MTRSSM_API int mtrssm_initial_state_supported(const MtrssmInitialState* p) { return initial_state_supported(p); }
+MTRSSM_API int mtrssm_initial_state_fwd(const MtrssmInitialState* p, void* stream) {
+  return initial_state_fwd_launch(p, static_cast<hipStream_t>(stream));
+}
+MTRSSM_API int mtrssm_initial_state_bwd(const MtrssmInitialState* p, void* stream) {
+  return initial_state_bwd_launch(p, static_cast<hipStream_t>(stream));
+}
+MTRSSM_API int64_t mtrssm_mrssm_scan_prepare_layout(int32_t D, int32_t H, int32_t S, int64_t* offsets) {
+  return mrssm_scan_prepare_layout(D, H, S, offsets);
+}
+MTRSSM_API int mtrssm_mrssm_scan_prepare(const MtrssmScanPrepare* p, void* stream) {
+  return mrssm_scan_prepare_launch(p, static_cast<hipStream_t>(stream));
+}
 MTRSSM_API int mtrssm_clear(void* p, int64_t bytes, void* stream) {
   return clear_async(p, bytes < 0 ? 0 : (size_t)bytes, static_cast<hipStream_t>(stream));
 }
diff --git a/multimodal_mtrssm_amd/csrc/categorical.h b/multimodal_mtrssm_amd/csrc/categorical.h
--- /dev/null
+++ b/multimodal_mtrssm_amd/csrc/categorical.h
@@ -0,0 +1,42 @@
+#pragma once
+#include <hip/hip_runtime.h>
+
+namespace mtrssm {
+
+__device__ __forceinline__ void categorical_sample_one(const float* x, float uu, int C, float* logp, float* probs, float* onehot) {
+  float m = x[0];
+  for (int c = 1; c < C; ++c) m = fmaxf(m, x[c]);
+  float sum = 0.f;
+  for (int c = 0; c < C; ++c) sum += expf(x[c] - m);
+  double dsum = 0.0;
+  for (int c = 0; c < C; ++c) dsum += exp((double)x[c] - (double)m);
+  const double ls = log(dsum);
+  float acc = 0.f;
+  int idx = 0;
+  for (int c = 0; c < C; ++c) {
+    const float p = expf(x[c] - m) / sum;
+    probs[c] = p;
+    logp[c] = (float)(((double)x[c] - (double)m) - ls);
+    acc += p;
+    if (c + 1 < C && acc <= uu) ++idx;
+  }
+  for (int c = 0; c < C; ++c) onehot[c] = c == idx ? 1.f : 0.f;
+}
+
+__device__ __forceinline__ void categorical_grad_one(const float* probs, const float* g_p, const float* g_l, int C, float* d_logits) {
+  float dot = 0.f, sl = 0.f;
+  for (int c = 0; c < C; ++c) {
+    const float p = probs[c];
+    if (g_p) dot += p * g_p[c];
+    if (g_l) sl += g_l[c];
+  }
+  for (int c = 0; c < C; ++c) {
+    const float p = probs[c];
+    float d = 0.f;
+    if (g_p) d += p * (g_p[c] - dot);
+    if (g_l) d += g_l[c] - p * sl;
+    d_logits[c] = d;
+  }
+}
+
+}
diff --git a/multimodal_mtrssm_amd/csrc/init_state.hip b/multimodal_mtrssm_amd/csrc/init_state.hip
--- /dev/null
+++ b/multimodal_mtrssm_amd/csrc/init_state.hip
@@ -0,0 +1,220 @@
+#include "categorical.h"
+#include "scan_common.h"
+
+namespace mtrssm {
+
+void set_error(const char* fmt, ...);
+void set_last_kernel(const char* name);
+
+constexpr int kInitThreads = 1024;
+constexpr int kInitMax = 1024;
+constexpr int kInitRows = 4;
+constexpr int64_t kInitWeightFloats = 512 * 1024;
+
+__device__ __forceinline__ float act_grad_in(float z, int act) {
+  switch (act) {
+    case MTRSSM_ACT_RELU: return z > 0.f ? 1.f : 0.f;
+    case MTRSSM_ACT_ELU: return z > 0.f ? 1.f : expf(z);
+    case MTRSSM_ACT_TANH: { const float t = tanhf(z); return 1.f - t * t; }
+    default: return 1.f;
+  }
+}
+
+template <typename Emit>
+__device__ __forceinline__ void rows_dot(const float* __restrict__ W, int ld, int N, int K, const float* x, const float* __restrict__ bias,
+                                         Emit&& emit) {
+  const int lane = threadIdx.x & (kWave - 1), wave = threadIdx.x / kWave, waves = blockDim.x / kWave;
+  const bool vec = (((uintptr_t)W & 15) == 0) && (ld & 3) == 0 && (K & 3) == 0;
+  for (int n0 = wave * kInitRows; n0 < N; n0 += waves * kInitRows) {
+    float acc[kInitRows];
+    const float* row[kInitRows];
+#pragma unroll
+    for (int i = 0; i < kInitRows; ++i) {
+      acc[i] = 0.f;
+      row[i] = W + (size_t)(n0 + i < N ? n0 + i : N - 1) * ld;
+    }
+    if (vec) {
+      for (int k = lane * 4; k < K; k += kWave * 4) {
+        const float4 xv = *reinterpret_cast<const float4*>(x + k);
+#pragma unroll
+        for (int i = 0; i < kInitRows; ++i) {
+          const float4 w = *reinterpret_cast<const float4*>(row[i] + k);
+          acc[i] = fmaf(w.x, xv.x, acc[i]);
+          acc[i] = fmaf(w.y, xv.y, acc[i]);
+          acc[i] = fmaf(w.z, xv.z, acc[i]);
+          acc[i] = fmaf(w.w, xv.w, acc[i]);
+        }
+      }
+    } else {
+      for (int k = lane; k < K; k += kWave) {
+        const float xv = x[k];
+#pragma unroll
+        for (int i = 0; i < kInitRows; ++i) acc[i] = fmaf(row[i][k], xv, acc[i]);
+      }
+    }
+#pragma unroll
+    for (int i = 0; i < kInitRows; ++i) {
+      const float s = wave_sum(acc[i]);
+      if (lane == 0 && n0 + i < N) emit(n0 + i, s + bias[n0 + i]);
+    }
+  }
+}
+
+template <typename Emit>
+__device__ __forceinline__ void cols_dot(const float* __restrict__ W, int ld, int R, int M, const float* y, float* part, Emit&& emit) {
+  const int tid = threadIdx.x;
+  int P = (int)blockDim.x / M;
+  if (P > R) P = R;
+  const int per = (R + P - 1) / P;
+  const int q = tid / M, m = tid - q * M;
+  if (q < P) {
+    const int r1 = (q + 1) * per < R ? (q + 1) * per : R;
+    float acc = 0.f;
+#pragma unroll 8
+    for (int r = q * per; r < r1; ++r) acc = fmaf(W[(size_t)r * ld + m], y[r], acc);
+    part[q * M + m] = acc;
+  }
+  __syncthreads();
+  if (tid < M) {
+    float s = part[tid];
+    for (int i = 1; i < P; ++i) s += part[i * M + tid];
+    emit(tid, s);
+  }
+}
+
+__device__ __forceinline__ int embed_mode(const MtrssmInitialState& p, int b) {
+  if (!p.ea) return 2;
+  if (!p.ev) return 1;
+  if (!p.mask0) return 0;
+  const bool a = p.mask0[2 * b] != 0, v = p.mask0[2 * b + 1] != 0;
+  return a && v ? 0 : (a ? 1 : 2);
+}
+
+__global__ __launch_bounds__(kInitThreads) void initial_state_fwd_kernel(const MtrssmInitialState p) {
+  __shared__ __attribute__((aligned(16))) float s_e[kInitMax], s_a[kInitMax], s_d[kInitMax], s_p[kInitMax], s_l[kInitMax];
+  const int b = blockIdx.x, tid = threadIdx.x;
+  const int S = p.K * p.C;
+  const int mode = embed_mode(p, b);
+  const float* ea = p.ea ? p.ea + (size_t)b * p.ea_stride : nullptr;
+  const float* ev = p.ev ? p.ev + (size_t)b * p.ev_stride : nullptr;
+  for (int k = tid; k < p.E; k += blockDim.x) {
+    const float v = mode == 0 ? (ea[k] + ev[k]) / 2.f : (mode == 1 ? ea[k] : ev[k]);
+    s_e[k] = v;
+    p.e[(size_t)b * p.E + k] = v;
+  }
+  __syncthreads();
+  rows_dot(p.wi1, p.ld_wi1, p.cells, p.E, s_e, p.bi1, [&](int n, float v) {
+    p.z1[(size_t)b * p.cells + n] = v;
+    s_a[n] = act_fwd(v, p.act_i);
+  });
+  __syncthreads();
+  rows_dot(p.wi2, p.ld_wi2, p.D, p.cells, s_a, p.bi2, [&](int n, float v) {
+    p.deter0[(size_t)b * p.D + n] = v;
+    s_d[n] = v;
+  });
+  __syncthreads();
+  rows_dot(p.wp1, p.ld_wp1, p.H, p.D, s_d, p.bp1, [&](int n, float v) {
+    p.zp[(size_t)b * p.H + n] = v;
+    s_p[n] = act_fwd(v, p.act_p);
+  });
+  __syncthreads();
+  rows_dot(p.wp2, p.ld_wp2, S, p.H, s_p, p.bp2, [&](int n, float v) { s_l[n] = v; });
+  __syncthreads();
+  if (tid < p.K) {
+    const size_t at = ((size_t)b * p.K + tid) * p.C;
+    categorical_sample_one(s_l + tid * p.C, p.u[(size_t)b * p.K + tid], p.C, p.logp + at, p.probs + at, p.stoch + at);
+  }
+}
+
+__global__ __launch_bounds__(kInitThreads) void initial_state_bwd_kernel(const MtrssmInitialState p) {
+  __shared__ __attribute__((aligned(16))) float s_gp[kInitMax], s_gl[kInitMax], s_dl[kInitMax], s_x[kInitMax], s_y[kInitMax], s_part[kInitMax];
+  const int b = blockIdx.x, tid = threadIdx.x;
+  const int S = p.K * p.C;
+  const bool has_gp = p.g_stoch0 || p.g_probs, has_gl = p.g_logp != nullptr;
+  for (int i = tid; i < S; i += blockDim.x) {
+    const size_t at = (size_t)b * S + i;
+    s_gp[i] = (p.g_stoch0 ? p.g_stoch0[at] : 0.f) + (p.g_probs ? p.g_probs[at] : 0.f);
+    s_gl[i] = has_gl ? p.g_logp[at] : 0.f;
+  }
+  __syncthreads();
+  if (tid < p.K)
+    categorical_grad_one(p.probs + ((size_t)b * p.K + tid) * p.C, has_gp ? s_gp + tid * p.C : nullptr, has_gl ? s_gl + tid * p.C : nullptr, p.C,
+                         s_dl + tid * p.C);
+  __syncthreads();
+  for (int i = tid; i < S; i += blockDim.x) p.d_logits[(size_t)b * S + i] = s_dl[i];
+  cols_dot(p.wp2, p.ld_wp2, S, p.H, s_dl, s_part, [&](int m, float s) {
+    const float v = s * act_grad_in(p.zp[(size_t)b * p.H + m], p.act_p);
+    p.d_zp[(size_t)b * p.H + m] = v;
+    s_x[m] = v;
+  });
+  __syncthreads();
+  cols_dot(p.wp1, p.ld_wp1, p.H, p.D, s_x, s_part, [&](int m, float s) {
+    const float v = s + (p.g_deter0 ? p.g_deter0[(size_t)b * p.D + m] : 0.f);
+    p.g_deter[(size_t)b * p.D + m] = v;
+    s_y[m] = v;
+  });
+  __syncthreads();
+  cols_dot(p.wi2, p.ld_wi2, p.D, p.cells, s_y, s_part, [&](int m, float s) {
+    const float v = s * act_grad_in(p.z1[(size_t)b * p.cells + m], p.act_i);
+    p.d_z1[(size_t)b * p.cells + m] = v;
+    s_x[m] = v;
+  });
+  __syncthreads();
+  const int mode = embed_mode(p, b);
+  cols_dot(p.wi1, p.ld_wi1, p.cells, p.E, s_x, s_part, [&](int m, float s) {
+    if (p.g_ea) p.g_ea[(size_t)b * p.E + m] = mode == 0 ? s / 2.f : (mode == 1 ? s : 0.f);
+    if (p.g_ev) p.g_ev[(size_t)b * p.E + m] = mode == 0 ? s / 2.f : (mode == 2 ? s : 0.f);
+  });
+}
+
+static const char* refusal(const MtrssmInitialState* p) {
+  if (!p) return "null argument";
+  if (p->depth_i != 1 || p->depth_p != 1) return "Linear-act-Linear stacks only (depth 1)";
+  for (int a : {p->act_i, p->act_p})
+    if (a < MTRSSM_ACT_IDENTITY || a > MTRSSM_ACT_TANH) return "unknown activation id";
+  if (p->B <= 0 || p->E <= 0 || p->cells <= 0 || p->D <= 0 || p->H <= 0 || p->K <= 0 || p->C <= 0) return "non-positive extent";
+  if (p->E > kInitMax || p->cells > kInitMax || p->D > kInitMax || p->H > kInitMax || p->K > kInitMax || p->C > kInitMax ||
+      (int64_t)p->K * p->C > kInitMax)
+    return "a layer is wider than 1024 (the activations of a layer sit in LDS)";
+  if ((int64_t)p->E * p->cells + (int64_t)p->cells * p->D + (int64_t)p->D * p->H + (int64_t)p->H * p->K * p->C > kInitWeightFloats)
+    return "more than 2 MB of weights (every batch row's workgroup streams them all)";
+  if (p->ld_wi1 < p->E || p->ld_wi2 < p->cells || p->ld_wp1 < p->D || p->ld_wp2 < p->H) return "a leading dimension is smaller than its row";
+  return nullptr;
+}
+
+static bool common_pointers(const MtrssmInitialState* p) {
+  return (p->ea || p->ev) && (!p->ea || p->ea_stride >= p->E) && (!p->ev || p->ev_stride >= p->E) && p->wi1 && p->bi1 && p->wi2 && p->bi2 &&
+         p->wp1 && p->bp1 && p->wp2 && p->bp2;
+}
+
+static int finish(const char* what) {
+  hipError_t e = hipGetLastError();
+  if (e != hipSuccess) { set_error("%s launch failed: %s", what, hipGetErrorString(e)); return MTRSSM_ELAUNCH; }
+  return MTRSSM_OK;
+}
+
+int initial_state_supported(const MtrssmInitialState* p) { return refusal(p) == nullptr ? 1 : 0; }
+
+int initial_state_fwd_launch(const MtrssmInitialState* p, hipStream_t stream) {
+  if (const char* why = refusal(p)) { set_error("initial_state_fwd: %s", why); return MTRSSM_EINVAL; }
+  if (!common_pointers(p) || !p->u || !p->e || !p->z1 || !p->deter0 || !p->zp || !p->logp || !p->probs || !p->stoch) {
+    set_error("initial_state_fwd: null pointer (or an embedding row stride below E)");
+    return MTRSSM_EINVAL;
+  }
+  set_last_kernel("mtrssm::initial_state_fwd_kernel");
+  hipLaunchKernelGGL(initial_state_fwd_kernel, dim3((unsigned)p->B), dim3(kInitThreads), 0, stream, *p);
+  return finish("initial_state_fwd");
+}
+
+int initial_state_bwd_launch(const MtrssmInitialState* p, hipStream_t stream) {
+  if (const char* why = refusal(p)) { set_error("initial_state_bwd: %s", why); return MTRSSM_EINVAL; }
+  if (!common_pointers(p) || !p->z1 || !p->zp || !p->probs || !p->d_logits || !p->d_zp || !p->g_deter || !p->d_z1) {
+    set_error("initial_state_bwd: null pointer (or an embedding row stride below E)");
+    return MTRSSM_EINVAL;
+  }
+  set_last_kernel("mtrssm::initial_state_bwd_kernel");
+  hipLaunchKernelGGL(initial_state_bwd_kernel, dim3((unsigned)p->B), dim3(kInitThreads), 0, stream, *p);
+  return finish("initial_state_bwd");
+}
+
+}
diff --git a/multimodal_mtrssm_amd/csrc/scan_prepare.hip b/multimodal_mtrssm_amd/csrc/scan_prepare.hip
--- /dev/null
+++ b/multimodal_mtrssm_amd/csrc/scan_prepare.hip
@@ -0,0 +1,154 @@
+#include "scan_common.h"
+
+namespace mtrssm {
+
+void set_error(const char* fmt, ...);
+void set_last_kernel(const char* name);
+
+constexpr int kPrepTile = 32;
+constexpr int kPrepChunk = 64;
+constexpr int kPrepThreads = 256;
+constexpr int kPrepSegs = 5;
+constexpr int kPrepAlign = 64;
+
+struct PrepSeg {
+  const float* src;
+  float* dst;
+  int rows, cols, ld_src, ld_dst, col_off, tiles_c;
+};
+
+struct PrepArgs {
+  PrepSeg seg[kPrepSegs];
+  int first[kPrepSegs + 2];
+  const float *w2, *b2, *wih, *bih;
+  float *wf_t, *bf;
+  int H, D3, ld_w2, ld_wih, tiles_j;
+};
+
+__device__ __forceinline__ void transpose_tile(const PrepSeg& s, int tile, float (*t)[kPrepTile + 1]) {
+  const int r0 = (tile / s.tiles_c) * kPrepTile, c0 = (tile % s.tiles_c) * kPrepTile;
+  const int tx = threadIdx.x & (kPrepTile - 1), ty = threadIdx.x / kPrepTile;
+#pragma unroll
+  for (int i = 0; i < kPrepTile; i += kPrepThreads / kPrepTile) {
+    const int r = r0 + ty + i, c = c0 + tx;
+    if (r < s.rows && c < s.cols) t[ty + i][tx] = s.src[(size_t)r * s.ld_src + c];
+  }
+  __syncthreads();
+#pragma unroll
+  for (int i = 0; i < kPrepTile; i += kPrepThreads / kPrepTile) {
+    const int c = c0 + ty + i, r = r0 + tx;
+    if (r < s.rows && c < s.cols) s.dst[(size_t)c * s.ld_dst + s.col_off + r] = t[tx][ty + i];
+  }
+}
+
+__global__ __launch_bounds__(kPrepThreads) void scan_prepare_kernel(const PrepArgs p) {
+  __shared__ float a_s[kPrepChunk][kPrepTile];
+  __shared__ float b_s[kPrepTile][kPrepChunk + 1];
+  const int block = blockIdx.x;
+  if (block < p.first[kPrepSegs]) {
+    int s = 0;
+    while (block >= p.first[s + 1]) ++s;
+    transpose_tile(p.seg[s], block - p.first[s], reinterpret_cast<float(*)[kPrepTile + 1]>(&b_s[0][0]));
+    return;
+  }
+  const int tile = block - p.first[kPrepSegs];
+  const int k0 = (tile / p.tiles_j) * kPrepTile, j0 = (tile % p.tiles_j) * kPrepTile;
+  const int tid = threadIdx.x;
+  const int H = p.H;
+  const int ak = tid & (kPrepTile - 1), ah = tid / kPrepTile;
+  const int bh = tid & (kPrepChunk - 1), bj = tid / kPrepChunk;
+  float ra[8], rb[8];
+  auto load = [&](int h0) {
+#pragma unroll
+    for (int i = 0; i < 8; ++i) {
+      const int h = h0 + ah + 8 * i, k = k0 + ak;
+      float v = 0.f;
+      if (h < H) {
+        if (k < H) v = p.w2[(size_t)h * p.ld_w2 + k];
+        else if (k == H) v = p.b2[h];
+      }
+      ra[i] = v;
+    }
+#pragma unroll
+    for (int i = 0; i < 8; ++i) {
+      const int j = j0 + bj + 4 * i, h = h0 + bh;
+      rb[i] = (j < p.D3 && h < H) ? p.wih[(size_t)j * p.ld_wih + h] : 0.f;
+    }
+  };
+  const int tj = tid & (kPrepTile - 1), tk = tid / kPrepTile;
+  float acc[4] = {0.f, 0.f, 0.f, 0.f};
+  load(0);
+  for (int h0 = 0; h0 < H; h0 += kPrepChunk) {
+#pragma unroll
+    for (int i = 0; i < 8; ++i) a_s[ah + 8 * i][ak] = ra[i];
+#pragma unroll
+    for (int i = 0; i < 8; ++i) b_s[bj + 4 * i][bh] = rb[i];
+    __syncthreads();
+    if (h0 + kPrepChunk < H) load(h0 + kPrepChunk);
+    const int hn = H - h0 < kPrepChunk ? H - h0 : kPrepChunk;
+    for (int h = 0; h < hn; ++h) {
+      const float b = b_s[tj][h];
+#pragma unroll
+      for (int i = 0; i < 4; ++i) acc[i] = fmaf(a_s[h][tk + 8 * i], b, acc[i]);
+    }
+    __syncthreads();
+  }
+  const int j = j0 + tj;
+  if (j >= p.D3) return;
+#pragma unroll
+  for (int i = 0; i < 4; ++i) {
+    const int k = k0 + tk + 8 * i;
+    if (k < H) p.wf_t[(size_t)k * p.D3 + j] = acc[i];
+    else if (k == H) p.bf[j] = acc[i] + p.bih[j];
+  }
+}
+
+static int64_t round_up(int64_t n) { return (n + kPrepAlign - 1) / kPrepAlign * kPrepAlign; }
+
+int64_t mrssm_scan_prepare_layout(int D, int H, int S, int64_t* offsets) {
+  if (D <= 0 || H <= 0 || S <= 0 || D > (1 << 14) || H > (1 << 14) || S > (1 << 14)) return 0;
+  const int64_t sizes[5] = {(int64_t)S * H, (int64_t)D * 3 * D, (int64_t)D * 3 * H, (int64_t)H * 3 * D, (int64_t)3 * D};
+  int64_t at = 0;
+  for (int i = 0; i < 5; ++i) {
+    if (offsets) offsets[i] = at;
+    at += round_up(sizes[i]);
+  }
+  return at;
+}
+
+int mrssm_scan_prepare_launch(const MtrssmScanPrepare* q, hipStream_t stream) {
+  if (!q || !q->w1 || !q->whh || !q->w3 || !q->wa1 || !q->wv1 || !q->out) { set_error("mrssm_scan_prepare: null pointer"); return MTRSSM_EINVAL; }
+  if (q->product && (!q->w2 || !q->b2 || !q->wih || !q->bih)) { set_error("mrssm_scan_prepare: the fused input path needs w2, b2, wih, bih (null)"); return MTRSSM_EINVAL; }
+  int64_t off[5];
+  const int64_t need = mrssm_scan_prepare_layout(q->D, q->H, q->S, off);
+  if (need == 0 || q->A < 0) { set_error("mrssm_scan_prepare: need 0 < D, H, S <= 16384 and A >= 0 (got %d %d %d %d)", q->D, q->H, q->S, q->A); return MTRSSM_EINVAL; }
+  if (q->out_floats < need) { set_error("mrssm_scan_prepare: the buffer holds %lld floats, the layouts take %lld", (long long)q->out_floats, (long long)need); return MTRSSM_EINVAL; }
+  const int D = q->D, H = q->H, S = q->S;
+  if (q->ld_w1 < q->A + S || q->ld_whh < D || q->ld_w3 < D || q->ld_wa1 < D || q->ld_wv1 < D || (q->product && (q->ld_w2 < H || q->ld_wih < H))) {
+    set_error("mrssm_scan_prepare: a leading dimension is smaller than the row it is read along");
+    return MTRSSM_EINVAL;
+  }
+  PrepArgs p;
+  auto tiles = [](int n) { return (n + kPrepTile - 1) / kPrepTile; };
+  auto seg = [&](int i, const float* src, float* dst, int rows, int cols, int ld_src, int ld_dst, int col_off) {
+    p.seg[i] = PrepSeg{src, dst, rows, cols, ld_src, ld_dst, col_off, tiles(cols)};
+    p.first[i + 1] = p.first[i] + tiles(rows) * tiles(cols);
+  };
+  p.first[0] = 0;
+  seg(0, q->w1 + q->A, q->out + off[0], H, S, q->ld_w1, H, 0);
+  seg(1, q->whh, q->out + off[1], 3 * D, D, q->ld_whh, 3 * D, 0);
+  seg(2, q->w3, q->out + off[2], H, D, q->ld_w3, 3 * H, 0);
+  seg(3, q->wa1, q->out + off[2], H, D, q->ld_wa1, 3 * H, H);
+  seg(4, q->wv1, q->out + off[2], H, D, q->ld_wv1, 3 * H, 2 * H);
+  p.w2 = q->w2; p.b2 = q->b2; p.wih = q->wih; p.bih = q->bih;
+  p.wf_t = q->out + off[3]; p.bf = q->out + off[4];
+  p.H = H; p.D3 = 3 * D; p.ld_w2 = q->ld_w2; p.ld_wih = q->ld_wih; p.tiles_j = tiles(3 * D);
+  p.first[kPrepSegs + 1] = p.first[kPrepSegs] + (q->product ? tiles(H + 1) * p.tiles_j : 0);
+  set_last_kernel("mtrssm::scan_prepare_kernel");
+  hipLaunchKernelGGL(scan_prepare_kernel, dim3((unsigned)p.first[kPrepSegs + 1]), dim3(kPrepThreads), 0, stream, p);
+  hipError_t e = hipGetLastError();
+  if (e != hipSuccess) { set_error("mrssm_scan_prepare launch failed: %s", hipGetErrorString(e)); return MTRSSM_ELAUNCH; }
+  return MTRSSM_OK;
+}
+
+}
diff --git a/multimodal_mtrssm_amd/csrc/train_ops.hip b/multimodal_mtrssm_amd/csrc/train_ops.hip
--- a/multimodal_mtrssm_amd/csrc/train_ops.hip
+++ b/multimodal_mtrssm_amd/csrc/train_ops.hip
@@ -1,4 +1,5 @@
 #include "scan_common.h"
+#include "categorical.h"
 
 namespace mtrssm {
 
@@ -269,44 +270,14 @@
                                               float* __restrict__ logp, float* __restrict__ probs, float* __restrict__ onehot) {
   const int64_t i = (int64_t)blockIdx.x * blockDim.x + threadIdx.x;
   if (i >= n) return;
-  const float* x = logits + i * C;
-  float m = x[0];
-  for (int c = 1; c < C; ++c) m = fmaxf(m, x[c]);
-  float sum = 0.f;
-  for (int c = 0; c < C; ++c) sum += expf(x[c] - m);
-  double dsum = 0.0;
-  for (int c = 0; c < C; ++c) dsum += exp((double)x[c] - (double)m);
-  const double ls = log(dsum);
-  const float uu = u[i];
-  float acc = 0.f;
-  int idx = 0;
-  for (int c = 0; c < C; ++c) {
-    const float p = expf(x[c] - m) / sum;
-    probs[i * C + c] = p;
-    logp[i * C + c] = (float)(((double)x[c] - (double)m) - ls);
-    acc += p;
-    if (c + 1 < C && acc <= uu) ++idx;
-  }
-  for (int c = 0; c < C; ++c) onehot[i * C + c] = c == idx ? 1.f : 0.f;
+  categorical_sample_one(logits + i * C, u[i], C, logp + i * C, probs + i * C, onehot + i * C);
 }
 
 __global__ void categorical_sample_bwd_kernel(const float* __restrict__ probs, const float* __restrict__ g_p, const float* __restrict__ g_l,
                                               int64_t n, int C, float* __restrict__ d_logits) {
   const int64_t i = (int64_t)blockIdx.x * blockDim.x + threadIdx.x;
   if (i >= n) return;
-  float dot = 0.f, sl = 0.f;
-  for (int c = 0; c < C; ++c) {
-    const float p = probs[i * C + c];
-    if (g_p) dot += p * g_p[i * C + c];
-    if (g_l) sl += g_l[i * C + c];
-  }
-  for (int c = 0; c < C; ++c) {
-    const float p = probs[i * C + c];
-    float d = 0.f;
-    if (g_p) d += p * (g_p[i * C + c] - dot);
-    if (g_l) d += g_l[i * C + c] - p * sl;
-    d_logits[i * C + c] = d;
-  }
+  categorical_grad_one(probs + i * C, g_p ? g_p + i * C : nullptr, g_l ? g_l + i * C : nullptr, C, d_logits + i * C);
 }
 
 int categorical_sample_fwd_launch(const float* logits, const float* u, int64_t rows, int K, int C, float* logp, float* probs, float* onehot,
diff --git a/multimodal_mtrssm_amd/linear.py b/multimodal_mtrssm_amd/linear.py
--- a/multimodal_mtrssm_amd/linear.py
+++ b/multimodal_mtrssm_amd/linear.py
@@ -113,13 +113,30 @@
     return lo, lo + 4 * (sum((n - 1) * st for n, st in zip(t.shape, t.stride(), strict=True)) + 1 if t.numel() else 0)
 
 
+def _columns(t: Tensor) -> tuple[int, int, int] | None:
+    if t.dim() != 2 or t.stride(1) != 1 or t.shape[0] <= 1 or t.stride(0) < t.shape[1]:
+        return None
+    pitch = int(t.stride(0))
+    return pitch, (t.data_ptr() // 4) % pitch, int(t.shape[1])
+
+
+def _disjoint(s: tuple, t: tuple) -> bool:
+    (lo, hi, cols), (lo2, hi2, cols2) = s, t
+    if hi <= lo2 or hi2 <= lo:
+        return True
+    if cols is None or cols2 is None or cols[0] != cols2[0]:
+        return False
+    pitch = cols[0]
+    return (cols2[1] - cols[1]) % pitch >= cols[2] and (cols[1] - cols2[1]) % pitch >= cols2[2]
+
+
 def _rounds(problems: list) -> list[list]:
     rounds: list[tuple[list, list]] = []
     for problem in problems:
         (_a, _b, c), kw = problem
-        spans = [_span(c)] + ([_span(kw["colsum"])] if kw.get("colsum") is not None else [])
+        spans = [(*_span(c), _columns(c))] + ([(*_span(kw["colsum"]), None)] if kw.get("colsum") is not None else [])
         for members, taken in rounds:
-            if all(hi <= lo2 or hi2 <= lo for lo, hi in spans for lo2, hi2 in taken):
+            if all(_disjoint(s, t) for s in spans for t in taken):
                 members.append(problem)
                 taken.extend(spans)
                 break
@@ -141,6 +158,15 @@
             gemm_group(members)
         return
     built = [_problem(a, b, c, **{**kw, "mfma_split": 0}) for (a, b, c), kw in problems]
+    at = 0
+    for g, _, _ in built:
+        if g.tickets:
+            tiles = ((g.M + 63) // 64) * ((g.N + 63) // 64)
+            if at + tiles <= _N_TICKETS:
+                g.tickets, g.n_tickets = g.tickets + 4 * at, tiles
+                at += tiles
+            else:
+                g.tickets, g.n_tickets = None, 0
     arr = (_lib.Gemm * len(built))(*[g for g, _, _ in built])
     dev = problems[0][0][0].device
     lib = _lib.load()
@@ -253,5 +279,70 @@
         return gx, gw, gb, None, None
 
 
+def _side_by_side(problems: list) -> None:
+    small = [p for p in problems if 2.0 * p[0][2].numel() * (p[0][0].shape[0] if p[1]["a_rmajor"] else p[0][0].shape[1]) < SPLIT_MIN_FLOPS]
+    gemm_group(small)
+    for (a, b, c), kw in problems:
+        if not any(c is s[0][2] for s in small):
+            gemm(a, b, c, **kw)
+
+
+class _LinearGroup(torch.autograd.Function):
+
+    @staticmethod
+    def forward(ctx, pre_acts: tuple[int, ...], *flat: Tensor | None):
+        items, leads, problems, ys = [], [], [], []
+        for i, pre_act in enumerate(pre_acts):
+            x, weight, bias = flat[3 * i : 3 * i + 3]
+            x2 = x.reshape(-1, x.shape[-1])
+            if x2.stride(1) != 1:
+                x2 = x2.contiguous()
+            w = weight if weight.stride(1) == 1 else weight.contiguous()
+            y = torch.empty(x2.shape[0], w.shape[0], device=x.device, dtype=torch.float32)
+            problems.append(((x2, w, y), dict(a_rmajor=False, b_rmajor=False, bias=None if bias is None else bias.contiguous(), act_a=pre_act)))
+            items += [x2, weight, bias if bias is not None else x2.new_zeros(0)]
+            leads.append((x.shape[:-1], bias is not None))
+            ys.append(y.reshape(*x.shape[:-1], w.shape[0]))
+        _side_by_side(problems)
+        ctx.save_for_backward(*items)
+        ctx.leads, ctx.pre_acts = leads, pre_acts
+        return tuple(ys)
+
+    @staticmethod
+    def backward(ctx, *gys: Tensor | None):
+        saved = ctx.saved_tensors
+        items = [(saved[3 * i], saved[3 * i + 1], saved[3 * i + 2] if has_bias else None, lead) for i, (lead, has_bias) in enumerate(ctx.leads)]
+        problems, grads, gy2s = [], [], []
+        for i, ((x2, weight, _bias, lead), pre_act, gy) in enumerate(zip(items, ctx.pre_acts, gys, strict=True)):
+            gx = gy2 = None
+            if gy is not None:
+                gy2 = gy.reshape(-1, gy.shape[-1])
+                if gy2.stride(1) != 1:
+                    gy2 = gy2.contiguous()
+                if ctx.needs_input_grad[1 + 3 * i]:
+                    w = weight if weight.stride(1) == 1 else weight.contiguous()
+                    gx = torch.empty_like(x2)
+                    problems.append(((gy2, w, gx), dict(a_rmajor=False, b_rmajor=True, zgrad=x2 if pre_act else None, act_z=pre_act)))
+                    gx = gx.reshape(*lead, x2.shape[1])
+            gy2s.append(gy2)
+            grads.append(gx)
+        _side_by_side(problems)
+        out: list = [None]
+        for i, ((x2, weight, bias, _lead), pre_act, gy2, gx) in enumerate(zip(items, ctx.pre_acts, gy2s, grads, strict=True)):
+            gw = gb = None
+            if gy2 is not None:
+                gw, gb = weight_grad(gy2, x2, weight, bias, act_x=pre_act, want_weight=ctx.needs_input_grad[2 + 3 * i],
+                                     want_bias=bias is not None and ctx.needs_input_grad[3 + 3 * i])
+            out += [gx, gw, gb]
+        return tuple(out)
+
+
+def linear_group(items: list[tuple[Tensor, Tensor, Tensor | None, int]]) -> list[Tensor]:
+    if len(items) == 1 or not GROUP_GEMMS:
+        return [linear(x, w, b, pre_act=a) for x, w, b, a in items]
+    flat = [t for x, w, b, _ in items for t in (x, w, b)]
+    return list(_LinearGroup.apply(tuple(int(a) for *_, a in items), *flat))
+
+
 def linear(x: Tensor, weight: Tensor, bias: Tensor | None = None, *, pre_act: int = 0, pieces: int | None = None) -> Tensor:
     return _Linear.apply(x, weight, bias, int(pre_act), pieces)
diff --git a/multimodal_mtrssm_amd/scan.py b/multimodal_mtrssm_amd/scan.py
--- a/multimodal_mtrssm_amd/scan.py
+++ b/multimodal_mtrssm_amd/scan.py
@@ -10,7 +10,7 @@
 from multimodal_mtrssm_amd import _lib
 from multimodal_mtrssm_amd.distributions import KL_BALANCE_ALPHA
 from multimodal_mtrssm_amd import linear as _linear
-from multimodal_mtrssm_amd.linear import gemm, gemm_group, grad_target, linear
+from multimodal_mtrssm_amd.linear import gemm, gemm_group, grad_target, linear, linear_group
 
 
 @dataclass(frozen=True)
@@ -216,6 +216,58 @@
         if t is not None and tuple(t.shape) != tuple(shape):
             msg = f"{name}: expected shape {tuple(shape)}, got {tuple(t.shape)}"
             raise ValueError(msg)
+
+
+def _head_rows(w3: Tensor, wa1: Tensor, wv1: Tensor, D: int) -> Tensor:
+    return torch.cat([w3, wa1[:, :D], wv1[:, :D]], dim=0)
+
+
+SCAN_PREPARE = True
+
+
+def _row_major(t: Tensor) -> Tensor:
+    return t if t.dim() == 2 and t.stride(1) == 1 and t.stride(0) >= t.shape[1] else _c(t)
+
+
+def _cluster_layouts(w1, w2, b2, wih, bih, whh, w3, wa1, wv1, D: int, H: int, S: int, A: int):
+    if not SCAN_PREPARE:
+        w1s_t, whh_t = _c(w1[:, A:].t()), _c(whh.t())
+        wh1_t = _c(_head_rows(w3, wa1, wv1, D).t())
+        wf_t, bf = _new(w1, H, 3 * D), _new(w1, 1, 3 * D)
+        gemm(w2, wih, wf_t, a_rmajor=True, b_rmajor=False)
+        gemm(b2.reshape(1, H), wih, bf, a_rmajor=False, b_rmajor=False, bias=_c(bih))
+        return w1s_t, whh_t, wh1_t, wf_t, bf.reshape(-1)
+    lib = _lib.load()
+    off = (C.c_int64 * 5)()
+    total = int(lib.mtrssm_mrssm_scan_prepare_layout(D, H, S, off))
+    if total <= 0:
+        msg = f"mtrssm_mrssm_scan_prepare_layout refused D = {D}, H = {H}, S = {S}"
+        raise _lib.MtrssmLibraryError(msg)
+    buf = _new(w1, total)
+    w1, w2, wih, whh, w3, wa1, wv1 = map(_row_major, (w1, w2, wih, whh, w3, wa1, wv1))
+    b2, bih = _c(b2), _c(bih)
+    product = 2.0 * H * 3 * D * H < _linear.SPLIT_MIN_FLOPS
+    p = _lib.ScanPrepare()
+    p._refs = (w1, w2, b2, wih, bih, whh, w3, wa1, wv1, buf)
+    p.w1, p.w2, p.b2, p.wih, p.bih = map(_lib.raw_ptr, (w1, w2, b2, wih, bih))
+    p.whh, p.w3, p.wa1, p.wv1 = map(_lib.raw_ptr, (whh, w3, wa1, wv1))
+    p.ld_w1, p.ld_w2, p.ld_wih, p.ld_whh = w1.stride(0), w2.stride(0), wih.stride(0), whh.stride(0)
+    p.ld_w3, p.ld_wa1, p.ld_wv1 = w3.stride(0), wa1.stride(0), wv1.stride(0)
+    p.D, p.H, p.S, p.A, p.product = D, H, S, A, int(product)
+    p.out, p.out_floats = buf.data_ptr(), total
+    _lib.check(_lib.TIMERS.call("mtrssm_mrssm_scan_prepare", lib.mtrssm_mrssm_scan_prepare, C.byref(p), _lib.stream_ptr(buf.device),
+                                flops=2.0 * (H + 1) * 3 * D * H if product else 0.0,
+                                nbytes=4.0 * (2 * (S * H + 3 * D * D + 3 * H * D) + (H * H + 2 * 3 * D * H if product else 0))),
+               "mtrssm_mrssm_scan_prepare")
+    w1s_t = buf[off[0] : off[0] + S * H].view(S, H)
+    whh_t = buf[off[1] : off[1] + D * 3 * D].view(D, 3 * D)
+    wh1_t = buf[off[2] : off[2] + D * 3 * H].view(D, 3 * H)
+    wf_t = buf[off[3] : off[3] + H * 3 * D].view(H, 3 * D)
+    bf = buf[off[4] : off[4] + 3 * D]
+    if not product:
+        gemm(w2, wih, wf_t, a_rmajor=True, b_rmajor=False)
+        gemm(b2.reshape(1, H), wih, bf.view(1, 3 * D), a_rmajor=False, b_rmajor=False, bias=bih)
+    return w1s_t, whh_t, wh1_t, wf_t, bf
 
 
 class _MrssmScan(torch.autograd.Function):
@@ -245,9 +297,6 @@
         expert_logw = check_expert_logw(expert_logw, B, T)
         modality = _weighted_modality(_modality(modality, B, T), expert_logw)
         u_prior = _opt(u_prior)
-        w1s_t = _c(w1[:, A:].t())
-        wh1 = torch.cat([w3, wa1[:, :D], wv1[:, :D]], dim=0)
-        whh_t, wh1_t = _c(whh.t()), _c(wh1.t())
         deter = _new(xa, B, T, D)
         prior_logits, post_logits, post_stoch = (_new(xa, B, T, S) for _ in range(3))
         prior_stoch = _new(xa, B, T, S) if u_prior is not None else None
@@ -270,11 +319,9 @@
         cluster = CLUSTER_SCAN and plain and bool(lib.mtrssm_mrssm_cluster_supported(C.byref(dims)))
         wide = WIDE_SCAN and plain and not cluster and bool(lib.mtrssm_mrssm_wide_supported(C.byref(dims), WIDE_PIECES))
         ctx.scan_kind = "cluster" if cluster else ("wide" if wide else None)
+        wh1 = None
         if cluster or wide:
-            wf_t = _new(xa, H, 3 * D)
-            gemm(w2, wih, wf_t, a_rmajor=True, b_rmajor=False)
-            bf = _new(xa, 1, 3 * D)
-            gemm(b2.reshape(1, H), wih, bf, a_rmajor=False, b_rmajor=False, bias=_c(bih))
+            w1s_t, whh_t, wh1_t, wf_t, bf = _cluster_layouts(w1, w2, b2, wih, bih, whh, w3, wa1, wv1, D, H, S, A)
             cw = _lib.fill(_lib.MrssmClusterWeights(), w1s_t=w1s_t, wf_t=wf_t, bf=bf.reshape(-1), whh_t=whh_t, bhh=_c(bhh),
                            wh1_t=wh1_t, b3=_c(b3), w4=_c(w4), b4=_c(b4), wa2=_c(wa2), ba2=_c(ba2), wv2=_c(wv2), bv2=_c(bv2))
             io.sv_h2 = None
@@ -293,6 +340,9 @@
             ctx.cluster_w = (wf_t, whh_t, wh1_t)
         else:
             ctx.cluster_w = None
+            w1s_t = _c(w1[:, A:].t())
+            wh1 = _head_rows(w3, wa1, wv1, D)
+            whh_t, wh1_t = _c(whh.t()), _c(wh1.t())
             fw = _lib.fill(
                 _lib.MrssmFwdWeights(), w1s_t=w1s_t, w2_t=_c(w2.t()), b2=_c(b2), wih_t=_c(wih.t()), bih=_c(bih), whh_t=whh_t,
                 bhh=_c(bhh), wh1_t=wh1_t, b3=_c(b3), w4=_c(w4), b4=_c(b4), wa2=_c(wa2), ba2=_c(ba2), wv2=_c(wv2), bv2=_c(bv2),
@@ -323,8 +373,6 @@
             g_prior_stoch = None
         _expect(g_deter=(g_deter, (B, T, D)), g_prior_logits=(g_prior_logits, (B, T, S)), g_post_logits=(g_post_logits, (B, T, S)),
                 g_post_stoch=(g_post_stoch, (B, T, S)), g_prior_stoch=(g_prior_stoch, (B, T, S)), g_kl=(g_kl, (B, T)))
-        bw = _lib.fill(_lib.MrssmBwdWeights(), w1s_t=w1s_t, w2=_c(w2), wih=_c(wih), whh=_c(whh), wh1=wh1, w4=_c(w4), wa2=_c(wa2),
-                       wv2=_c(wv2))
         g_deter0, g_stoch0 = _new(deter, B, D), _new(deter, B, S)
         d_z1, d_h2 = _new(deter, B, T, H), _new(deter, B, T, H)
         d_gi, d_gh = _new(deter, B, T, 3 * D), _new(deter, B, T, 3 * D)
@@ -363,6 +411,10 @@
                                             flops=2.0 * B * T * macs, nbytes=4.0 * B * T * per_bt), "mtrssm_mrssm_rollout_bwd_wide")
             gemm(_flat2(d_gi), wih, _flat2(d_h2), a_rmajor=False, b_rmajor=True)
         else:
+            if wh1 is None:
+                wh1 = _head_rows(ctx.w3, wa1, wv1, D)
+            bw = _lib.fill(_lib.MrssmBwdWeights(), w1s_t=w1s_t, w2=_c(w2), wih=_c(wih), whh=_c(whh), wh1=wh1, w4=_c(w4), wa2=_c(wa2),
+                           wv2=_c(wv2))
             _lib.check(_lib.TIMERS.call("mtrssm_mrssm_rollout_bwd", lib.mtrssm_mrssm_rollout_bwd, C.byref(dims), C.byref(bw), C.byref(io),
                                         _lib.stream_ptr(deter.device), flops=2.0 * B * T * macs, nbytes=4.0 * B * T * per_bt),
                        "mtrssm_mrssm_rollout_bwd")
@@ -414,9 +466,11 @@
         msg = f"the HIP scan uses one activation for all heads, got {sorted(act_names)}"
         raise NotImplementedError(msg)
     cfg = ScanConfig(K, Cc, _lib.ACT_IDS[act_names.pop()], balancing, rows_per_block, threads)
-    xa = linear(actions, l1.weight[:, :A], l1.bias)
-    pa = _projection(audio_embed, a1, D, xa)
-    pv = _projection(vision_embed, v1, D, xa)
+    present = [(embed, layer) for embed, layer in ((audio_embed, a1), (vision_embed, v1)) if embed is not None]
+    outs = linear_group([(actions, l1.weight[:, :A], l1.bias, 0)] + [(embed, layer.weight[:, D:], layer.bias, 0) for embed, layer in present])
+    xa, rest = outs[0], outs[1:]
+    pa = rest.pop(0) if audio_embed is not None else _projection(None, a1, D, xa)
+    pv = rest.pop(0) if vision_embed is not None else _projection(None, v1, D, xa)
     cell = transition.rnn_cell
     deter, prior_logits, post_logits, post_stoch, prior_stoch, kl = _MrssmScan.apply(
         cfg, xa, pa, pv, deter0, stoch0, u_post, u_prior,
```

Result: faster. 386,100 seq-steps/s (median of 6 runs) (+2.2%).
